# wangbaonan/RAG-SNVBERT

Hardware: AMD Instinct MI355X
Metric: masked SNVs imputed/sec (+ kNN queries/sec), window=1024 k=32 (higher is better)
Workload: dtype bf16

## Files before the change

### include/snvrag.h

```cpp
#ifndef SNVRAG_H
#define SNVRAG_H

#include <stddef.h>
#include <stdint.h>

#ifdef __cplusplus
extern "C" {
#endif

#define SNVRAG_ABI_VERSION 31

enum { SNVRAG_F32 = 0, SNVRAG_BF16 = 1 };
enum { SNVRAG_ACT_NONE = 0, SNVRAG_ACT_GELU = 1, SNVRAG_ACT_LRELU = 2, SNVRAG_ACT_SIGMOID = 3 };

int snvrag_abi_version(void);
const char* snvrag_last_error(void);
int snvrag_device_info(int device, char* name, int name_len);
int snvrag_set_option(const char* name, int64_t value);
int snvrag_get_option(const char* name, int64_t* value);

typedef struct {
  const float* bias;
  const float* row1; int64_t row1_stride; const float* col1;
  const float* row2; int64_t row2_stride; const float* col2;
  int64_t row_period;
  int act; float slope;
  const void* resid; int64_t ld_resid;
  const float* ln_g; const float* ln_b; float ln_eps; int ln_act;
  const void* post_base; int64_t ld_post; float post_scale;
  const float* post_af; int64_t post_af_period; int post_maf;
  float* stats_out;
} snvrag_epilogue_t;

typedef struct {
  const float* stats; int n_parts; int64_t dim; float eps; const float* c1;
} snvrag_rownorm_t;

int snvrag_linear(int dtype_in, int dtype_out, int64_t M, int64_t N, int64_t K,
                  const void* A, int64_t lda, const void* W, int64_t ldw,
                  void* C, int64_t ldc, const snvrag_epilogue_t* epi, void* stream);
int snvrag_linear_ex(int dtype_in, int dtype_out, int64_t M, int64_t N, int64_t K,
                     const void* A, int64_t lda, const void* W, int64_t ldw,
                     void* C, int64_t ldc, const snvrag_epilogue_t* epi,
                     const snvrag_rownorm_t* rownorm, void* stream);

typedef struct {
  const void* base; int64_t ld_base;
  float scale;
  const float* af; int64_t af_period; int maf_weight;
  int act;
} snvrag_ln_post_t;

int snvrag_layernorm(int dtype_in, int dtype_out, int64_t M, int64_t N,
                     const void* X, int64_t ldx, const void* R, int64_t ldr,
                     const float* gamma, const float* beta, float eps,
                     void* Y, int64_t ldy, const snvrag_ln_post_t* post, void* stream);

int snvrag_attention(int dtype, int64_t nseq, int64_t L, int heads, int dh,
                     const void* qkv, int64_t ld_qkv, void* out, int64_t ld_out,
                     float scale, void* stream);
int snvrag_attention_fallbacks(int reset);

int snvrag_af_features(int dtype_out, int64_t M, const float* af, const float* freqs, int nb,
                       void* feat, void* stream);
int snvrag_embed_tokens(int dtype_out, int64_t nseq, int64_t L, int64_t D, const int64_t* tok,
                        const float* W, int64_t vocab, const float* pe, const void* afemb,
                        int afemb_dtype, int64_t af_period, void* out, void* stream);

typedef struct {
  const float* c1_w; const float* c1_b;
  const float* c2_w; const float* c2_b;
  const float* c3_w; const float* c3_b;
  const float* bn1_w; const float* bn1_b; const float* bn1_rm; const float* bn1_rv;
  const float* bn2_w; const float* bn2_b; const float* bn2_rm; const float* bn2_rv;
  float bn_eps;
} snvrag_posfeat_w_t;
int snvrag_posfeat(int64_t B, int64_t L, const float* pos, const snvrag_posfeat_w_t* w,
                   float* out, void* stream);

typedef struct {
  const float* g1_w; const float* g1_b;
  const float* g2_w; const float* g2_b;
  const float* j_w; const float* j_b;
  const float* ln_w; const float* ln_b;
  float res_scale;
} snvrag_afgate_w_t;
int snvrag_af_gate(int dtype_out, int64_t M, int64_t D, const float* af, const float* af_p,
                   const snvrag_afgate_w_t* w, void* out, void* stream);

int snvrag_rag_weighted_concat(int dtype, int64_t M, int64_t D, const void* q, const void* rag,
                               const void* wgt, int64_t period, void* out, void* stream);

int snvrag_hap_head_out(int dtype_in, int64_t M, int64_t K, const void* H, int64_t ldh,
                        const float* w , const float* b ,
                        float* logits , float* probs , void* stream);
typedef struct {
  const float* f_w; const float* f_b;
  const float* n_w; const float* n_b;
  const float* w1; const float* b1;
  const float* ln_w; const float* ln_b;
  const float* w2; const float* b2;
  const float* c_w; const float* c_b;
} snvrag_gt_w_t;
int snvrag_gt_head(int64_t M, const float* p1, const float* p2, const float* ref,
                   const float* het, const float* hom, int64_t period,
                   const snvrag_gt_w_t* w, float* out , void* stream);

size_t snvrag_knn_lut_bytes(int64_t nq, int32_t n_sites_pad, int limbs);
int snvrag_knn_lut(int64_t nq, int64_t L, int64_t D, const int64_t* tok_q, const float* W,
                   const float* Aq, int64_t aq_period, const float* Ar,
                   const uint8_t* site_mask, int32_t n_sites, int32_t n_sites_pad,
                   int tok0, int tok1, int mask_tok, int limbs,
                   void* lut_out, int32_t* exp_out, float* const_out, void* stream);
int snvrag_knn_lut_panel(int64_t nq, int64_t L, int64_t D, const int64_t* tok_q, const float* W,
                         const float* Wp, const float* Aq, int64_t aq_period, const float* Ar,
                         const uint8_t* site_mask, int32_t n_sites, int32_t n_sites_pad,
                         int tok0, int tok1, int mask_tok, int limbs,
                         void* lut_out, int32_t* exp_out, float* const_out, void* stream);

int snvrag_knn_scan_parts(int64_t n_ref, int32_t nq);
int snvrag_knn_scan(const uint8_t* codes, int64_t n_ref, int64_t ld_codes, int32_t n_sites_pad,
                    const void* lut, int32_t nq, int limbs, int k, int64_t ref_offset,
                    uint64_t* part_keys, int32_t n_parts, const int32_t* th_init, void* stream);
int snvrag_knn_threshold(const uint64_t* keys, int32_t nq, int k, int32_t* th_out, void* stream);
size_t snvrag_topk_merge_ws_bytes(int32_t n_lists, int32_t nq, int k);
int snvrag_topk_merge(const uint64_t* keys, int32_t n_lists, int32_t nq, int k,
                      uint64_t* out_keys, void* ws, size_t ws_bytes, void* stream);
int snvrag_knn_decode(const uint64_t* keys, int32_t nq, int k, const int32_t* exps,
                      const float* consts, int64_t* idx_out, float* dist_out, void* stream);

int snvrag_knn_emb_splits(int64_t N, int64_t K, int Bq);
size_t snvrag_knn_emb_ws_bytes(int64_t N, int Bq, int splits);
size_t snvrag_knn_emb_packed_bytes(int64_t N, int64_t K);
int snvrag_knn_emb_pack(const void* E, int64_t N, int64_t K, void* Et, void* stream);
int snvrag_knn_emb_scan(const void* Et, int64_t N, int64_t K, const void* Q, int Bq, int splits, float* ws,
                        void* stream);
int snvrag_knn_emb_finish(const float* ws, int splits, int Bq, int64_t N, const float* qn, const float* rn,
                          float* dist, void* stream);

int snvrag_rag_mean(int dtype_out, int64_t nq, int64_t L, int64_t D, int k, const int64_t* idx,
                    const uint8_t* codes, int64_t ld_codes, int32_t n_sites,
                    const float* W, const float* pe, const float* Ar,
                    int tok0, int tok1, int sos, int eos, int pad, void* out, void* stream);

int snvrag_neighbor_counts(int64_t nq, int k, const int64_t* idx, const uint8_t* codes, int64_t ld,
                           int64_t row0, int64_t n_rows, uint8_t* counts, int64_t ld_out, void* stream);
int snvrag_rag_mean_counts(int dtype_out, int64_t nq, int64_t L, int64_t D, int k, const int64_t* idx,
                           const uint8_t* counts, int64_t ld_counts, int32_t n_sites,
                           const float* W, const float* pe, const float* Ar,
                           int tok0, int tok1, int sos, int eos, int pad, void* out, void* stream);

int snvrag_panel_pack_bits(const uint8_t* codes, int64_t n, int64_t ld, uint8_t* bits, int64_t ld_bits,
                           void* stream);
int snvrag_panel_synth_bits(uint8_t* bits, int64_t row0, int64_t n_rows, int64_t ld_bits, int32_t n_sites,
                            const float* af, uint64_t seed, void* stream);
int snvrag_panel_unpack_rows(const uint8_t* bits, int64_t n_ref, int64_t ld_bits, const int64_t* rows,
                             int64_t n_rows, uint8_t* out, int64_t ld_out, void* stream);
int snvrag_knn_scan_bits(const uint8_t* bits, int64_t n_ref, int64_t ld_bits, int32_t n_sites_pad,
                         const void* lut, int32_t nq, int limbs, int k, int64_t ref_offset,
                         uint64_t* part_keys, int32_t n_parts, const int32_t* th_init, void* stream);
int snvrag_rag_mean_bits(int dtype_out, int64_t nq, int64_t L, int64_t D, int k, const int64_t* idx,
                         const uint8_t* bits, int64_t ld_bits, int32_t n_sites,
                         const float* W, const float* pe, const float* Ar,
                         int tok0, int tok1, int sos, int eos, int pad, void* out, void* stream);
int snvrag_neighbor_counts_bits(int64_t nq, int k, const int64_t* idx, const uint8_t* bits, int64_t ld_bits,
                                int64_t row0, int64_t n_rows, uint8_t* counts, int64_t ld_out, void* stream);

int snvrag_hamming_lists(int64_t nq, int64_t N, int32_t nw, int k, const uint32_t* codes_wm,
                         const uint32_t* queries, uint64_t* lists, void* stream);
int32_t snvrag_hamming_list_count(void);

int snvrag_panel_synth(uint8_t* codes, int64_t n_ref, int64_t ld, int32_t n_sites,
                       const float* af, uint64_t seed, void* stream);
int snvrag_panel_synth_rows(uint8_t* codes, int64_t row0, int64_t n_rows, int64_t ld, int32_t n_sites,
                            const float* af, uint64_t seed, void* stream);

typedef struct {
  const void* w_qkv; const float* b_qkv;
  const void* w_o; const float* b_o;
  const float* ln1_g; const float* ln1_b;
  const void* w1; const float* b1;
  const float* lnf_g; const float* lnf_b;
  const void* w2; const float* b2;
  const float* ln2_g; const float* ln2_b;
  const void* w2g; const float* b2g; const float* c2g;
  float q_scale;
  const float* ffn_v;
  const void* tail_w;
  const void* qkv_pw;
  const void* qkv_sg;
} snvrag_layer_t;

size_t snvrag_tail_pack_bytes(int D);
int snvrag_tail_pack(int D, const void* w_o, const void* w1, const void* w2g, void* out, void* stream);
int snvrag_tail_forward(int64_t M, int D, const void* att, void* x, const void* wstream, const float* b_o,
                        const float* ln1_g, const float* ln1_b, const float* ffn_vec, float eps, void* stream);
int snvrag_tail_ffn_forward(int64_t M, int D, const void* x1, void* out, const void* wstream,
                            const float* ffn_vec, float eps, void* stream);
int snvrag_tail_qkv_forward(int64_t M, int D, const void* att, void* x, const void* wstream, const float* b_o,
                            const float* ln1_g, const float* ln1_b, const float* ffn_vec, float eps,
                            const void* qkv_pw, const float* b_qkv, void* qkv_out, void* stream);
int snvrag_tail_stamps(void* buf);
size_t snvrag_proj_pack_bytes(int D, int NC);
int snvrag_proj_pack(int D, int NC, const void* w, void* out, void* stream);
int snvrag_proj_forward(int64_t M, int D, int NC, const void* x, const void* wstream, const float* bias,
                        void* out, void* stream);

int snvrag_sgemm_cat_forward(int64_t M, int Dh, int N, const void* q, const void* x2, const void* g2,
                             int64_t period2, const void* wstream, const float* vec, void* out, void* stream);
size_t snvrag_mlp_pack_bytes(int D);
int snvrag_mlp_pack(int D, const void* w1, const void* w2, void* out, void* stream);
int snvrag_mlp_forward(int64_t M, int D, int epi2, const void* x, const void* wstream, const float* vec,
                       const float* r1, const float* r2, int64_t period, float eps, void* out, void* stream);
int snvrag_mlp_afgate_forward(int64_t M, int D, const float* af, const float* af_p, const void* gate_frags,
                              float res_scale, const void* wstream, const float* vec, void* out, void* stream);
size_t snvrag_sgemm_pack_bytes(int D, int N);
int snvrag_sgemm_pack(int D, int N, const void* w, void* out, void* stream);

typedef struct {
  int32_t kind, nparts;
  int64_t rows, cols, dst_ld, piece0, pieces;
  int64_t part_rows[4], rs[4], cs[4];
  const float* src[4];
  void* dst;
} snvrag_derive_job_t;
int snvrag_derive(const snvrag_derive_job_t* jobs, int njobs, int64_t total_pieces, void* stream);

size_t snvrag_gemm256_pack_bytes(int N, int K);
int snvrag_gemm256_pack(int N, int K, const void* w, int64_t ldw, void* out, void* stream);
int snvrag_gemm256_forward(int64_t M, int N, int K, const void* A, int64_t lda, const void* wpacked, const float* bias,
                           const void* resid, int64_t ld_resid, void* out, int64_t ldo, void* stream);
int snvrag_gemm256_ln_forward(int64_t M, int N, int K, const void* A, int64_t lda, const void* wpacked,
                              const float* bias, const float* ln_g, const float* ln_b, float eps, const void* base,
                              int64_t ld_base, float post_scale, const float* post_af, int64_t post_af_period,
                              void* out, int64_t ldo, void* stream);

int snvrag_head2_fwd(int64_t M, int K, const void* x, const float* w, const float* b, float* out, void* stream);
size_t snvrag_head2_ws_bytes(int64_t M, int K);
size_t snvrag_tokgrad_ws_bytes(int64_t M, int V, int D);
int snvrag_tokgrad(int64_t M, int V, int D, int padding_idx, const int64_t* tok, const float* g, float* dw,
                   void* ws, size_t ws_bytes, void* stream);
int snvrag_head2_bwd(int64_t M, int K, const float* g, const void* x, const float* w, void* dx, float* dw,
                     int accumulate, void* ws, size_t ws_bytes, void* stream);
int snvrag_sgemm_forward(int64_t M, int D, int N, int epi, int act, float slope, const void* x,
                         const void* wstream, const float* vec, const float* r1, const float* r2,
                         int64_t period, float eps, void* out, float* probs, float* logits, void* stream);

size_t snvrag_encoder_ws_bytes(int dtype, int64_t nseq, int64_t L, int D, int heads);
int snvrag_encoder_forward(int dtype, int64_t nseq, int64_t L, int D, int heads, int n_layers,
                           const snvrag_layer_t* layers, void* x, void* ws, size_t ws_bytes,
                           void* stream);

int snvrag_evlog_enable(int capacity);
int snvrag_evlog_pause(int paused);
int snvrag_evlog_reset(void);
int snvrag_evlog_read(int* kinds, float* ms, double* work, int max);

int snvrag_attention_train_fwd(int64_t nseq, int64_t L, int heads, int dh, const void* qkv, int64_t ld_qkv,
                               void* out, int64_t ld_out, float* lse, float scale, float dropout_p,
                               uint64_t seed, void* stream);
int snvrag_attention_bwd(int64_t nseq, int64_t L, int heads, int dh, const void* qkv, int64_t ld_qkv,
                         const void* out, int64_t ld_out, const void* dout, int64_t ld_dout,
                         const float* lse, float* d_ws, void* dqkv, int64_t ld_dqkv, float scale,
                         float dropout_p, uint64_t seed, void* stream);
int snvrag_focal_loss(int64_t M, int C, const float* probs, const int64_t* labels, const uint8_t* mask,
                      float gamma, float weight, float* loss_sum, float* grad, void* stream);
size_t snvrag_focal_loss_det_ws_bytes(int64_t M);
int snvrag_focal_loss_det(int64_t M, int C, const float* probs, const int64_t* labels, const uint8_t* mask,
                          float gamma, float weight, float* loss_sum, float* grad, float* ws, size_t ws_bytes,
                          void* stream);
int snvrag_sqnorm(int64_t n, const float* x, float* acc, void* stream);
size_t snvrag_sqnorm_ws_bytes(void);
int snvrag_sqnorm_ws(int64_t n, const float* x, float* acc, float* ws, size_t ws_bytes, void* stream);
typedef struct {
  float lr, beta1, beta2, eps, weight_decay;
  float grad_scale;
  float max_norm;
  int step;
} snvrag_adam_t;
int snvrag_adam_step(int64_t n, float* p, const float* g, float* m, float* v, void* p_bf16,
                     const float* sqnorm, const snvrag_adam_t* a, void* stream);
int snvrag_confusion(int64_t M, int C, const float* probs, const int64_t* labels, const uint8_t* mask,
                     const uint8_t* mask2, uint64_t* counts, void* stream);

int snvrag_ln_fwd_train(int64_t M, int N, const void* x, const void* r, const float* g, const float* b,
                        float eps, void* y, void* s_out, float* stats, float p_r, float p_out, uint64_t seed,
                        void* stream);
int snvrag_ln_fwd_train_act(int64_t M, int N, const void* x, const void* r, const float* g, const float* b,
                            float eps, void* y, void* s_out, float* stats, float p_r, float p_out, uint64_t seed,
                            float slope_x, float slope_r, void* stream);
int snvrag_ln_bwd_act(int64_t M, int N, const void* dy, const void* s, const float* stats, const float* g,
                      void* ds, void* dres, const void* r_pre, float* dg, float* db, int accumulate, float p_r,
                      float p_out, uint64_t seed, float slope_x, float slope_r, void* ws, size_t ws_bytes,
                      void* stream);
int snvrag_nbr_mean_drop_fwd(int64_t nq, int k, int64_t L, int D, int n_sites, int64_t ld_codes, int V,
                             const int32_t* inv, const uint8_t* codes, const float* W, const float* pe,
                             const float* Ar, float p, uint64_t seed, int tok0, int sos, int eos, int pad,
                             float* out, void* stream);
int snvrag_nbr_mean_drop_bwd(int64_t nq, int k, int64_t L, int D, int n_sites, int64_t ld_codes, int V,
                             const int32_t* inv, const uint8_t* codes, const float* W, const float* pe,
                             const float* Ar, float p, uint64_t seed, int tok0, int sos, int eos, int pad,
                             const float* dout, float* dW, float* dAr, void* stream);
size_t snvrag_nbr_mean_drop_bwd_det_ws_bytes(int64_t L, int V, int D);
int snvrag_nbr_mean_drop_bwd_det(int64_t nq, int k, int64_t L, int D, int n_sites, int64_t ld_codes, int V,
                                 const int32_t* inv, const uint8_t* codes, const float* W, const float* pe,
                                 const float* Ar, float p, uint64_t seed, int tok0, int sos, int eos, int pad,
                                 const float* dout, float* dW, float* dAr, void* ws, size_t ws_bytes, void* stream);
size_t snvrag_ln_bwd_ws_bytes(int64_t M, int N);
int snvrag_ln_bwd(int64_t M, int N, const void* dy, const void* s, const float* stats, const float* g,
                  void* ds, void* dres, float* dg, float* db, int accumulate, float p_r, float p_out,
                  uint64_t seed, void* ws, size_t ws_bytes, void* stream);
size_t snvrag_colsum_ws_bytes(int64_t M, int N);
int snvrag_colsum_bf16(int64_t M, int N, const void* x, float* out, void* ws, size_t ws_bytes, void* stream);

int snvrag_dw_splits(int64_t M, int64_t N, int64_t K);
int snvrag_linear_dw(int64_t M, int64_t N, int64_t K, const void* dy, int64_t ldy, const void* x, int64_t ldx,
                     float* dw, float* db, int splits, void* stream);
int snvrag_linear_dw_parts(int64_t M, int64_t N, int64_t K, const void* dy, int64_t ldy, const void* x,
                           int64_t ldx, int n_parts, float* const* dw_parts, float* const* db_parts, int splits,
                           void* stream);
size_t snvrag_linear_dw_det_ws_bytes(int64_t M, int64_t N, int64_t K, int splits);
int snvrag_linear_dw_det(int64_t M, int64_t N, int64_t K, const void* dy, int64_t ldy, const void* x, int64_t ldx,
                         float* dw, float* db, int splits, void* ws, size_t ws_bytes, void* stream);
int snvrag_linear_dw_parts_det(int64_t M, int64_t N, int64_t K, const void* dy, int64_t ldy, const void* x,
                               int64_t ldx, int n_parts, float* const* dw_parts, float* const* db_parts,
                               int splits, void* ws, size_t ws_bytes, void* stream);

int snvrag_infer_post(int64_t M, const float* probs_h1, const float* probs_h2, float* p1, float* p2,
                      float* gt, void* stream);

int snvrag_infer_scatter(int64_t B, int32_t L, const float* probs_h1, const float* probs_h2,
                         const int64_t* mask, const int32_t* rows_dev, const int32_t* rows_host,
                         int32_t window_len, int64_t n_variants, int64_t S, float* hap1, float* hap2,
                         float* gp, int64_t* mask_out, void* stream);

typedef struct {
  const uint8_t* gt_bits;
  const int32_t* win_off;
  const int32_t* site_row;
  const int32_t* freq_col;
  const float* pos_norm;
  const uint8_t* win_mask;
  const float* freq;
  const int32_t* pop_of_sample;
  int64_t ld_bits;
  int64_t n_cols;
  int32_t n_samples;
  int32_t n_windows;
  int32_t max_window_sites;
  int32_t n_pop;
  int32_t global_row;
} snvrag_feature_tables_t;
int snvrag_batch_features(const snvrag_feature_tables_t* tables, const int32_t* rows_dev,
                          const int32_t* rows_host, int64_t B, int32_t L, int sos, int eos, int pad, int mask,
                          int tok0, int tok1, int64_t* tokens, int64_t* mask_out, float* floats, int64_t* labels,
                          void* stream);

int snvrag_vcf_format(int64_t n, int64_t S, const float* h1, const float* h2, const float* gt,
                      int64_t n_lines, const int32_t* rows, const int64_t* line_off, const int32_t* prefix_off,
                      const uint8_t* prefix_blob, int64_t prefix_bytes, uint8_t* out, int64_t out_bytes,
                      int32_t* bad_count, void* stream);

int snvrag_site_stats(int64_t n, int64_t S, const float* h1, const float* h2, const float* gt,
                      const int8_t* truth, int64_t n_truth, int64_t S_truth, const int32_t* truth_row,
                      const int32_t* truth_col, double* est, double* acc, int32_t* table, int32_t* bad_count,
                      void* stream);

size_t snvrag_vcf_line_index_ws_bytes(int64_t nbytes);
int snvrag_vcf_line_index(const uint8_t* text, int64_t nbytes, int64_t max_lines, int64_t* line_off,
                          int64_t* n_lines, void* ws, size_t ws_bytes, void* stream);
size_t snvrag_vcf_parse_ws_bytes(int64_t n_lines, int64_t S);
int snvrag_vcf_parse_gt(const uint8_t* text, int64_t nbytes, const int64_t* line_off, int64_t n_lines,
                        int64_t S, int force_general, int32_t* pos, uint32_t* flags, uint8_t* codes,
                        int64_t ld_codes, void* ws, size_t ws_bytes, void* stream);
int snvrag_vcf_pack_rows(const uint8_t* codes, int64_t ld_codes, int64_t n_lines, int64_t S, int64_t site0,
                         uint8_t* alt_bits, uint8_t* miss_bits, int64_t ld_bits, void* stream);
int snvrag_panel_gather_bits(const uint8_t* bits, int64_t N, int64_t ld_bits, int64_t n_src_sites,
                             const int32_t* site_idx, int64_t n, int64_t n_sites_pad, int packed, uint8_t* out,
                             void* stream);
int snvrag_vcf_unpack_gt(const uint8_t* alt_bits, const uint8_t* miss_bits, int64_t ld_bits, int64_t S,
                         int64_t n_sites, int8_t* gt, void* stream);

enum { SNVRAG_INFL_OK = 0, SNVRAG_INFL_BAD_TYPE = 1, SNVRAG_INFL_BAD_STORED = 2, SNVRAG_INFL_BAD_LENGTHS = 3,
       SNVRAG_INFL_BAD_SYMBOL = 4, SNVRAG_INFL_BAD_DISTANCE = 5, SNVRAG_INFL_INPUT_END = 6,
       SNVRAG_INFL_OUTPUT_FULL = 7, SNVRAG_INFL_OUTPUT_SHORT = 8, SNVRAG_INFL_BAD_CRC = 9 };
int snvrag_bgzf_inflate(const uint8_t* comp, int64_t comp_bytes, const int64_t* table_host, int64_t* table_dev,
                        int64_t n_blocks, uint8_t* text, int64_t text_bytes, int32_t* status, void* stream);
int snvrag_text_last_newline(const uint8_t* text, int64_t nbytes, int64_t* out, void* stream);

int snvrag_bgzf_deflate(const uint8_t* text, int64_t nbytes, int64_t block_size, uint8_t* members,
                        int32_t* member_len, void* stream);
int snvrag_bgzf_pack(const uint8_t* members, const int32_t* member_len, int64_t n_blocks, uint8_t* out,
                     int64_t out_bytes, int64_t* total, void* stream);

int snvrag_selftest_mfma(void* stream);

#ifdef __cplusplus
}
#endif
#endif
```

### rag-snvbert_amd/csrc/common.h

```cpp
#pragma once
#include <hip/hip_runtime.h>
#include <stdint.h>
#include <stddef.h>
#include <string>
#include <type_traits>

#pragma clang diagnostic ignored "-Winline-asm"

#include "../../include/snvrag.h"
#include "host.h"

namespace snvrag {

typedef __bf16 bf16;
typedef __bf16 bf16x8 __attribute__((ext_vector_type(8)));
typedef __bf16 bf16x4 __attribute__((ext_vector_type(4)));
typedef float f32x4 __attribute__((ext_vector_type(4)));
typedef float f32x16 __attribute__((ext_vector_type(16)));
typedef int i32x4 __attribute__((ext_vector_type(4)));
typedef uint32_t u32x4 __attribute__((ext_vector_type(4)));

void set_error(const std::string& msg);

enum EvKind { EV_GEMM = 1, EV_ATTN = 2, EV_LN = 3, EV_KNN_SCAN = 4, EV_KNN_LUT = 5, EV_MERGE = 6, EV_OTHER = 7, EV_BLOCK = 8,
              EV_ATTN_BWD = 10, EV_TRAIN = 11 };
bool evlog_on();
void evlog_begin(hipStream_t s);
void evlog_end(hipStream_t s, int kind, double work);
struct Options {
  int64_t knn_no_reduce;
  int64_t scan_mode;
  int64_t scan_nt;
  int64_t unfused_ln;
  int64_t encoder_chunk;
  int64_t gemm_tile128;
  int64_t gemm_nw;
  int64_t tail_variant;
  int64_t tail_desync;
  int64_t sg_desync;
  int64_t mlp_desync;
  int64_t g2_desync;
  int64_t sg_waves4;
  int64_t ln_bwd_nopf;
  int64_t attn_variant;
  int64_t dw_xcd;
  int64_t ln_rows1;
  int64_t g2_groups;
  int64_t g2_variant;
  int64_t tail_split;
  int64_t proj_wide;
  int64_t tail_wide;
  int64_t tail_qkv;
  int64_t deterministic;
};
Options& options();
unsigned long long* diag_stamps();

int tailw_launch(int M, const void* att, const void* resid, void* out, const void* ws, const float* vec,
                 const float* b_o, const float* g1, const float* be1, float eps, int desync, int var,
                 const void* pw, const float* pbias, void* qkv_out, hipStream_t s);

int projw_launch(int M, int NC, const void* x, const void* ws, const float* bias, void* out, int desync, hipStream_t s);

__device__ __forceinline__ i32x4 dma_rsrc(const void* base, long bytes) {
  const uint64_t a = (uint64_t)(uintptr_t)base;
  i32x4 r;
  r[0] = __builtin_amdgcn_readfirstlane((int)(uint32_t)a);
  r[1] = __builtin_amdgcn_readfirstlane((int)((uint32_t)(a >> 32) & 0xffffu));
  r[2] = __builtin_amdgcn_readfirstlane((int)(bytes < 0x7fffffffL ? bytes : 0x7fffffffL));
  r[3] = 0x00020000;
  return r;
}

__device__ __forceinline__ void dma_x4(const i32x4& rsrc, uint32_t lds, int voffset, int soffset) {
  asm volatile("s_mov_b32 m0, %0\n\ts_nop 0\n\tbuffer_load_dwordx4 %1, %2, %3 offen lds"
               :
               : "s"(lds), "v"(voffset), "s"(rsrc), "s"(soffset)
               : "memory", "m0");
}
__device__ __forceinline__ uint32_t lds_addr(const void* p) {
  return __builtin_amdgcn_readfirstlane((int)(uint32_t)(uintptr_t)p);
}
template <typename A, typename B>
__device__ __forceinline__ void retire_loads(A& a, B& b) { asm volatile("" : "+v"(a), "+v"(b)); }
template <typename A, typename B, typename C>
__device__ __forceinline__ void retire_loads(A& a, B& b, C& c) { asm volatile("" : "+v"(a), "+v"(b), "+v"(c)); }

template <int PPT>
__device__ __forceinline__ void ring_wait(int y) {
  if (y >= 2) asm volatile("s_waitcnt vmcnt(%0)" ::"n"(2 * PPT) : "memory");
  else if (y == 1) asm volatile("s_waitcnt vmcnt(%0)" ::"n"(PPT) : "memory");
  else asm volatile("s_waitcnt vmcnt(0)" ::: "memory");
}

__device__ __forceinline__ float to_f32(float x) { return x; }
__device__ __forceinline__ float to_f32(bf16 x) { return (float)x; }
template <typename T> __device__ __forceinline__ T from_f32(float x);
template <> __device__ __forceinline__ float from_f32<float>(float x) { return x; }
template <> __device__ __forceinline__ bf16 from_f32<bf16>(float x) { return (bf16)x; }

__device__ __forceinline__ float gelu_erf(float x) {
  const float ax = fabsf(x) * 0.70710678118654752f;
  const float t = __builtin_amdgcn_rcpf(fmaf(0.3275911f, ax, 1.0f));
  float q = fmaf(t, 1.061405429f, -1.453152027f);
  q = fmaf(t, q, 1.421413741f);
  q = fmaf(t, q, -0.284496736f);
  q = fmaf(t, q, 0.254829592f);
  q = t * q * __builtin_amdgcn_exp2f(ax * ax * -1.4426950408889634f);
  return x * (x >= 0.f ? fmaf(-0.5f, q, 1.0f) : 0.5f * q);
}
__device__ __forceinline__ float gelu_bf16(float x) {
  constexpr float L2E = 1.4426950408889634f;
  const float xc = __builtin_amdgcn_fmed3f(x, -8.f, 8.f);
  const float x2 = xc * xc;
  const float z = xc * fmaf(x2, fmaf(x2, 7.03033577e-4f * L2E, -7.40112920e-2f * L2E), -1.59501577f * L2E);
  return x * __builtin_amdgcn_rcpf(1.0f + __builtin_amdgcn_exp2f(z));
}
__device__ __forceinline__ float sigmoidf_(float x) { return 1.0f / (1.0f + __expf(-x)); }

__device__ __forceinline__ float apply_act(int act, float x, float slope) {
  switch (act) {
    case SNVRAG_ACT_GELU: return gelu_erf(x);
    case SNVRAG_ACT_LRELU: return x >= 0.f ? x : x * slope;
    case SNVRAG_ACT_SIGMOID: return 1.0f / (1.0f + expf(-x));
    default: return x;
  }
}
template <typename TO> __device__ __forceinline__ float apply_act_t(int act, float x, float slope) {
  if constexpr (std::is_same<TO, bf16>::value) {
    if (act == SNVRAG_ACT_GELU) return gelu_bf16(x);
  }
  return apply_act(act, x, slope);
}

__device__ __forceinline__ float wave_sum(float v) {
#pragma unroll
  for (int o = 32; o >= 1; o >>= 1) v += __shfl_xor(v, o, 64);
  return v;
}
template <int CTRL> __device__ __forceinline__ float dpp_mov(float v) {
  return __builtin_bit_cast(float, __builtin_amdgcn_update_dpp(0, __builtin_bit_cast(int, v), CTRL, 0xF, 0xF, false));
}
template <int W> __device__ __forceinline__ float group_sum(float v) {
  static_assert(W == 2 || W == 4 || W == 8 || W == 16, "group width");
  v += dpp_mov<0xB1>(v);
  if constexpr (W >= 4) v += dpp_mov<0x4E>(v);
  if constexpr (W >= 8) v += dpp_mov<0x141>(v);
  if constexpr (W >= 16) v += dpp_mov<0x140>(v);
  return v;
}
__device__ __forceinline__ float wave_max(float v) {
#pragma unroll
  for (int o = 32; o >= 1; o >>= 1) v = fmaxf(v, __shfl_xor(v, o, 64));
  return v;
}

}
```

### rag-snvbert_amd/csrc/engine.hip

```cpp
#include "common.h"

#include <cmath>

namespace snvrag {

static int64_t chunk_seqs(int64_t nseq, int64_t L, int D, int esz) {
  if (options().encoder_chunk > 0) return std::min<int64_t>(options().encoder_chunk, nseq);
  const double per_seq = (double)L * D * 10.0 * esz;
  int64_t c = (int64_t)(16.0e9 / per_seq);
  if (c < 1) c = 1;
  if (c >= nseq) return nseq;
  const int64_t nchunks = (nseq + c - 1) / c;
  return (nseq + nchunks - 1) / nchunks;
}

}

using namespace snvrag;

extern "C" size_t snvrag_encoder_ws_bytes(int dtype, int64_t nseq, int64_t L, int D, int heads) {
  (void)heads;
  const int esz = dtype == SNVRAG_BF16 ? 2 : 4;
  const int64_t c = chunk_seqs(nseq, L, D, esz);
  const size_t M = (size_t)c * L;
  return M * (size_t)D * 9 * esz + M * 64 * 8 + 8192;
}

extern "C" int snvrag_encoder_forward(int dtype, int64_t nseq, int64_t L, int D, int heads, int n_layers,
                                      const snvrag_layer_t* layers, void* x, void* ws, size_t ws_bytes,
                                      void* stream) {
  SNV_CHECK_PTRS(layers, x, ws);
  SNV_CHECK_ARG(D % heads == 0, "D % heads");
  SNV_CHECK_ARG(ws_bytes >= snvrag_encoder_ws_bytes(dtype, nseq, L, D, heads), "encoder workspace too small");
  const int esz = dtype == SNVRAG_BF16 ? 2 : 4;
  const int64_t cs = chunk_seqs(nseq, L, D, esz);
  const size_t Mc = (size_t)cs * L;
  char* w = (char*)ws;
  auto carve = [&](size_t elems) { char* p = w; w += ((elems * esz + 255) / 256) * 256; return (void*)p; };
  void* qkv = carve(Mc * 3 * D);
  void* att = carve(Mc * D);
  void* x1 = carve(Mc * D);
  void* h = carve(Mc * 4 * D);
  const int n_stat_parts = (4 * D) % 384 == 0 ? (4 * D) / 384 : (4 * D) % 256 == 0 ? (4 * D) / 256
                           : (4 * D) % 128 == 0 ? (4 * D) / 128 : (4 * D) / 64;
  w = (char*)(((uintptr_t)w + 255) & ~(uintptr_t)255);
  void* stats = w; w += ((Mc * n_stat_parts * 8 + 255) / 256) * 256;
  const int dh = D / heads;
  const float scale = 1.0f / sqrtf((float)dh);

  const bool fused = (D == 64 || D == 128 || D == 256 || D == 384) && !options().unfused_ln &&
                     layers[0].w2g && layers[0].b2g && layers[0].c2g;
  for (int64_t s0 = 0; s0 < nseq; s0 += cs) {
    const int64_t ns = std::min<int64_t>(cs, nseq - s0);
    const int64_t M = ns * L;
    char* xc = (char*)x + (size_t)s0 * L * D * esz;
    bool have_qkv = false;
    for (int i = 0; i < n_layers; ++i) {
      const snvrag_layer_t& ly = layers[i];
      snvrag_epilogue_t e{};
      int rc;
      e.bias = ly.b_qkv;
      if (have_qkv)
        rc = 0;
      else if (dtype == SNVRAG_BF16 && ly.qkv_sg && M * 3 * D * 2 < (1L << 31))
        rc = snvrag_sgemm_forward(M, (int)D, (int)(3 * D), 0, SNVRAG_ACT_NONE, 0.f, xc, ly.qkv_sg, ly.b_qkv, nullptr,
                                  nullptr, 0, 0.f, qkv, nullptr, nullptr, stream);
      else if (dtype == SNVRAG_BF16 && ly.qkv_pw)
        rc = snvrag_proj_forward(M, D, 3, xc, ly.qkv_pw, ly.b_qkv, qkv, stream);
      else
        rc = snvrag_linear(dtype, dtype, M, 3 * D, D, xc, D, ly.w_qkv, D, qkv, 3 * D, &e, stream);
      if (rc) return rc;
      const float sc = ly.q_scale > 0.f ? scale / ly.q_scale : scale;
      rc = snvrag_attention(dtype, ns, L, heads, dh, qkv, 3 * D, att, D, sc, stream);
      if (rc) return rc;
      if (fused && dtype == SNVRAG_BF16 && ly.tail_w && ly.ffn_v) {
        have_qkv = i + 1 < n_layers && D == 384 && options().tail_qkv && options().tail_variant == 0 &&
                   (options().tail_wide == 1 || options().tail_wide == 2) && layers[i + 1].qkv_pw &&
                   layers[i + 1].b_qkv && M * 3 * D * 2 < (1L << 31);
        if (have_qkv)
          rc = snvrag_tail_qkv_forward(M, D, att, xc, ly.tail_w, ly.b_o, ly.ln1_g, ly.ln1_b, ly.ffn_v, 1e-5f,
                                       layers[i + 1].qkv_pw, layers[i + 1].b_qkv, qkv, stream);
        else
          rc = snvrag_tail_forward(M, D, att, xc, ly.tail_w, ly.b_o, ly.ln1_g, ly.ln1_b, ly.ffn_v, 1e-5f, stream);
        if (rc) return rc;
        continue;
      }
      if (fused) {
        e = snvrag_epilogue_t{};
        e.bias = ly.b_o; e.resid = xc; e.ld_resid = D; e.ln_g = ly.ln1_g; e.ln_b = ly.ln1_b; e.ln_eps = 1e-5f;
        rc = snvrag_linear(dtype, dtype, M, D, D, att, D, ly.w_o, D, x1, D, &e, stream);
        if (rc) return rc;
        e = snvrag_epilogue_t{};
        e.bias = ly.b1; e.act = SNVRAG_ACT_LRELU; e.slope = 0.1f; e.stats_out = (float*)stats;
        rc = snvrag_linear(dtype, dtype, M, 4 * D, D, x1, D, ly.w1, D, h, 4 * D, &e, stream);
        if (rc) return rc;
        snvrag_rownorm_t rn{(const float*)stats, n_stat_parts, 4 * D, 1e-5f, ly.c2g};
        e = snvrag_epilogue_t{};
        e.bias = ly.b2g; e.act = SNVRAG_ACT_LRELU; e.slope = 0.1f; e.resid = x1; e.ld_resid = D;
        e.ln_g = ly.ln2_g; e.ln_b = ly.ln2_b; e.ln_eps = 1e-5f;
        rc = snvrag_linear_ex(dtype, dtype, M, D, 4 * D, h, 4 * D, ly.w2g, 4 * D, xc, D, &e, &rn, stream);
        if (rc) return rc;
        continue;
      }
      e = snvrag_epilogue_t{};
      e.bias = ly.b_o; e.resid = xc; e.ld_resid = D;
      rc = snvrag_linear(dtype, dtype, M, D, D, att, D, ly.w_o, D, x1, D, &e, stream);
      if (rc) return rc;
      rc = snvrag_layernorm(dtype, dtype, M, D, x1, D, nullptr, 0, ly.ln1_g, ly.ln1_b, 1e-5f, x1, D, nullptr, stream);
      if (rc) return rc;
      e = snvrag_epilogue_t{};
      e.bias = ly.b1; e.act = SNVRAG_ACT_LRELU; e.slope = 0.1f;
      rc = snvrag_linear(dtype, dtype, M, 4 * D, D, x1, D, ly.w1, D, h, 4 * D, &e, stream);
      if (rc) return rc;
      rc = snvrag_layernorm(dtype, dtype, M, 4 * D, h, 4 * D, nullptr, 0, ly.lnf_g, ly.lnf_b, 1e-5f, h, 4 * D,
                            nullptr, stream);
      if (rc) return rc;
      e = snvrag_epilogue_t{};
      e.bias = ly.b2; e.act = SNVRAG_ACT_LRELU; e.slope = 0.1f; e.resid = x1; e.ld_resid = D;
      rc = snvrag_linear(dtype, dtype, M, D, 4 * D, h, 4 * D, ly.w2, 4 * D, xc, D, &e, stream);
      if (rc) return rc;
      rc = snvrag_layernorm(dtype, dtype, M, D, xc, D, nullptr, 0, ly.ln2_g, ly.ln2_b, 1e-5f, xc, D, nullptr, stream);
      if (rc) return rc;
    }
  }
  return 0;
}
```

### rag-snvbert_amd/csrc/misc.hip

```cpp
#include "common.h"

#include <cctype>
#include <cstdlib>
#include <cstring>

namespace snvrag {

static thread_local std::string g_err;

struct EvLog {
  bool on = false;
  int cap = 0, n = 0;
  hipEvent_t* ev = nullptr;
  int* kind = nullptr;
  double* work = nullptr;
};
static EvLog g_ev;

bool evlog_on() { return g_ev.on && g_ev.n < g_ev.cap; }
void evlog_begin(hipStream_t s) {
  if (evlog_on()) (void)hipEventRecord(g_ev.ev[2 * g_ev.n], s);
}
void evlog_end(hipStream_t s, int kind, double work) {
  if (!evlog_on()) return;
  (void)hipEventRecord(g_ev.ev[2 * g_ev.n + 1], s);
  g_ev.kind[g_ev.n] = kind;
  g_ev.work[g_ev.n] = work;
  g_ev.n++;
}

void set_error(const std::string& msg) { g_err = msg; }
int fail(const char* where, const std::string& msg) {
  g_err = std::string(where) + ": " + msg;
  return 1;
}

__global__ void mfma_selftest_kernel(int* errors) {
  const int lane = threadIdx.x, li = lane & 15, lg = lane >> 4;
  __shared__ int A[16][64], B[64][16];
  for (int i = lane; i < 16 * 64; i += 64) {
    const int r = i / 64, k = i % 64;
    A[r][k] = ((r * 7 + k * 3) % 11) - 5;
    B[k][r] = ((k * 5 + r * 13) % 9) - 4;
  }
  __syncthreads();
  int err = 0;
  {
    int8_t a8[16], b8[16];
    for (int j = 0; j < 16; ++j) { a8[j] = (int8_t)A[li][16 * lg + j]; b8[j] = (int8_t)B[16 * lg + j][li]; }
    i32x4 av = *reinterpret_cast<i32x4*>(a8), bv = *reinterpret_cast<i32x4*>(b8);
    i32x4 c = __builtin_amdgcn_mfma_i32_16x16x64_i8(av, bv, i32x4{0, 0, 0, 0}, 0, 0, 0);
    for (int i = 0; i < 4; ++i) {
      const int row = 4 * lg + i, col = li;
      int ref = 0;
      for (int k = 0; k < 64; ++k) ref += A[row][k] * B[k][col];
      err += c[i] != ref;
    }
  }
  {
    bf16x8 av, bv;
    for (int j = 0; j < 8; ++j) { av[j] = (bf16)(float)A[li][8 * lg + j]; bv[j] = (bf16)(float)B[8 * lg + j][li]; }
    f32x4 c = __builtin_amdgcn_mfma_f32_16x16x32_bf16(av, bv, f32x4{0, 0, 0, 0}, 0, 0, 0);
    for (int i = 0; i < 4; ++i) {
      const int row = 4 * lg + i, col = li;
      int ref = 0;
      for (int k = 0; k < 32; ++k) ref += A[row][k] * B[k][col];
      err += c[i] != (float)ref;
    }
  }
  {
    f32x4 c = __builtin_amdgcn_mfma_f32_16x16x4f32((float)A[li][lg], (float)B[lg][li], f32x4{0, 0, 0, 0}, 0, 0, 0);
    for (int i = 0; i < 4; ++i) {
      const int row = 4 * lg + i, col = li;
      int ref = 0;
      for (int k = 0; k < 4; ++k) ref += A[row][k] * B[k][col];
      err += c[i] != (float)ref;
    }
  }
  atomicAdd(errors, err);
}

}

using namespace snvrag;

namespace snvrag {
namespace {
struct OptDesc { const char* name; int64_t Options::*field; int64_t dflt; };
const OptDesc kOpts[] = {
    {"knn_no_reduce", &Options::knn_no_reduce, 0}, {"scan_mode", &Options::scan_mode, 0},
    {"scan_nt", &Options::scan_nt, -1},            {"unfused_ln", &Options::unfused_ln, 0},
    {"encoder_chunk", &Options::encoder_chunk, 0}, {"gemm_tile128", &Options::gemm_tile128, 0},
    {"gemm_nw", &Options::gemm_nw, 0},             {"tail_variant", &Options::tail_variant, 0},
    {"tail_desync", &Options::tail_desync, -1},    {"sg_desync", &Options::sg_desync, -1},      {"mlp_desync", &Options::mlp_desync, -1},      {"g2_desync", &Options::g2_desync, -1},
    {"sg_waves4", &Options::sg_waves4, 0},         {"ln_bwd_nopf", &Options::ln_bwd_nopf, 0},
    {"attn_variant", &Options::attn_variant, 0},   {"dw_xcd", &Options::dw_xcd, 1},
    {"ln_rows1", &Options::ln_rows1, 0},           {"tail_wide", &Options::tail_wide, 1},
    {"proj_wide", &Options::proj_wide, 1},         {"g2_variant", &Options::g2_variant, 0},
    {"g2_groups", &Options::g2_groups, 0},         {"tail_split", &Options::tail_split, 64},
    {"deterministic", &Options::deterministic, 0}, {"tail_qkv", &Options::tail_qkv, 1},
};
Options make_options() {
  Options o{};
  for (const OptDesc& d : kOpts) {
    std::string env = "SNVRAG_";
    for (const char* c = d.name; *c; ++c) env += (char)toupper(*c);
    const char* v = getenv(env.c_str());
    o.*(d.field) = v ? atoll(v) : d.dflt;
  }
  return o;
}
const OptDesc* find_opt(const char* name) {
  for (const OptDesc& d : kOpts)
    if (name && strcmp(d.name, name) == 0) return &d;
  return nullptr;
}
}
Options& options() {
  static Options o = make_options();
  return o;
}
}

extern "C" int snvrag_set_option(const char* name, int64_t value) {
  const snvrag::OptDesc* d = snvrag::find_opt(name);
  if (!d) return fail(__func__, std::string("unknown option ") + (name ? name : "(null)"));
  snvrag::options().*(d->field) = value;
  return 0;
}

extern "C" int snvrag_get_option(const char* name, int64_t* value) {
  const snvrag::OptDesc* d = snvrag::find_opt(name);
  if (!d || !value) return fail(__func__, std::string("unknown option ") + (name ? name : "(null)"));
  *value = snvrag::options().*(d->field);
  return 0;
}

extern "C" int snvrag_abi_version(void) { return SNVRAG_ABI_VERSION; }
extern "C" const char* snvrag_last_error(void) { return g_err.c_str(); }

extern "C" int snvrag_device_info(int device, char* name, int name_len) {
  hipDeviceProp_t p;
  if (hipGetDeviceProperties(&p, device) != hipSuccess) return -1;
  if (name && name_len > 0) {
    std::strncpy(name, p.gcnArchName, name_len - 1);
    name[name_len - 1] = 0;
  }
  return p.multiProcessorCount;
}

extern "C" int snvrag_evlog_enable(int capacity) {
  if (g_ev.ev) {
    for (int i = 0; i < 2 * g_ev.cap; ++i) (void)hipEventDestroy(g_ev.ev[i]);
    delete[] g_ev.ev; delete[] g_ev.kind; delete[] g_ev.work;
    g_ev = EvLog{};
  }
  if (capacity <= 0) return 0;
  g_ev.ev = new hipEvent_t[2 * capacity];
  g_ev.kind = new int[capacity];
  g_ev.work = new double[capacity];
  for (int i = 0; i < 2 * capacity; ++i) SNV_HIP(hipEventCreate(&g_ev.ev[i]));
  g_ev.cap = capacity;
  g_ev.n = 0;
  g_ev.on = true;
  return 0;
}

extern "C" int snvrag_evlog_pause(int paused) { g_ev.on = !paused && g_ev.cap > 0; return 0; }
extern "C" int snvrag_evlog_reset(void) { g_ev.n = 0; return 0; }

extern "C" int snvrag_evlog_read(int* kinds, float* ms, double* work, int max) {
  const int n = g_ev.n < max ? g_ev.n : max;
  for (int i = 0; i < n; ++i) {
    SNV_HIP(hipEventSynchronize(g_ev.ev[2 * i + 1]));
    float t = 0.f;
    SNV_HIP(hipEventElapsedTime(&t, g_ev.ev[2 * i], g_ev.ev[2 * i + 1]));
    kinds[i] = g_ev.kind[i];
    ms[i] = t;
    work[i] = g_ev.work[i];
  }
  return n;
}

extern "C" int snvrag_selftest_mfma(void* stream) {
  int* d = nullptr;
  SNV_HIP(hipMalloc(&d, sizeof(int)));
  hipStream_t s = as_stream(stream);
  SNV_HIP(hipMemsetAsync(d, 0, sizeof(int), s));
  hipLaunchKernelGGL(mfma_selftest_kernel, dim3(1), dim3(64), 0, s, d);
  int h = -1;
  SNV_HIP(hipMemcpyAsync(&h, d, sizeof(int), hipMemcpyDeviceToHost, s));
  SNV_HIP(hipStreamSynchronize(s));
  SNV_HIP(hipFree(d));
  return h;
}
```

### rag-snvbert_amd/csrc/tailw.hip

```cpp
#include "common.h"
#include "mfma32.h"

namespace snvrag {

#ifndef TW_PACKED_LN
#define TW_PACKED_LN 1
#endif

constexpr int TW_D = 384, TW_NT = 12, TW_KS = 24;
constexpr int TW_FPRE = TW_NT * TW_KS;
constexpr int TW_FPC = 96;
constexpr int TW_NFRAG = TW_FPRE + 24 * TW_FPC;
constexpr int TW_X = 0;
constexpr int TW_H = 96 * 1024;
constexpr int TW_LDS = 160 * 1024;
constexpr int TW_AH = 9;
constexpr int TW_RING = 12;
constexpr int TW_QA = 24;
constexpr int TW_Q0 = 48;
constexpr int TW_HS = 32;
constexpr int TW_QF = TW_Q0 + 11 * TW_HS;
constexpr int TW_QEND = TW_QF + 8;
constexpr int TW_QREP = TW_Q0 + TW_HS;
constexpr int TW_NB1 = 4;

__host__ __device__ constexpr int tw_nf(int q) {
  return q < 0 ? 0 : q < TW_QA ? 3 : q < TW_Q0 ? 1 : q < TW_QF ? ((q - TW_Q0) % TW_HS < 24 ? 1 : 3) : q < TW_QEND ? 3 : 0;
}
__host__ __device__ constexpr int tw_f0(int q) {
  if (q <= TW_QA) return 3 * q;
  if (q <= TW_Q0) return 72 + (q - TW_QA);
  if (q <= TW_QF) {
    const int k = (q - TW_Q0) / TW_HS, r = (q - TW_Q0) % TW_HS;
    return 96 + 48 * k + (r <= 24 ? r : 24 + 3 * (r - 24));
  }
  return q <= TW_QEND ? 624 + 3 * (q - TW_QF) : 648;
}
__host__ __device__ constexpr int tw_step_of(int m) {
  if (m < 72) return m / 3;
  if (m < 96) return TW_QA + (m - 72);
  if (m < 624) {
    const int k = (m - 96) / 48, r = (m - 96) % 48;
    return TW_Q0 + TW_HS * k + (r < 24 ? r : 24 + (r - 24) / 3);
  }
  return TW_QF + (m - 624) / 3;
}
constexpr int TW_NFRAGW = 648;
__host__ __device__ constexpr int tw_extra(int q) {
  return (q == TW_QA + 16 || (q >= TW_Q0 && q < TW_QF && (q - TW_Q0) % TW_HS == 24)) ? TW_NB1 : 0;
}
__host__ __device__ constexpr int tw_issuer(int n) { return n < TW_AH ? -1 : tw_step_of(n - TW_AH); }
__host__ __device__ constexpr int tw_min(int a, int b) { return a < b ? a : b; }
__host__ __device__ constexpr int tw_younger(int q) {
  const int nl = tw_f0(q) + tw_nf(q) - 1;
  int n = tw_min(tw_f0(q) + TW_AH, TW_NFRAGW) - 1 - nl;
  const int qi = tw_issuer(nl);
  for (int j = qi < 0 ? 0 : qi; j < q; ++j) n += tw_extra(j);
  return n;
}
__host__ __device__ constexpr int tw_ops_between(int qa, int qb) {
  int n = 0;
  for (int q = qa + 1; q <= qb; ++q) n += (tw_f0(q) + TW_AH < TW_NFRAGW ? tw_nf(q) : 0) + tw_extra(q);
  return n;
}
constexpr int TW_B1_WAIT = tw_min(tw_ops_between(TW_QA + 16, TW_Q0 + 2), tw_ops_between(TW_Q0 + 24, TW_QREP + 2));
constexpr int TW_B1_WAIT_END = tw_ops_between(TW_Q0 + 10 * TW_HS + 24, TW_QF - 1);
__host__ __device__ constexpr int tw_younger_it(int i) {
  int m = 63;
  for (int h = 1; h <= 11; ++h) m = tw_min(m, tw_younger(TW_Q0 + (h - 1) * TW_HS + i));
  return m;
}
__host__ __device__ constexpr int tw_wait_of(int q) {
  return (q >= TW_QREP && q < TW_QREP + TW_HS) ? tw_younger_it(q - TW_QREP) : tw_younger(q);
}
__host__ __device__ constexpr bool tw_ring_periodic() {
  return tw_f0(TW_QEND) == TW_NFRAGW && tw_f0(TW_QA) % TW_RING == 0 && tw_f0(TW_Q0) % TW_RING == 0 &&
         tw_f0(TW_QREP) % TW_RING == 0 && (tw_f0(TW_QREP + TW_HS) - tw_f0(TW_QREP)) % TW_RING == 0 &&
         tw_f0(TW_QF) % TW_RING == 0;
}
static_assert(tw_ring_periodic(), "fragment ring registers periodic over the sections");
static_assert(TW_B1_WAIT_END <= 63 && tw_younger(0) <= 63, "vmcnt range");

#ifndef TW_NOPMASK
#define TW_NOPMASK 2
#endif
__device__ __forceinline__ void tw_drain_o(f32x16 (&a)[3][4]) {
  asm volatile("s_nop 7\n\ts_nop 7\n\ts_nop 7"
               : "+a"(a[0][0]), "+a"(a[0][1]), "+a"(a[0][2]), "+a"(a[0][3]), "+a"(a[1][0]), "+a"(a[1][1]),
                 "+a"(a[1][2]), "+a"(a[1][3]), "+a"(a[2][0]), "+a"(a[2][1]), "+a"(a[2][2]), "+a"(a[2][3])
               :: "memory");
}
template <bool AGPR> __device__ __forceinline__ void tw_drain_h4(f32x16 (&h)[4]) {
  if constexpr (AGPR)
    asm volatile("s_nop 7\n\ts_nop 7\n\ts_nop 7" : "+a"(h[0]), "+a"(h[1]), "+a"(h[2]), "+a"(h[3]) :: "memory");
  else
    asm volatile("s_nop 7\n\ts_nop 7\n\ts_nop 7" : "+v"(h[0]), "+v"(h[1]), "+v"(h[2]), "+v"(h[3]) :: "memory");
}
__device__ __forceinline__ f32x2 tw_lrelu2(f32x2 x) {
  const f32x2 m = x * 0.1f;
  float a, b;
  asm("v_max_f32 %0, %1, %2" : "=v"(a) : "v"(x.x), "v"(m.x));
  asm("v_max_f32 %0, %1, %2" : "=v"(b) : "v"(x.y), "v"(m.y));
  return f32x2{a, b};
}
__device__ __forceinline__ void tw_ld16p(const char* p, float (&v)[16]) {
#pragma unroll
  for (int i = 0; i < 4; ++i) {
    const f32x4 q = *reinterpret_cast<const f32x4*>(p + 16 * i);
#pragma unroll
    for (int j = 0; j < 4; ++j) v[4 * i + j] = q[j];
  }
}
#ifndef TW_ASM_WAITS
#define TW_ASM_WAITS 0
#endif
template <int Y> __device__ __forceinline__ void tw_wait1(u32x4& a) {
  static_assert(Y >= 0 && Y <= 63, "vmcnt range");
  if constexpr (TW_ASM_WAITS) asm volatile("s_waitcnt vmcnt(%1)" : "+v"(a) : "n"(Y) : "memory");
}
template <int Y> __device__ __forceinline__ void tw_wait3(u32x4& a, u32x4& b, u32x4& c) {
  static_assert(Y >= 0 && Y <= 63, "vmcnt range");
  if constexpr (TW_ASM_WAITS) asm volatile("s_waitcnt vmcnt(%3)" : "+v"(a), "+v"(b), "+v"(c) : "n"(Y) : "memory");
}
template <int OFF> __device__ __forceinline__ void tw_load_off(u32x4& r, int voff, const i32x4& rsrc, int so) {
  asm volatile("buffer_load_dwordx4 %0, %1, %2, %3 offen offset:%4" : "=v"(r) : "v"(voff), "s"(rsrc), "s"(so), "n"(OFF) : "memory");
}
__device__ __forceinline__ void tw_barrier() { asm volatile("s_waitcnt lgkmcnt(0)\n\ts_barrier" ::: "memory"); }

struct TwArgs {
  int M;
  const bf16* att;
  const bf16* resid;
  bf16* out;
  const char* ws;
  const float* vec;
  const float* b_o; const float* g1; const float* be1;
  float eps;
  int desync;
  unsigned long long* stamps;
  int n_full;
  const char* pw;
  const float* pbias;
  bf16* qkv_out;
};

__device__ __forceinline__ void pw_loadW(u32x4& r, const __amdgpu_buffer_rsrc_t wrb, int lane16, int wave, int NC, int c,
                                         int n72) {
  const int cc = c < NC ? c : NC - 1;
  r = __builtin_amdgcn_raw_buffer_load_b128(wrb, lane16, (cc * TW_FPRE + (n72 / 3) * TW_NT + 3 * wave + n72 % 3) * FRAG_BYTES, 0);
}
template <int G, bool NOP>
__device__ __forceinline__ void pw_chunks(const char* smem, uint32_t bias_lds, int wave, int lane16,
                                          const __amdgpu_buffer_rsrc_t wrb, int NC, const __amdgpu_buffer_rsrc_t ors,
                                          u32x4 (&wf)[TW_RING], f32x16 (&acc)[3][4]) {
  constexpr int D = TW_D, KS = TW_KS, GI = G > 1 ? 1 : 0;
  auto rdB = [&](int blk) -> u32x4 { return *reinterpret_cast<const u32x4*>(smem + TW_X + blk * FRAG_BYTES + lane16); };
  u32x4 bq[2][4];
#pragma unroll 1
  for (int c = 0; c < NC; ++c) {
#pragma unroll
    for (int g = 0; g < G; ++g) bq[0][g] = rdB(g);
    unroll([&](auto sc) {
      constexpr int s = decltype(sc)::value, n0 = 3 * s;
#pragma unroll
      for (int g = 0; g < G; ++g) {
#pragma unroll
        for (int t = 0; t < 3; ++t) {
          if constexpr (s == 0) mfma32_asm0<true, NOP>(acc[t][g], wf[(n0 + t) % TW_RING], bq[s & 1][g]);
          else mfma32_asm<true, NOP>(acc[t][g], wf[(n0 + t) % TW_RING], bq[s & 1][g]);
        }
        if constexpr (s + 1 < KS) bq[(s + 1) & 1][g] = rdB((s + 1) * 4 + g);
        if (g == GI) {
#pragma unroll
          for (int t = 0; t < 3; ++t) {
            const int m = n0 + TW_AH + t;
            if (m < 72) pw_loadW(wf[(n0 + TW_AH + t) % TW_RING], wrb, lane16, wave, NC, c, m);
            else pw_loadW(wf[(n0 + TW_AH + t) % TW_RING], wrb, lane16, wave, NC, c + 1, m - 72);
          }
        }
      }
      __builtin_amdgcn_sched_barrier(0);
    }, std::make_integer_sequence<int, KS>{});
    tw_drain_o(acc);
    const int l = lane_id();
    const uint32_t bb = bias_lds + 4 * (c * D + 16 * (l >> 5));
#pragma unroll
    for (int t = 0; t < 3; ++t) {
      const int T = 3 * wave + t;
      float bv[16];
      ld16(bb + 4 * 32 * T, bv);
#pragma unroll
      for (int g = 0; g < G; ++g) {
        const int ro = ((32 * g + (l & 31)) * NC * D + c * D + 32 * T + 16 * (l >> 5)) * 2;
#pragma unroll
        for (int h2 = 0; h2 < 2; ++h2) {
          float y[8];
#pragma unroll
          for (int j = 0; j < 8; ++j) y[j] = acc[t][g][8 * h2 + j] + bv[8 * h2 + j];
          __builtin_amdgcn_raw_buffer_store_b128(u32x4{pack2(y[0], y[1]), pack2(y[2], y[3]), pack2(y[4], y[5]),
                                                       pack2(y[6], y[7])},
                                                 ors, ro + 16 * h2, 0, 0);
        }
      }
    }
  }
}
__device__ __forceinline__ __amdgpu_buffer_rsrc_t pw_out_rsrc(bf16* out, int M, long row0, int NC) {
  const long o_bytes = ((long)M - row0) * NC * TW_D * 2;
  return __builtin_amdgcn_make_buffer_rsrc((void*)(out + row0 * NC * TW_D), (short)0,
                                           (int)(o_bytes < 0x7fffffffL ? o_bytes : 0x7fffffffL), 0x00020000);
}

template <bool STAMP, int G, bool PROJ>
__device__ __forceinline__ void tailw_body(const TwArgs& p, const long row0, const int wave) {
  constexpr int D = TW_D, NT = TW_NT, GI = G > 1 ? 1 : 0;
  constexpr uint32_t TW_PB = TW_H + 16 * 1024;
  constexpr int TW_RES_STEP = 21;
  constexpr bool NOPA = G == 1 || (TW_NOPMASK & 1), NOP0 = G == 1 || (TW_NOPMASK & 2);
  constexpr bool NOPT = G == 1 || (TW_NOPMASK & 4), NOPF = G == 1 || (TW_NOPMASK & 8);
  constexpr bool NOPP = G == 1 || (TW_NOPMASK & 16);
  using TNA = std::integral_constant<bool, NOP0>;
  using TNT = std::integral_constant<bool, NOPT>;
  using TNF = std::integral_constant<bool, NOPF>;
  extern __shared__ __attribute__((aligned(16))) char smem[];
  unsigned long long st[8] = {};
  auto stamp = [&](int i) {
    if constexpr (STAMP) st[i] = __builtin_amdgcn_s_memtime();
  };
  if (p.desync > 0 && blockIdx.x < 256) stagger_wait(p.desync);
  stamp(0);
  const uint32_t lds0 = lds_addr(smem);
  int lane16 = lane_id() * 16;
  asm volatile("" : "+v"(lane16));

  const i32x4 ars = dma_rsrc(p.att + row0 * D, ((long)p.M - row0) * D * 2);
  const i32x4 wrs = dma_rsrc(p.ws, (long)TW_NFRAG * FRAG_BYTES);
  const i32x4 brs = dma_rsrc(p.vec, 4L * D * 4);
  {
    const int l = lane_id();
    const int voff = (32 * wave + (l & 31)) * (D * 2) + 32 * (l >> 5);
    if (wave < G) {
#pragma unroll
      for (int s = 0; s < TW_KS; ++s)
        dma_x4(ars, lds0 + TW_X + (s * 4 + wave) * FRAG_BYTES, voff, 64 * (s >> 1) + 16 * (s & 1));
    }
  }
  u32x4 wf[TW_RING];
  const __amdgpu_buffer_rsrc_t wrb = __builtin_amdgcn_make_buffer_rsrc((void*)p.ws, (short)0, TW_NFRAG * FRAG_BYTES, 0x00020000);
  auto loadW = [&](u32x4& r, int F) { r = __builtin_amdgcn_raw_buffer_load_b128(wrb, lane16, F * FRAG_BYTES, 0); };
  auto f_ffn1 = [&](int h, int i) { return TW_FPRE + (4 * (h >> 1) + wave) * TW_FPC + 2 * i + (h & 1); };
  auto f_ffn2 = [&](int h, int u, int t) {
    return TW_FPRE + (4 * (h >> 1) + (u >> 1)) * TW_FPC + 48 + (2 * (h & 1) + (u & 1)) * NT + 3 * wave + t;
  };
  auto issue_a = [&](auto n_tag) {
    constexpr int n = decltype(n_tag)::value;
    if constexpr (n < 72) loadW(wf[n % TW_RING], (n / 3) * NT + 3 * wave + n % 3);
    else if constexpr (n < 96) loadW(wf[n % TW_RING], f_ffn1(0, n - 72));
    else loadW(wf[n % TW_RING], f_ffn1(1, n - 96));
  };
  unroll([&](auto nc) { issue_a(nc); }, std::make_integer_sequence<int, TW_AH>{});
  u32x4 rr[3][4][2];
  auto load_res = [&]() {
    const int l = lane_id();
#pragma unroll
    for (int g = 0; g < G; ++g) {
      long r = row0 + 32 * g + (l & 31);
      r = r < p.M ? r : (long)p.M - 1;
#pragma unroll
      for (int t = 0; t < 3; ++t)
#pragma unroll
        for (int h2 = 0; h2 < 2; ++h2)
          rr[t][g][h2] = *reinterpret_cast<const u32x4*>(p.resid + r * D + 32 * (3 * wave + t) + 16 * (l >> 5) + 8 * h2);
    }
  };
  float* tab = reinterpret_cast<float*>(smem + TW_H);
  for (int i = 64 * wave + lane_id(); i < D; i += 256) {
    tab[i] = p.b_o[i];
    tab[D + i] = p.g1[i];
    tab[2 * D + i] = p.be1[i];
  }
  asm volatile("s_waitcnt vmcnt(0)" ::: "memory");
  tw_barrier();
  stamp(1);

  f32x16 acc[3][4];
  u32x4 bq[3][4];
  auto rdB = [&](uint32_t base, int blk) -> u32x4 {
    return *reinterpret_cast<const u32x4*>(smem + base + blk * FRAG_BYTES + lane16);
  };
#pragma unroll
  for (int g = 0; g < G; ++g) bq[0][g] = rdB(TW_X, g);
  unroll([&](auto qc) {
    constexpr int q = decltype(qc)::value, n0 = 3 * q;
    tw_wait3<tw_younger(q)>(wf[n0 % TW_RING], wf[(n0 + 1) % TW_RING], wf[(n0 + 2) % TW_RING]);
#pragma unroll
    for (int g = 0; g < G; ++g) {
#pragma unroll
      for (int t = 0; t < 3; ++t) {
        if constexpr (q == 0) mfma32_asm0<true, NOPA>(acc[t][g], wf[(n0 + t) % TW_RING], bq[q & 1][g]);
        else mfma32_asm<true, NOPA>(acc[t][g], wf[(n0 + t) % TW_RING], bq[q & 1][g]);
      }
      if constexpr (q + 1 < TW_KS) bq[(q + 1) & 1][g] = rdB(TW_X, (q + 1) * 4 + g);
      if (g == GI)
        unroll([&](auto tc) { issue_a(std::integral_constant<int, n0 + TW_AH + decltype(tc)::value>{}); },
                  std::make_integer_sequence<int, 3>{});
    }
    if constexpr (q == TW_RES_STEP) load_res();
    __builtin_amdgcn_sched_barrier(0);
  }, std::make_integer_sequence<int, TW_QA>{});
  tw_drain_o(acc);
  stamp(2);

  float2* s1 = reinterpret_cast<float2*>(smem + TW_H + 8 * 1024);
  {
    const uint32_t tb = lds0 + TW_H + 64 * (lane_id() >> 5);
#if TW_PACKED_LN
    f32x2 s2v[4], q2v[4];
#pragma unroll
    for (int g = 0; g < G; ++g) s2v[g] = q2v[g] = f32x2{0.f, 0.f};
#pragma unroll
    for (int t = 0; t < 3; ++t) {
      float bo[16];
      tw_ld16p(smem + (tb - lds0) + 4 * 32 * (3 * wave + t), bo);
#pragma unroll
      for (int g = 0; g < G; ++g)
#pragma unroll
        for (int e = 0; e < 8; ++e) {
          const f32x2 v = f32x2{acc[t][g][2 * e], acc[t][g][2 * e + 1]} + f32x2{bo[2 * e], bo[2 * e + 1]} +
                          bf_pair(rr[t][g][e >> 2][e & 3]);
          acc[t][g][2 * e] = v.x;
          acc[t][g][2 * e + 1] = v.y;
          s2v[g] += v;
          q2v[g] = v * v + q2v[g];
        }
    }
    float sum[4], sq[4];
#pragma unroll
    for (int g = 0; g < G; ++g) {
      sum[g] = s2v[g].x + s2v[g].y;
      sq[g] = q2v[g].x + q2v[g].y;
    }
#else
    float sum[4] = {0.f, 0.f, 0.f, 0.f}, sq[4] = {0.f, 0.f, 0.f, 0.f};
#pragma unroll
    for (int t = 0; t < 3; ++t) {
      float bo[16];
      tw_ld16p(smem + (tb - lds0) + 4 * 32 * (3 * wave + t), bo);
#pragma unroll
      for (int g = 0; g < G; ++g)
#pragma unroll
        for (int i = 0; i < 16; ++i) {
          const float v = acc[t][g][i] + bo[i] + bf_at(rr[t][g][i >> 3], i & 7);
          acc[t][g][i] = v;
          sum[g] += v;
          sq[g] = fmaf(v, v, sq[g]);
        }
    }
#endif
#pragma unroll
    for (int t = 0; t < 3; ++t)
#pragma unroll
      for (int g = 0; g < G; ++g) {}
    const int l = lane_id();
#pragma unroll
    for (int g = 0; g < G; ++g) {
      sum[g] = xsum32(sum[g]);
      sq[g] = xsum32(sq[g]);
      s1[wave * 128 + 32 * g + (l & 31)] = make_float2(sum[g], sq[g]);
    }
  }
  tw_barrier();
  {
    const int l = lane_id();
    const uint32_t tb = lds0 + TW_H + 64 * (l >> 5);
    float mean[4], rstd[4];
#pragma unroll
    for (int g = 0; g < G; ++g) {
      float a = 0.f, b = 0.f;
#pragma unroll
      for (int w2 = 0; w2 < 4; ++w2) {
        const float2 v = s1[w2 * 128 + 32 * g + (l & 31)];
        a += v.x;
        b += v.y;
      }
      mean[g] = a * (1.0f / D);
      rstd[g] = 1.0f / sqrtf(fmaxf(b * (1.0f / D) - mean[g] * mean[g], 0.f) + p.eps);
    }
#pragma unroll
    for (int t = 0; t < 3; ++t) {
      float gg[16], bb[16];
      tw_ld16p(smem + (tb - lds0) + 4 * (D + 32 * (3 * wave + t)), gg);
      tw_ld16p(smem + (tb - lds0) + 4 * (2 * D + 32 * (3 * wave + t)), bb);
      const int T = 3 * wave + t;
#pragma unroll
      for (int g = 0; g < G; ++g) {
        float y[16];
#if TW_PACKED_LN
        const float nmr = -mean[g] * rstd[g];
#pragma unroll
        for (int e = 0; e < 8; ++e) {
          const f32x2 z = (f32x2{acc[t][g][2 * e], acc[t][g][2 * e + 1]} * rstd[g] + nmr) * f32x2{gg[2 * e], gg[2 * e + 1]} +
                          f32x2{bb[2 * e], bb[2 * e + 1]};
          y[2 * e] = z.x;
          y[2 * e + 1] = z.y;
        }
#else
#pragma unroll
        for (int i = 0; i < 16; ++i) y[i] = (acc[t][g][i] - mean[g]) * rstd[g] * gg[i] + bb[i];
#endif
#pragma unroll
        for (int h2 = 0; h2 < 2; ++h2)
          *reinterpret_cast<u32x4*>(smem + TW_X + ((2 * T + h2) * 4 + g) * FRAG_BYTES + lane16) =
              u32x4{pack2(y[8 * h2], y[8 * h2 + 1]), pack2(y[8 * h2 + 2], y[8 * h2 + 3]),
                    pack2(y[8 * h2 + 4], y[8 * h2 + 5]), pack2(y[8 * h2 + 6], y[8 * h2 + 7])};
      }
    }
  }
  tw_barrier();
  stamp(3);

  f32x16 hv[4], ha[4];
#pragma unroll
  for (int t = 0; t < 3; ++t)
#pragma unroll
    for (int g = 0; g < G; ++g) acc[t][g] = f32x16{};
#pragma unroll
  for (int t = 0; t < 3; ++t)
#pragma unroll
    for (int g = 0; g < G; ++g) asm volatile("" : "+a"(acc[t][g]));
  typedef float f2 __attribute__((ext_vector_type(2)));
  float sa1[4], sa2[4];
#pragma unroll
  for (int g = 0; g < G; ++g) sa1[g] = sa2[g] = 0.f;
  u32x4 b1v[4];
  const __amdgpu_buffer_rsrc_t b1b = __builtin_amdgcn_make_buffer_rsrc((void*)p.vec, (short)0, 4 * D * 4, 0x00020000);
  auto b1_load = [&](int h) {
    const int so = 4 * (64 * (4 * (h >> 1) + wave) + 32 * (h & 1));
    const int vo = 16 * (lane_id() >> 5);
#pragma unroll
    for (int r = 0; r < 4; ++r) b1v[r] = __builtin_amdgcn_raw_buffer_load_b128(b1b, vo + 32 * r, so, 0);
  };
  constexpr int TW_EP = 3 * G;
  float ex[8];
  uint32_t epk[4];
  auto epi_piece = [&](auto k_tag, auto q_tag, auto p_tag) {
    constexpr int k = decltype(k_tag)::value, Q = decltype(q_tag)::value, pc = decltype(p_tag)::value;
    constexpr int g = k >> 1, j = k & 1;
    if constexpr (g < G) {
      const f32x16& a = Q ? ha[g] : hv[g];
      unroll([&](auto vc) {
        constexpr int v = decltype(vc)::value;
        if constexpr (v * (TW_EP - 2) / 8 == pc) {
          const float u = a[8 * j + v] + __uint_as_float(b1v[(8 * j + v) >> 2][(8 * j + v) & 3]);
          const float x = fmaxf(u, 0.1f * u);
          ex[v] = x;
          sa1[g] += x;
          sa2[g] = fmaf(x, x, sa2[g]);
        }
      }, std::make_integer_sequence<int, 8>{});
      if constexpr (pc == TW_EP - 2) {
#pragma unroll
        for (int e2 = 0; e2 < 4; ++e2) epk[e2] = pack2(ex[2 * e2], ex[2 * e2 + 1]);
      }
      if constexpr (pc == TW_EP - 1)
        *reinterpret_cast<u32x4*>(smem + TW_H + Q * 32768 + ((wave * 2 + j) * 4 + g) * FRAG_BYTES + lane16) =
            u32x4{epk[0], epk[1], epk[2], epk[3]};
    }
  };
  auto issue_it = [&](auto r_tag, int h, auto last_tag) {
    constexpr int r = decltype(r_tag)::value, n = r;
    if constexpr (r < 24) loadW(wf[n % TW_RING], f_ffn1(h, r));
    else if constexpr (r < 48) loadW(wf[n % TW_RING], f_ffn2(h - 1, (r - 24) / 3, (r - 24) % 3));
    else if constexpr (decltype(last_tag)::value) loadW(wf[n % TW_RING], f_ffn2(h, (r - 48) / 3, (r - 48) % 3));
    else loadW(wf[n % TW_RING], f_ffn1(h + 1, r - 48));
  };
  auto seg1 = [&](int h, auto p_tag, auto q0_tag, auto epi_tag, auto nop_tag) {
    constexpr int P = decltype(p_tag)::value, Q0 = decltype(q0_tag)::value;
    constexpr bool EPI = decltype(epi_tag)::value, NOP = decltype(nop_tag)::value;
    constexpr int F0 = tw_f0(Q0);
    unroll([&](auto ic) {
      constexpr int i = decltype(ic)::value, q = Q0 + i, n = F0 + i;
      tw_wait1<tw_wait_of(q)>(wf[n % TW_RING]);
      unroll([&](auto gc) {
        constexpr int g = decltype(gc)::value;
        if constexpr (P == 0) {
          if constexpr (i == 0) mfma32_asm0<false, NOP>(hv[g], wf[n % TW_RING], bq[(i + 2) % 3][g]);
          else mfma32_asm<false, NOP>(hv[g], wf[n % TW_RING], bq[(i + 2) % 3][g]);
        } else {
          if constexpr (i == 0) mfma32_asm0<true, NOP>(ha[g], wf[n % TW_RING], bq[(i + 2) % 3][g]);
          else mfma32_asm<true, NOP>(ha[g], wf[n % TW_RING], bq[(i + 2) % 3][g]);
        }
        if constexpr (i + 2 < 24) bq[(i + 4) % 3][g] = rdB(TW_X, (i + 2) * 4 + g);
        if constexpr (g == GI) {
          if constexpr (Q0 == TW_QA) issue_a(std::integral_constant<int, n + TW_AH>{});
          else issue_it(std::integral_constant<int, i + TW_AH>{}, h, std::false_type{});
        }
        if constexpr (EPI) {
          epi_piece(std::integral_constant<int, i / 3>{}, std::integral_constant<int, 1 - P>{},
                    std::integral_constant<int, (i % 3) * G + g>{});
          __builtin_amdgcn_sched_barrier(0);
        }
      }, std::make_integer_sequence<int, G>{});
      if constexpr (Q0 == TW_QA && i == 16) b1_load(0);
      __builtin_amdgcn_sched_barrier(0);
    }, std::make_integer_sequence<int, 24>{});
    if constexpr (P == 0) tw_drain_h4<false>(hv);
    else tw_drain_h4<true>(ha);
  };
  auto seg2 = [&](int h, auto p_tag, auto q0_tag, auto last_tag, auto final_tag, auto nop_tag) {
    constexpr int P = decltype(p_tag)::value, Q0 = decltype(q0_tag)::value;
    constexpr bool LAST = decltype(last_tag)::value, FINAL = decltype(final_tag)::value;
    constexpr bool NOP = decltype(nop_tag)::value;
    constexpr uint32_t HB = TW_H + P * 32768;
    constexpr int F0 = tw_f0(Q0);
// ... 348 lines not shown
```

### rag-snvbert_amd/src/engine.py

```python

from __future__ import annotations

import weakref
from typing import Dict, Optional

import math
import os

import torch
import torch.nn as nn

from . import kernels as K
from . import native as N

_ENGINES: "weakref.WeakKeyDictionary[nn.Module, Engine]" = weakref.WeakKeyDictionary()


def engine_for(module: nn.Module) -> "Engine":
    eng = _ENGINES.get(module)
    if eng is None:
        eng = Engine(module)
        _ENGINES[module] = eng
    return eng


def _rag_block_current(x: Dict[str, torch.Tensor]) -> bool:
    if "rag_emb_h1" not in x or "rag_mean" not in x:
        return True
    m, B = x["rag_mean"], x["rag_emb_h1"].shape[0]
    return (x["rag_emb_h1"].data_ptr() == m.data_ptr() and x["rag_emb_h2"].data_ptr() == m[B:].data_ptr()
            and x["rag_emb_h1"].dtype == m.dtype)


def set_compute_dtype(module: nn.Module, dtype: torch.dtype) -> None:
    engine_for(module).set_dtype(dtype)


class _Packed:
    pass


class Engine:
    rag_tail_wide = True
    rag_afgate_fused = True

    def __init__(self, root: nn.Module):
        self.root = root
        self.dtype = torch.float32
        self._packed: Optional[_Packed] = None
        self._key = None
        self._enc_ws: Optional[torch.Tensor] = None

    def set_dtype(self, dtype: torch.dtype) -> None:
        if dtype not in (torch.float32, torch.bfloat16):
            raise ValueError("compute dtype must be float32 or bfloat16")
        if dtype != self.dtype:
            self.dtype, self._packed = dtype, None
        _, _, emb = self._modules()
        if emb is not None and emb is not self.root:
            engine_for(emb).set_dtype(dtype)

    def _modules(self):
        r = self.root
        from .model.foundation_model import BERTFoundationModel
        from .model.bert import BERT
        from .model.embedding.bert import BERTEmbedding
        from .model.embedding.af_embedding import AFEmbedding
        if isinstance(r, BERTFoundationModel):
            return r, r.bert, r.bert.embedding
        if isinstance(r, BERT):
            return None, r, r.embedding
        if isinstance(r, BERTEmbedding):
            return None, None, r
        if isinstance(r, AFEmbedding):
            return None, None, None
        raise TypeError(f"no native engine for {type(r).__name__}")

    def _param_key(self):
        from .autograd_ops import _EPOCH
        return (_EPOCH[0],) + tuple((p.data_ptr(), p._version) for p in self.root.parameters()) + \
            tuple((b.data_ptr(), b._version) for b in self.root.buffers())

    def packed(self, allow_train: bool = False) -> _Packed:
        if self.root.training and not allow_train:
            raise NotImplementedError("the native engine runs eval semantics (dropout off); train-mode "
                                      "forwards go through src/train_forward.py (BERTFoundationModel.forward)")
        key = self._param_key()
        if self._packed is None or key != self._key:
            self._packed = self._pack()
            self._key = key
        return self._packed

    def _pack(self) -> _Packed:
        fm, bert, emb = self._modules()
        dev = next(self.root.parameters()).device
        if dev.type != "cuda":
            raise N.NativeUnavailable("model parameters must live on the HIP device (model.to('cuda'))")
        N.load()
        T = self.dtype
        P = _Packed()
        f32 = lambda t: t.detach().to(dev, torch.float32).contiguous()
        cvt = lambda t: t.detach().to(dev, T).contiguous()
        P.keep = []

        def afmlp(a):
            return dict(freqs=f32(a.basis_freqs), w0=cvt(a.projection[0].weight), b0=f32(a.projection[0].bias),
                        g=f32(a.projection[1].weight), bb=f32(a.projection[1].bias),
                        w3=cvt(a.projection[3].weight), b3=f32(a.projection[3].bias))

        if emb is None:
            P.af = afmlp(self.root)
            return P
        P.D = emb.embed_size
        P.W = f32(emb.tokenizer.weight)
        P.pe = f32(emb.position.pe[0])
        P.pe0 = torch.zeros_like(P.pe)
        P.af = afmlp(emb.af_embedding) if emb.use_af else None
        if bert is None:
            return P
        D = P.D
        P.heads, P.n_layers = bert.attn_heads, bert.n_layers
        ef = bert.emb_fusion
        fw = f32(ef.fusion.weight)
        P.ef = dict(w=cvt(fw[:, :D]), c_pos=fw[:, D].contiguous(), c_af=fw[:, D + 1].contiguous(),
                    b=f32(ef.fusion.bias), g=f32(ef.norm.weight), bb=f32(ef.norm.bias))
        sg_ok = T == torch.bfloat16 and D in (128, 256, 384)
        if sg_ok:
            P.ef["w_sg"] = K.sgemm_pack(P.ef["w"])
            P.ef["v_sg"] = K.sgemm_vec(P.ef["b"], P.ef["c_pos"], P.ef["c_af"], ln=(P.ef["g"], P.ef["bb"]))
        pf = ef.pos_feat
        P.pf_t = [f32(t) for t in (pf.conv1.weight, pf.conv1.bias, pf.conv2.weight, pf.conv2.bias,
                                   pf.conv3.weight, pf.conv3.bias, pf.norm1.weight, pf.norm1.bias,
                                   pf.norm1.running_mean, pf.norm1.running_var, pf.norm2.weight, pf.norm2.bias,
                                   pf.norm2.running_mean, pf.norm2.running_var)]
        P.pf = N.PosfeatW(*[t.data_ptr() for t in P.pf_t], pf.norm1.eps)
        rf = bert.rag_fusion
        ai = rf.af_interaction
        P.ag_t = [f32(t) for t in (ai.gate_net[0].weight, ai.gate_net[0].bias, ai.gate_net[2].weight,
                                   ai.gate_net[2].bias, ai.joint_encoder[0].weight, ai.joint_encoder[0].bias,
                                   ai.joint_encoder[1].weight, ai.joint_encoder[1].bias)]
        P.ag = N.AfGateW(*[t.data_ptr() for t in P.ag_t], float(ai.res_scale.detach().float().item()))
        P.rf = dict(a0=cvt(rf.af_adapter[0].weight), a0b=f32(rf.af_adapter[0].bias),
                    a3=cvt(rf.af_adapter[3].weight), a3b=f32(rf.af_adapter[3].bias),
                    f0=cvt(rf.fusion[0].weight), f0b=f32(rf.fusion[0].bias),
                    f3=cvt(rf.fusion[3].weight), f3b=f32(rf.fusion[3].bias),
                    g=f32(rf.fusion[4].weight), bb=f32(rf.fusion[4].bias),
                    rs=float(rf.res_scale.detach().float().item()))
        if sg_ok and D == 384 and P.rf["f0"].shape == (4 * D, 2 * D):
            P.rf["f0_sg"], P.rf["f0_v"] = K.sgemm_pack(P.rf["f0"]), K.sgemm_vec(P.rf["f0b"])
        if sg_ok and D == 384 and P.rf["f3"].shape == (D, 4 * D) and self.rag_tail_wide:
            P.rf["f3_g2"] = K.gemm256_pack(P.rf["f3"])
        mlp_ok = sg_ok and D == 384
        if mlp_ok and P.rf["a0"].shape == (4 * D, D) and P.rf["a3"].shape == (D, 4 * D):
            P.rf["a_mlp"] = K.mlp_pack(P.rf["a0"], P.rf["a3"])
            P.rf["a_mlp_v"] = K.sgemm_vec(torch.cat([P.rf["a0b"], P.rf["a3b"]]))
            if self.rag_afgate_fused and P.ag_t[2].shape == (D, 32):
                P.rf["afg_frags"], P.rf["afg_v"] = K.mlp_afgate_pack(P.ag_t, P.rf["a_mlp_v"])
        elif sg_ok and P.rf["a0"].shape == (4 * D, D):
            P.rf["a0_sg"], P.rf["a0_v"] = K.sgemm_pack(P.rf["a0"]), K.sgemm_vec(P.rf["a0b"])
        P.layers_t, P.layers = [], []
        for blk in bert.transformer_blocks:
            a, ff = blk.attention, blk.feed_forward
            w2g, b2g, c2g = K.fold_layernorm(ff.w_2.weight.detach().to(dev), ff.w_2.bias.detach().to(dev),
                                             ff.norm.weight.detach().to(dev), ff.norm.bias.detach().to(dev), T)
            qs = math.log2(math.e) / math.sqrt(a.dims) if T == torch.bfloat16 else 0.0
            wq = torch.cat([l.weight for l in a.linear_layers], 0).detach().to(dev).float().clone()
            bq = torch.cat([l.bias for l in a.linear_layers], 0).detach().to(dev).float().clone()
            if qs:
                wq[:D] *= qs
                bq[:D] *= qs
            t = dict(w_qkv=cvt(wq), b_qkv=f32(bq),
                     w_o=cvt(a.output_layer.weight), b_o=f32(a.output_layer.bias),
                     ln1_g=f32(blk.input_sublayer.norm.weight), ln1_b=f32(blk.input_sublayer.norm.bias),
                     w1=cvt(ff.w_1.weight), b1=f32(ff.w_1.bias),
                     lnf_g=f32(ff.norm.weight), lnf_b=f32(ff.norm.bias),
                     w2=cvt(ff.w_2.weight), b2=f32(ff.w_2.bias),
                     ln2_g=f32(blk.output_sublayer.norm.weight), ln2_b=f32(blk.output_sublayer.norm.bias),
                     w2g=w2g, b2g=b2g, c2g=c2g)
            if T == torch.bfloat16 and D in (128, 256, 384):
                t["ffn_v"] = K.ffn_vec(t["b1"], b2g, w2g, t["ln2_g"], t["ln2_b"])
                t["tail_w"] = K.tail_pack(t["w_o"], t["w1"], w2g)
                t["qkv_sg"] = K.sgemm_pack(t["w_qkv"])
                t["qkv_pw"] = K.proj_pack(t["w_qkv"])
            P.layers_t.append(t)
            P.layers.append(N.LayerW(**{k: v.data_ptr() for k, v in t.items()}, q_scale=qs))
        if fm is None:
            return P
        hc = fm.hap_classifier
        hw = f32(hc.af_fusion[0].weight)
        P.hh = dict(w0=cvt(hw[:, :D]), c_af=hw[:, D].contiguous(), c_afp=hw[:, D + 1].contiguous(),
                    b0=f32(hc.af_fusion[0].bias), w2=cvt(hc.af_fusion[2].weight), b2=f32(hc.af_fusion[2].bias),
                    g=f32(hc.af_fusion[3].weight), bb=f32(hc.af_fusion[3].bias),
                    n0=cvt(hc.net[0].weight), n0b=f32(hc.net[0].bias),
                    n2=f32(hc.net[2].weight), n2b=f32(hc.net[2].bias))
        if sg_ok and D == 384 and P.hh["w2"].shape == (D, 4 * D):
            P.hh["f_mlp"] = K.mlp_pack(P.hh["w0"], P.hh["w2"])
            P.hh["f_mlp_v"] = torch.cat([P.hh["b0"], P.hh["c_af"], P.hh["c_afp"], P.hh["b2"], P.hh["g"],
                                         P.hh["bb"]]).float().contiguous()
        elif sg_ok and P.hh["w0"].shape == (4 * D, D):
            P.hh["w0_sg"] = K.sgemm_pack(P.hh["w0"])
            P.hh["w0_v"] = K.sgemm_vec(P.hh["b0"], P.hh["c_af"], P.hh["c_afp"])
        if sg_ok and P.hh["n2"].shape[0] == 2 and P.hh["n0"].shape == (4 * D, D):
            P.hh["n0_sg"] = K.sgemm_pack(P.hh["n0"])
            P.hh["n0_v"] = K.sgemm_vec(P.hh["n0b"], head=(P.hh["n2"], P.hh["n2b"]))
        gc = fm.gt_classifier
        P.gt_t = [f32(t) for t in (gc.gf_fusion.weight, gc.gf_fusion.bias, gc.gf_norm.weight, gc.gf_norm.bias,
                                   gc.layer.w_1.weight, gc.layer.w_1.bias, gc.layer.norm.weight,
                                   gc.layer.norm.bias, gc.layer.w_2.weight, gc.layer.w_2.bias,
                                   gc.classifier.weight, gc.classifier.bias)]
        P.gt = N.GtW(*[t.data_ptr() for t in P.gt_t])
        return P

    def af_embedding(self, af: torch.Tensor, allow_train: bool = False) -> torch.Tensor:
        P = self.packed(allow_train)
        a = P.af
        N.require_gpu(af)
        af = af.float().contiguous()
        T = self.dtype
        feat = K.af_features(af, a["freqs"], T)
        h = K.linear(feat, a["w0"], a["b0"], ln=(a["g"], a["bb"]), ln_act=N.ACT_GELU)
        return K.linear(h, a["w3"], a["b3"])

    def embed(self, seq: torch.Tensor, af: Optional[torch.Tensor] = None, pos: bool = False,
              af_period: int = 0, afemb: Optional[torch.Tensor] = None) -> torch.Tensor:
        P = self.packed()
        N.require_gpu(seq)
        seq = seq.long().contiguous()
        if afemb is None and af is not None and P.af is not None:
            afemb = self.af_embedding(af)
            af_period = af_period or afemb.shape[0]
        return K.embed_tokens(seq, P.W, P.pe if pos else P.pe0, afemb, af_period, self.dtype)

    def _inputs(self, x: Dict[str, torch.Tensor]):
        h1, h2 = x["hap_1"], x["hap_2"]
        N.require_gpu(h1, h2)
        g = lambda k: x[k].to(h1.device, torch.float32).contiguous()
        return (h1.long().contiguous(), h2.long().contiguous(), g("af"), g("af_p") if "af_p" in x else g("af"),
                g("pos"))

    def input_block(self, B: int, L: int, device) -> torch.Tensor:
        return torch.empty(4 * B, L, self.packed(allow_train=True).D, device=device, dtype=self.dtype)

    def rag_means(self, x: Dict[str, torch.Tensor], B: int, L: int, D: int) -> Optional[torch.Tensor]:
        if not _rag_block_current(x):
            x = {k: v for k, v in x.items() if k not in ("rag_block", "rag_mean")}
        if "rag_block" in x:
            return x["rag_block"][2 * B:].to(self.dtype)
        if "rag_mean" in x:
            return x["rag_mean"].to(self.dtype).contiguous()
        if "rag_emb_h1" not in x:
            return None
        out = []
        for key in ("rag_emb_h1", "rag_emb_h2"):
            r = x[key]
            r = r[:, 0] if (r.dim() == 4 and r.size(1) == 1) else (r.mean(1) if r.dim() == 4 else r)
            out.append(r.to(self.dtype))
        return torch.cat(out, 0).contiguous()

    def forward_bert(self, x: Dict[str, torch.Tensor]) -> Dict[str, torch.Tensor]:
        P = self.packed()
        T, D = self.dtype, P.D
        h1, h2, af, af_p, pos = self._inputs(x)
        B, L = h1.shape
        BL = B * L
        afemb = self.af_embedding(af)
        rag = self.rag_means(x, B, L, D)
        nblk = 4 if rag is not None else 2
        blk = x.get("rag_block") if _rag_block_current(x) else None
        if blk is not None and (blk.dtype != T or tuple(blk.shape) != (4 * B, L, D) or not blk.is_contiguous()):
            blk = None
        if blk is not None:
            hm = blk
        else:
            hm = torch.empty(nblk * B, L, D, device=h1.device, dtype=T)
        K.embed_tokens(torch.cat([h1, h2], 0), P.W, P.pe, afemb, B, T, out=hm[:2 * B])
        if rag is not None and blk is None:
            hm[2 * B:].copy_(rag)
        pf = K.posfeat(pos, P.pf)
        ef = P.ef
        if "w_sg" in ef:
            fused = K.sgemm(hm, ef["w_sg"], D, ef["v_sg"], epi=K.SG_LN, act=N.ACT_LRELU, slope=0.1,
                            rank=(pf, af, BL))
        else:
            fused = K.linear(hm, ef["w"], ef["b"], row1=(pf, 1, ef["c_pos"]), row2=(af, 1, ef["c_af"]),
                             row_period=BL, act=N.ACT_LRELU, slope=0.1, resid=hm, ln=(ef["g"], ef["bb"]))
        if rag is not None:
            rf = P.rf
            if "afg_frags" in rf:
                aw = K.mlp_afgate(af, af_p, rf["afg_frags"], P.ag.res_scale, rf["a_mlp"], rf["afg_v"], D)
            elif "a_mlp" in rf:
                fa = K.af_gate(af, af_p, P.ag, D, T)
                aw = K.mlp(fa, rf["a_mlp"], rf["a_mlp_v"], epi2=0)
            else:
                fa = K.af_gate(af, af_p, P.ag, D, T)
                if "a0_sg" in rf:
                    t = K.sgemm(fa, rf["a0_sg"], rf["a0"].shape[0], rf["a0_v"], act=N.ACT_GELU)
                else:
                    t = K.linear(fa, rf["a0"], rf["a0b"], act=N.ACT_GELU)
                aw = K.linear(t, rf["a3"], rf["a3b"], act=N.ACT_SIGMOID)
            if "f0_sg" in rf:
                h = K.sgemm_cat(fused[:2 * B], fused[2 * B:], aw, BL, rf["f0_sg"], rf["f0"].shape[0], rf["f0_v"])
            else:
                cat = K.rag_concat(fused[:2 * B], fused[2 * B:], aw, BL)
                h = K.linear(cat, rf["f0"], rf["f0b"], act=N.ACT_GELU)
            if "f3_g2" in rf:
                xx = K.gemm256_ln(h.view(-1, h.shape[-1]), rf["f3_g2"], rf["f3b"], (rf["g"], rf["bb"]),
                                  base=fused[:2 * B].view(-1, D), post_scale=rf["rs"], post_af=af.view(-1),
                                  post_af_period=BL).view(2 * B, L, D)
            else:
                xx = K.linear(h, rf["f3"], rf["f3b"], ln=(rf["g"], rf["bb"]), post_base=fused[:2 * B],
                              post_scale=rf["rs"], post_af=af, post_af_period=BL, post_maf=True)
        else:
            xx = fused[:2 * B].clone()
        ws_bytes = K.encoder_ws_bytes(T, 2 * B, L, D, P.heads)
        if self._enc_ws is None or self._enc_ws.numel() < ws_bytes or self._enc_ws.device != h1.device:
            self._enc_ws = torch.empty(ws_bytes, device=h1.device, dtype=torch.uint8)
        K.encoder_forward(xx, P.layers, P.heads, self._enc_ws)
        return dict(h1_after=xx[:B], h2_after=xx[B:], h1_before=hm[:B], h2_before=hm[B:2 * B],
                    af=af, af_p=af_p, x_all=xx, B=B, L=L)

    def forward(self, x: Dict[str, torch.Tensor], want_logits: bool = False) -> Dict[str, torch.Tensor]:
        o = self.forward_bert(x)
        P = self.packed()
        B, L = o["B"], o["L"]
        BL = B * L
        hh = P.hh
        if "f_mlp" in hh:
            h = K.mlp(o["x_all"], hh["f_mlp"], hh["f_mlp_v"], epi2=1, rank=(o["af"], o["af_p"], BL))
        else:
            if "w0_sg" in hh:
                h = K.sgemm(o["x_all"], hh["w0_sg"], hh["w0"].shape[0], hh["w0_v"], act=N.ACT_GELU,
                            rank=(o["af"], o["af_p"], BL))
            else:
                h = K.linear(o["x_all"], hh["w0"], hh["b0"], row1=(o["af"], 1, hh["c_af"]),
                             row2=(o["af_p"], 1, hh["c_afp"]), row_period=BL, act=N.ACT_GELU)
            h = K.linear(h, hh["w2"], hh["b2"], ln=(hh["g"], hh["bb"]))
        if "n0_sg" in hh:
            logits, probs = K.sgemm(h, hh["n0_sg"], hh["n0"].shape[0], hh["n0_v"], epi=K.SG_HEAD2, act=N.ACT_GELU,
                                    want_logits=want_logits)
        else:
            h = K.linear(h, hh["n0"], hh["n0b"], act=N.ACT_GELU)
            logits, probs = K.hap_head_out(h, hh["n2"], hh["n2b"], want_logits=want_logits)
        dev = probs.device
        g = lambda k: x[k].to(dev, torch.float32).contiguous()
        gt = K.gt_head(probs[:B], probs[B:], g("ref"), g("het"), g("hom"), BL, P.gt)
        o.update(probs_h1=probs[:B], probs_h2=probs[B:], gt=gt)
        if want_logits:
            o.update(logits_h1=logits[:B], logits_h2=logits[B:])
        return o
```

### rag-snvbert_amd/src/kernels.py

```python

from __future__ import annotations

import contextlib

import ctypes as C
from typing import Optional, Sequence, Tuple

import torch

from . import native as N
from .native import check, ptr, stream_ptr

_dt = N.dtype_code


def _c(t: torch.Tensor) -> torch.Tensor:
    if not t.is_contiguous():
        raise ValueError("expected a contiguous tensor")
    return t


def linear(x: torch.Tensor, w: torch.Tensor, bias: Optional[torch.Tensor] = None, *,
           act: int = N.ACT_NONE, slope: float = 0.0,
           row1: Optional[Tuple[torch.Tensor, int, torch.Tensor]] = None,
# ... 181 lines not shown


def af_features(af: torch.Tensor, freqs: torch.Tensor, dtype: torch.dtype) -> torch.Tensor:
    N.require_gpu(af)
    nb = freqs.numel()
    out = torch.empty(*af.shape, 2 * nb, device=af.device, dtype=dtype)
    check(N.lib().snvrag_af_features(_dt(dtype), af.numel(), ptr(_c(af)), ptr(_c(freqs)), nb, ptr(out),
                                     stream_ptr()), "af_features")
    return out


def embed_tokens(tok: torch.Tensor, W: torch.Tensor, pe: torch.Tensor, afemb: Optional[torch.Tensor],
                 af_period: int, dtype: torch.dtype, out: Optional[torch.Tensor] = None) -> torch.Tensor:
    N.require_gpu(tok, W, pe, afemb, out)
    assert tok.dtype == torch.int64
    nseq, L = tok.shape
    D = W.shape[1]
    if W.dtype != torch.float32 or pe.dtype != torch.float32 or pe.dim() != 2 or pe.shape[0] < L or pe.shape[1] != D:
        raise ValueError(f"W and pe must be float32 with pe [>= {L}, {D}], got pe {tuple(pe.shape)} {pe.dtype}, W {W.dtype}")
    if afemb is not None:
        rows = af_period if af_period > 0 else nseq
        if afemb.shape[-2:] != (L, D) or afemb.numel() != rows * L * D:
            raise ValueError(f"afemb must be [{rows}, {L}, {D}], got {tuple(afemb.shape)}")
        _c(afemb)
    if out is None:
        out = torch.empty(nseq, L, D, device=tok.device, dtype=dtype)
    elif out.dtype != dtype or tuple(out.shape) != (nseq, L, D):
        raise ValueError(f"out must be {dtype} [{nseq}, {L}, {D}], got {out.dtype} {tuple(out.shape)}")
    check(N.lib().snvrag_embed_tokens(_dt(dtype), nseq, L, D, ptr(_c(tok)), ptr(_c(W)), W.shape[0],
                                      ptr(_c(pe)), ptr(afemb), _dt(afemb.dtype) if afemb is not None else 0,
                                      af_period, ptr(_c(out)), stream_ptr()), "embed_tokens")
    return out


def posfeat(pos: torch.Tensor, w: "N.PosfeatW") -> torch.Tensor:
    N.require_gpu(pos)
    B, L = pos.shape
    out = torch.empty(B, L, device=pos.device, dtype=torch.float32)
    check(N.lib().snvrag_posfeat(B, L, ptr(_c(pos)), C.byref(w), ptr(out), stream_ptr()), "posfeat")
    return out


def af_gate(af: torch.Tensor, af_p: torch.Tensor, w: "N.AfGateW", D: int, dtype: torch.dtype) -> torch.Tensor:
    N.require_gpu(af)
    out = torch.empty(*af.shape, D, device=af.device, dtype=dtype)
    check(N.lib().snvrag_af_gate(_dt(dtype), af.numel(), D, ptr(_c(af)), ptr(_c(af_p)), C.byref(w), ptr(out),
                                 stream_ptr()), "af_gate")
    return out


def rag_concat(q: torch.Tensor, rag: torch.Tensor, wgt: torch.Tensor, period: int) -> torch.Tensor:
    D = q.shape[-1]
    M = q.numel() // D
    out = torch.empty(*q.shape[:-1], 2 * D, device=q.device, dtype=q.dtype)
    check(N.lib().snvrag_rag_weighted_concat(_dt(q.dtype), M, D, ptr(_c(q)), ptr(_c(rag)), ptr(_c(wgt)),
                                             period, ptr(out), stream_ptr()), "rag_concat")
    return out


def hap_head_out(h: torch.Tensor, w: torch.Tensor, b: torch.Tensor, want_logits: bool = True):
    K = h.shape[-1]
    M = h.numel() // K
    probs = torch.empty(*h.shape[:-1], 2, device=h.device, dtype=torch.float32)
    logits = torch.empty_like(probs) if want_logits else None
    check(N.lib().snvrag_hap_head_out(_dt(h.dtype), M, K, ptr(_c(h)), K, ptr(_c(w)), ptr(_c(b)),
                                      ptr(logits), ptr(probs), stream_ptr()), "hap_head_out")
    return logits, probs


def gt_head(p1, p2, ref, het, hom, period: int, w: "N.GtW") -> torch.Tensor:
    M = p1.numel() // 2
    out = torch.empty(*p1.shape[:-1], 4, device=p1.device, dtype=torch.float32)
    check(N.lib().snvrag_gt_head(M, ptr(_c(p1)), ptr(_c(p2)), ptr(_c(ref)), ptr(_c(het)), ptr(_c(hom)), period,
                                 C.byref(w), ptr(out), stream_ptr()), "gt_head")
    return out


def knn_lut(tok_q: torch.Tensor, W: torch.Tensor, site_mask: torch.Tensor, n_sites: int, n_sites_pad: int,
            limbs: int = 2, Aq: Optional[torch.Tensor] = None, aq_period: int = 0,
            Ar: Optional[torch.Tensor] = None, tok0: int = 5, tok1: int = 6, mask_tok: int = 4,
            Wp: Optional[torch.Tensor] = None):
    N.require_gpu(tok_q)
    nq, L = tok_q.shape
    D = W.shape[1]
    nbytes = N.lib().snvrag_knn_lut_bytes(nq, n_sites_pad, limbs)
    lut = torch.empty(nbytes, device=tok_q.device, dtype=torch.int8)
    exps = torch.empty(nq, device=tok_q.device, dtype=torch.int32)
    consts = torch.empty(nq, device=tok_q.device, dtype=torch.float32)
    if Wp is not None and Wp is not W:
        assert Wp.shape == W.shape and Wp.dtype == torch.float32
        check(N.lib().snvrag_knn_lut_panel(nq, L, D, ptr(_c(tok_q)), ptr(_c(W)), ptr(_c(Wp)), ptr(Aq), aq_period,
                                           ptr(Ar), ptr(_c(site_mask)), n_sites, n_sites_pad, tok0, tok1, mask_tok,
                                           limbs, ptr(lut), ptr(exps), ptr(consts), stream_ptr()), "knn_lut_panel")
    else:
        check(N.lib().snvrag_knn_lut(nq, L, D, ptr(_c(tok_q)), ptr(_c(W)), ptr(Aq), aq_period, ptr(Ar),
                                     ptr(_c(site_mask)), n_sites, n_sites_pad, tok0, tok1, mask_tok, limbs,
                                     ptr(lut), ptr(exps), ptr(consts), stream_ptr()), "knn_lut")
    return lut, exps, consts


def knn_scan(codes: torch.Tensor, n_sites_pad: int, lut: torch.Tensor, nq: int, limbs: int, k: int,
             ref_offset: int = 0, n_parts: Optional[int] = None, th_init: Optional[torch.Tensor] = None) -> torch.Tensor:
    n_ref, ld = codes.shape
    if n_parts is None:
        n_parts = N.lib().snvrag_knn_scan_parts(n_ref, nq)
    parts = torch.empty(n_parts, nq, k, device=codes.device, dtype=torch.int64)
    if th_init is not None:
        assert th_init.dtype == torch.int32 and th_init.numel() == nq
    check(N.lib().snvrag_knn_scan(ptr(_c(codes)), n_ref, ld, n_sites_pad, ptr(lut), nq, limbs, k, ref_offset,
                                  ptr(parts), n_parts, ptr(th_init), stream_ptr()), "knn_scan")
    return parts


def knn_scan_bits(bits: torch.Tensor, n_sites_pad: int, lut: torch.Tensor, nq: int, limbs: int, k: int,
                  ref_offset: int = 0, n_parts: Optional[int] = None,
                  th_init: Optional[torch.Tensor] = None) -> torch.Tensor:
    assert bits.dtype == torch.uint8 and bits.dim() == 2
    n_ref, ldb = bits.shape
    if n_parts is None:
        n_parts = N.lib().snvrag_knn_scan_parts(n_ref, nq)
    parts = torch.empty(n_parts, nq, k, device=bits.device, dtype=torch.int64)
    if th_init is not None:
        assert th_init.dtype == torch.int32 and th_init.numel() == nq
    check(N.lib().snvrag_knn_scan_bits(ptr(_c(bits)), n_ref, ldb, n_sites_pad, ptr(lut), nq, limbs, k, ref_offset,
                                       ptr(parts), n_parts, ptr(th_init), stream_ptr()), "knn_scan_bits")
    return parts


def knn_threshold(keys: torch.Tensor, k: int) -> torch.Tensor:
    nq = keys.shape[0]
    th = torch.empty(nq, device=keys.device, dtype=torch.int32)
    check(N.lib().snvrag_knn_threshold(ptr(_c(keys)), nq, k, ptr(th), stream_ptr()), "knn_threshold")
    return th


def topk_merge(keys: torch.Tensor, k: int) -> torch.Tensor:
    n_lists, nq, kk = keys.shape
    assert kk == k
    out = torch.empty(nq, k, device=keys.device, dtype=torch.int64)
    wsb = N.lib().snvrag_topk_merge_ws_bytes(n_lists, nq, k)
    ws = torch.empty(wsb, device=keys.device, dtype=torch.uint8)
    check(N.lib().snvrag_topk_merge(ptr(_c(keys)), n_lists, nq, k, ptr(out), ptr(ws), wsb, stream_ptr()),
          "topk_merge")
    return out


def knn_decode(keys: torch.Tensor, exps: Optional[torch.Tensor] = None, consts: Optional[torch.Tensor] = None):
    nq, k = keys.shape
    idx = torch.empty(nq, k, device=keys.device, dtype=torch.int64)
    dist = torch.empty(nq, k, device=keys.device, dtype=torch.float32) if exps is not None else None
    check(N.lib().snvrag_knn_decode(ptr(_c(keys)), nq, k, ptr(exps), ptr(consts), ptr(idx), ptr(dist),
                                    stream_ptr()), "knn_decode")
    return idx, dist


def knn_emb_norms(E: torch.Tensor, chunk: int = 4096) -> torch.Tensor:
    out = torch.empty(E.shape[0], device=E.device, dtype=torch.float32)
    for i in range(0, E.shape[0], chunk):
        out[i:i + chunk] = E[i:i + chunk].float().pow(2).sum(1)
    return out


def knn_emb_pack(E: torch.Tensor, out: Optional[torch.Tensor] = None) -> torch.Tensor:
    assert E.dtype == torch.bfloat16 and E.dim() == 2
    n, kk = E.shape
    assert kk % 64 == 0
    rows = int(N.lib().snvrag_knn_emb_packed_bytes(n, kk)) // (2 * kk)
    if out is None:
        out = torch.empty(rows, kk, device=E.device, dtype=torch.bfloat16)
    assert out.dtype == torch.bfloat16 and out.is_contiguous() and out.numel() >= rows * kk
    check(N.lib().snvrag_knn_emb_pack(ptr(_c(E)), n, kk, ptr(out), stream_ptr()), "knn_emb_pack")
    return out


def knn_emb_dist(Et: torch.Tensor, Q: torch.Tensor, rn: torch.Tensor, qn: Optional[torch.Tensor] = None,
                 splits: Optional[int] = None) -> torch.Tensor:
    assert Et.dtype == torch.bfloat16 and Q.dtype == torch.bfloat16 and Et.shape[1] == Q.shape[1]
    n, kk = rn.shape[0], Et.shape[1]
    assert Et.shape[0] == (n + 31) // 32 * 32, "Et must be knn_emb_pack's output for len(rn) rows"
    bq = Q.shape[0]
    assert 0 < bq <= 128 and kk % 64 == 0
    if splits is None:
        splits = int(N.lib().snvrag_knn_emb_splits(n, kk, bq))
    if qn is None:
        qn = knn_emb_norms(Q)
    ws = torch.empty(int(N.lib().snvrag_knn_emb_ws_bytes(n, bq, splits)) // 4, device=Et.device, dtype=torch.float32)
    check(N.lib().snvrag_knn_emb_scan(ptr(_c(Et)), n, kk, ptr(_c(Q)), bq, splits, ptr(ws), stream_ptr()),
          "knn_emb_scan")
    dist = torch.empty(bq, n, device=Et.device, dtype=torch.float32)
    check(N.lib().snvrag_knn_emb_finish(ptr(ws), splits, bq, n, ptr(_c(qn.float())), ptr(_c(rn.float())), ptr(dist),
                                        stream_ptr()), "knn_emb_finish")
    return dist


def knn_emb_search(Et: torch.Tensor, Q: torch.Tensor, k: int, rn: torch.Tensor, qn: Optional[torch.Tensor] = None):
    d = knn_emb_dist(Et, Q, rn, qn)
    return torch.topk(d, k, dim=1, largest=False, sorted=True)


def rag_mean(idx: torch.Tensor, codes: torch.Tensor, n_sites: int, W: torch.Tensor, pe: torch.Tensor,
             Ar: Optional[torch.Tensor], L: int, dtype: torch.dtype, tok0=5, tok1=6, sos=2, eos=3, pad=0,
             out: Optional[torch.Tensor] = None, counts: Optional[torch.Tensor] = None, bits: bool = False):
    nq, k = idx.shape
    D = W.shape[1]
    if out is None:
        out = torch.empty(nq, L, D, device=idx.device, dtype=dtype)
    assert out.dtype == dtype and tuple(out.shape) == (nq, L, D) and out.is_contiguous()
    if counts is not None:
        assert counts.dtype == torch.uint8 and counts.shape[0] == nq
        check(N.lib().snvrag_rag_mean_counts(_dt(dtype), nq, L, D, k, ptr(_c(idx)), ptr(_c(counts)), counts.shape[1],
                                             n_sites, ptr(_c(W)), ptr(_c(pe)), ptr(Ar), tok0, tok1, sos, eos, pad,
                                             ptr(out), stream_ptr()), "rag_mean_counts")
        return out
    if bits:
        check(N.lib().snvrag_rag_mean_bits(_dt(dtype), nq, L, D, k, ptr(_c(idx)), ptr(_c(codes)), codes.shape[1],
                                           n_sites, ptr(_c(W)), ptr(_c(pe)), ptr(Ar), tok0, tok1, sos, eos, pad,
                                           ptr(out), stream_ptr()), "rag_mean_bits")
        return out
    check(N.lib().snvrag_rag_mean(_dt(dtype), nq, L, D, k, ptr(_c(idx)), ptr(_c(codes)), codes.shape[1], n_sites,
                                  ptr(_c(W)), ptr(_c(pe)), ptr(Ar), tok0, tok1, sos, eos, pad, ptr(out),
                                  stream_ptr()), "rag_mean")
    return out


def neighbor_counts(idx: torch.Tensor, codes: torch.Tensor, row0: int, ld_out: Optional[int] = None,
                    out: Optional[torch.Tensor] = None, bits: bool = False) -> torch.Tensor:
    nq, k = idx.shape
    n_rows, ld = codes.shape
    ld_out = ld_out or (8 * ld if bits else ld)
    if out is None:
        out = torch.empty(nq, ld_out, device=idx.device, dtype=torch.uint8)
    if bits:
        check(N.lib().snvrag_neighbor_counts_bits(nq, k, ptr(_c(idx)), ptr(_c(codes)), ld, row0, n_rows, ptr(out),
                                                  ld_out, stream_ptr()), "neighbor_counts_bits")
        return out
    check(N.lib().snvrag_neighbor_counts(nq, k, ptr(_c(idx)), ptr(_c(codes)), ld, row0, n_rows, ptr(out), ld_out,
                                         stream_ptr()), "neighbor_counts")
    return out


def hamming_topk(codes_wm: torch.Tensor, queries: torch.Tensor, k: int) -> torch.Tensor:
    nw, n = codes_wm.shape
    nq = queries.shape[0]
    assert queries.shape[1] == nw and codes_wm.dtype == torch.int32 and queries.dtype == torch.int32
    n_lists = int(N.lib().snvrag_hamming_list_count())
    lists = torch.empty(n_lists, nq, k, device=queries.device, dtype=torch.int64)
    check(N.lib().snvrag_hamming_lists(nq, n, nw, k, ptr(_c(codes_wm)), ptr(_c(queries)), ptr(lists),
                                       stream_ptr()), "hamming_lists")
    return topk_merge(lists, k)


def panel_synth(n_ref: int, n_sites: int, af: torch.Tensor, seed: int, ld: Optional[int] = None,
                row0: int = 0) -> torch.Tensor:
    N.require_gpu(af)
    ld = ld or max(256, ((n_sites + 255) // 256) * 256)
    codes = torch.empty(n_ref, ld, device=af.device, dtype=torch.uint8)
    check(N.lib().snvrag_panel_synth_rows(ptr(codes), row0, n_ref, ld, n_sites, ptr(_c(af)), seed, stream_ptr()),
          "panel_synth")
    return codes


def panel_synth_bits(n_ref: int, n_sites: int, af: torch.Tensor, seed: int, ld_bits: Optional[int] = None,
                     row0: int = 0) -> torch.Tensor:
    N.require_gpu(af)
    ld_bits = ld_bits or max(256, ((n_sites + 255) // 256) * 256) // 8
    bits = torch.empty(n_ref, ld_bits, device=af.device, dtype=torch.uint8)
    check(N.lib().snvrag_panel_synth_bits(ptr(bits), row0, n_ref, ld_bits, n_sites, ptr(_c(af)), seed, stream_ptr()),
          "panel_synth_bits")
    return bits


def panel_pack_bits(codes: torch.Tensor) -> torch.Tensor:
    N.require_gpu(codes)
    assert codes.dtype == torch.uint8 and codes.dim() == 2 and codes.shape[1] % 16 == 0
    n, ld = codes.shape
    bits = torch.empty(n, ld // 8, device=codes.device, dtype=torch.uint8)
    check(N.lib().snvrag_panel_pack_bits(ptr(_c(codes)), n, ld, ptr(bits), ld // 8, stream_ptr()), "panel_pack_bits")
    return bits


def panel_unpack_rows(bits: torch.Tensor, rows: torch.Tensor, ld_out: Optional[int] = None) -> torch.Tensor:
    N.require_gpu(bits, rows)
    assert bits.dtype == torch.uint8 and bits.dim() == 2 and rows.dtype == torch.int64 and rows.dim() == 1
    n_ref, ldb = bits.shape
    ld_out = ld_out or 8 * ldb
    out = torch.empty(rows.numel(), ld_out, device=bits.device, dtype=torch.uint8)
    check(N.lib().snvrag_panel_unpack_rows(ptr(_c(bits)), n_ref, ldb, ptr(_c(rows)), rows.numel(), ptr(out), ld_out,
                                           stream_ptr()), "panel_unpack_rows")
    return out


def encoder_forward(x: torch.Tensor, layers: Sequence["N.LayerW"], heads: int, ws: torch.Tensor) -> torch.Tensor:
    nseq, L, D = x.shape
    arr = (N.LayerW * len(layers))(*layers)
    check(N.lib().snvrag_encoder_forward(_dt(x.dtype), nseq, L, D, heads, len(layers), arr, ptr(_c(x)),
                                         ptr(ws), ws.numel(), stream_ptr()), "encoder_forward")
    return x


def encoder_ws_bytes(dtype: torch.dtype, nseq: int, L: int, D: int, heads: int) -> int:
    return int(N.lib().snvrag_encoder_ws_bytes(_dt(dtype), nseq, L, D, heads))


def selftest_mfma() -> int:
    return int(N.lib().snvrag_selftest_mfma(stream_ptr()))


def set_option(name: str, value: int) -> int:
    import ctypes
    prev = ctypes.c_int64()
    check(N.lib().snvrag_get_option(name.encode(), ctypes.byref(prev)), "get_option")
    check(N.lib().snvrag_set_option(name.encode(), int(value)), "set_option")
    return int(prev.value)


@contextlib.contextmanager
def option(name: str, value: int):
    prev = set_option(name, value)
    try:
        yield
    finally:
        set_option(name, prev)


_det_ws: dict = {}


def deterministic() -> bool:
    v = C.c_int64()
    check(N.lib().snvrag_get_option(b"deterministic", C.byref(v)), "get_option")
    return bool(v.value)


def _det_workspace(dev: torch.device, nbytes: int) -> torch.Tensor:
    key = (dev.index if dev.index is not None else torch.cuda.current_device(), stream_ptr())
    ws = _det_ws.get(key)
    if ws is None or ws.numel() < nbytes:
        ws = _det_ws[key] = torch.empty(max(int(nbytes), 16), device=dev, dtype=torch.uint8)
    return ws


def attention_train_fwd(qkv: torch.Tensor, nseq: int, L: int, heads: int, dh: int, dropout_p: float = 0.0,
                        seed: int = 0):
    N.require_gpu(qkv)
    assert qkv.dtype == torch.bfloat16
    D = heads * dh
    out = torch.empty(nseq * L, D, device=qkv.device, dtype=qkv.dtype)
    lse = torch.empty(nseq, heads, L, device=qkv.device, dtype=torch.float32)
    check(N.lib().snvrag_attention_train_fwd(nseq, L, heads, dh, ptr(_c(qkv)), qkv.shape[-1], ptr(out), D,
                                             ptr(lse), 1.0 / float(dh) ** 0.5, float(dropout_p), int(seed) & (2 ** 64 - 1),
                                             stream_ptr()), "attention_train_fwd")
    return out, lse


def attention_bwd(qkv: torch.Tensor, out: torch.Tensor, dout: torch.Tensor, lse: torch.Tensor, nseq: int, L: int,
                  heads: int, dh: int, dropout_p: float = 0.0, seed: int = 0) -> torch.Tensor:
    N.require_gpu(qkv, out, dout, lse)
    D = heads * dh
    dqkv = torch.empty(nseq * L, 3 * D, device=qkv.device, dtype=torch.bfloat16)
    ws = torch.empty(nseq * heads * L, device=qkv.device, dtype=torch.float32)
    check(N.lib().snvrag_attention_bwd(nseq, L, heads, dh, ptr(_c(qkv)), qkv.shape[-1], ptr(_c(out)), out.shape[-1],
                                       ptr(_c(dout)), dout.shape[-1], ptr(_c(lse)), ptr(ws), ptr(dqkv), 3 * D,
                                       1.0 / float(dh) ** 0.5, float(dropout_p), int(seed) & (2 ** 64 - 1),
                                       stream_ptr()), "attention_bwd")
    return dqkv


def focal_loss(probs: torch.Tensor, labels: torch.Tensor, mask: torch.Tensor, gamma: float, weight: float,
               loss_acc: Optional[torch.Tensor] = None):
    N.require_gpu(probs)
    Cc = probs.shape[-1]
    M = probs.numel() // Cc
    p = _c(probs.float().contiguous())
    lab = labels.reshape(-1).long().contiguous()
    msk = mask.reshape(-1).to(torch.uint8).contiguous()
    if loss_acc is None:
        loss_acc = torch.zeros(1, device=probs.device, dtype=torch.float32)
    grad = torch.empty_like(p)
    if deterministic():
        nb = int(N.lib().snvrag_focal_loss_det_ws_bytes(M))
        ws = _det_workspace(p.device, nb)
        check(N.lib().snvrag_focal_loss_det(M, Cc, ptr(p), ptr(lab), ptr(msk), float(gamma), float(weight),
                                            ptr(loss_acc), ptr(grad), ptr(ws), ws.numel(), stream_ptr()),
              "focal_loss_det")
        return loss_acc, grad
    check(N.lib().snvrag_focal_loss(M, Cc, ptr(p), ptr(lab), ptr(msk), float(gamma), float(weight), ptr(loss_acc),
                                    ptr(grad), stream_ptr()), "focal_loss")
    return loss_acc, grad


def sqnorm(x: torch.Tensor, acc: Optional[torch.Tensor] = None, ws: Optional[torch.Tensor] = None) -> torch.Tensor:
    N.require_gpu(x)
    assert x.dtype == torch.float32
    if acc is None:
        acc = torch.empty(1, device=x.device, dtype=torch.float32)
    nb = int(N.lib().snvrag_sqnorm_ws_bytes())
    if ws is None or ws.numel() * ws.element_size() < nb:
        ws = torch.empty(nb // 4, device=x.device, dtype=torch.float32)
    check(N.lib().snvrag_sqnorm_ws(x.numel(), ptr(_c(x)), ptr(acc), ptr(ws), ws.numel() * ws.element_size(),
                                   stream_ptr()), "sqnorm")
    return acc


def adam_step(p: torch.Tensor, g: torch.Tensor, m: torch.Tensor, v: torch.Tensor, *, lr: float, betas=(0.9, 0.999),
              eps: float = 1e-8, weight_decay: float = 0.0, step: int, grad_scale: float = 1.0,
              max_norm: float = 0.0, sq: Optional[torch.Tensor] = None, p_bf16: Optional[torch.Tensor] = None):
    N.require_gpu(p, g, m, v)
    a = N.AdamS(lr, betas[0], betas[1], eps, weight_decay, grad_scale, max_norm, step)
    check(N.lib().snvrag_adam_step(p.numel(), ptr(_c(p)), ptr(_c(g)), ptr(_c(m)), ptr(_c(v)), ptr(p_bf16), ptr(sq),
                                   C.byref(a), stream_ptr()), "adam_step")


def confusion(probs: torch.Tensor, labels: torch.Tensor, mask: torch.Tensor, counts: torch.Tensor,
              mask2: Optional[torch.Tensor] = None) -> torch.Tensor:
    N.require_gpu(probs)
    Cc = probs.shape[-1]
    M = probs.numel() // Cc
    p = probs.float().contiguous()
    m2 = mask2.reshape(-1).to(torch.uint8).contiguous() if mask2 is not None else None
    check(N.lib().snvrag_confusion(M, Cc, ptr(p), ptr(labels.reshape(-1).long().contiguous()),
                                   ptr(mask.reshape(-1).to(torch.uint8).contiguous()), ptr(m2), ptr(_c(counts)),
                                   stream_ptr()), "confusion")
    return counts


def infer_post(probs_h1: torch.Tensor, probs_h2: torch.Tensor):
    N.require_gpu(probs_h1, probs_h2)
    a, b = probs_h1.float().contiguous(), probs_h2.float().contiguous()
    M = a.numel() // 2
    p1 = torch.empty(a.shape[:-1], device=a.device, dtype=torch.float32)
    p2 = torch.empty_like(p1)
    gt = torch.empty(*a.shape[:-1], 4, device=a.device, dtype=torch.float32)
    check(N.lib().snvrag_infer_post(M, ptr(a), ptr(b), ptr(p1), ptr(p2), ptr(gt), stream_ptr()), "infer_post")
    return p1, p2, gt


def _rows_host(rows_host: torch.Tensor, B: int) -> int:
    assert not rows_host.is_cuda and rows_host.dtype == torch.int32 and rows_host.is_contiguous() and \
        rows_host.numel() >= 3 * B
    return int(rows_host.data_ptr())


def infer_scatter(probs_h1: torch.Tensor, probs_h2: torch.Tensor, mask: torch.Tensor, rows_dev: torch.Tensor,
                  rows_host: torch.Tensor, window_len: int, hap1: torch.Tensor, hap2: torch.Tensor, gp: torch.Tensor,
                  mask_out: torch.Tensor) -> None:
    N.require_gpu(probs_h1, probs_h2, mask, rows_dev, hap1, hap2, gp, mask_out)
    B, L = mask.shape
    assert probs_h1.shape == (B, L, 2) and probs_h2.shape == (B, L, 2) and mask.dtype == torch.int64
    assert probs_h1.dtype == torch.float32 and probs_h2.dtype == torch.float32
    assert rows_dev.dtype == torch.int32 and rows_dev.numel() >= 3 * B
    n_variants, S = hap1.shape
    assert hap2.shape == (n_variants, S) and gp.shape == (n_variants, S, 4) and mask_out.shape == (n_variants, S)
    assert hap1.dtype == hap2.dtype == gp.dtype == torch.float32 and mask_out.dtype == torch.int64
    check(N.lib().snvrag_infer_scatter(B, L, ptr(_c(probs_h1)), ptr(_c(probs_h2)), ptr(_c(mask)), ptr(_c(rows_dev)),
                                       _rows_host(rows_host, B), window_len, n_variants, S, ptr(_c(hap1)),
                                       ptr(_c(hap2)), ptr(_c(gp)), ptr(_c(mask_out)), stream_ptr()), "infer_scatter")


def batch_features(tables: "N.FeatureTables", rows_dev: torch.Tensor, rows_host: torch.Tensor, B: int, L: int,
                   token_ids: Sequence[int], labels: bool = False):
    N.require_gpu(rows_dev)
    assert rows_dev.dtype == torch.int32 and rows_dev.is_contiguous() and rows_dev.numel() >= 3 * B
    dev = rows_dev.device
    tokens = torch.empty(2 * B, L, device=dev, dtype=torch.int64)
    mask = torch.empty(B, L, device=dev, dtype=torch.int64)
    floats = torch.empty(6, B, L, device=dev, dtype=torch.float32)
    lab = torch.empty(3, B, L, device=dev, dtype=torch.int64) if labels else None
    sos, eos, pad, msk, tok0, tok1 = (int(v) for v in token_ids)
    check(N.lib().snvrag_batch_features(C.byref(tables), ptr(rows_dev), _rows_host(rows_host, B), B, L, sos, eos, pad,
                                        msk, tok0, tok1, ptr(tokens), ptr(mask), ptr(floats), ptr(lab), stream_ptr()),
          "batch_features")
    return tokens, mask, floats, lab


def vcf_format(h1: torch.Tensor, h2: torch.Tensor, gt: torch.Tensor, rows: torch.Tensor, line_off: torch.Tensor,
               prefix_off: torch.Tensor, prefix_blob: torch.Tensor, out: torch.Tensor, out_bytes: int,
               bad_count: torch.Tensor) -> None:
    N.require_gpu(h1, h2, gt, rows, line_off, prefix_off, prefix_blob, out, bad_count)
    n, S = h1.shape
    n_lines = rows.numel()
    assert h2.shape == (n, S) and gt.shape == (n, S, 4)
    assert h1.dtype == h2.dtype == gt.dtype == torch.float32
    assert h1.is_contiguous() and h2.is_contiguous() and gt.is_contiguous()
    assert rows.dtype == torch.int32 and prefix_off.dtype == torch.int32 and line_off.dtype == torch.int64
    assert rows.is_contiguous() and line_off.is_contiguous() and prefix_off.is_contiguous()
    assert line_off.numel() == n_lines + 1 and prefix_off.numel() == n_lines + 1
    assert prefix_blob.dtype == torch.uint8 and out.dtype == torch.uint8 and bad_count.dtype == torch.int32
    assert prefix_blob.is_contiguous() and out.is_contiguous() and 0 <= out_bytes <= out.numel()
    check(N.lib().snvrag_vcf_format(n, S, ptr(h1), ptr(h2), ptr(gt), n_lines, ptr(rows), ptr(line_off),
                                    ptr(prefix_off), ptr(prefix_blob), prefix_blob.numel(), ptr(out), out_bytes,
                                    ptr(bad_count), stream_ptr()), "vcf_format")


def site_stats(h1: torch.Tensor, h2: torch.Tensor, gt: torch.Tensor, truth: Optional[torch.Tensor] = None,
               truth_row: Optional[torch.Tensor] = None, truth_col: Optional[torch.Tensor] = None,
               bad_count: Optional[torch.Tensor] = None):
    N.require_gpu(h1, h2, gt, truth, truth_row, truth_col, bad_count)
    n, S = h1.shape
    assert h2.shape == (n, S) and gt.shape == (n, S, 4)
    assert h1.dtype == h2.dtype == gt.dtype == torch.float32
    assert h1.is_contiguous() and h2.is_contiguous() and gt.is_contiguous()
    dev = h1.device
    est = torch.empty(n, 5, device=dev, dtype=torch.float64)
    acc = table = None
    n_truth = S_truth = 0
    if truth is not None:
        assert truth_row is not None and truth_col is not None, "truth needs truth_row and truth_col"
        assert truth.dtype == torch.int8 and truth.dim() == 3 and truth.shape[2] == 2 and truth.is_contiguous()
        assert truth_row.dtype == truth_col.dtype == torch.int32
        assert truth_row.is_contiguous() and truth_col.is_contiguous()
        assert truth_row.numel() == n and truth_col.numel() == S
        n_truth, S_truth = truth.shape[:2]
        acc = torch.empty(n, 3, device=dev, dtype=torch.float64)
        table = torch.empty(n, 9, device=dev, dtype=torch.int32)
        if bad_count is None:
            bad_count = torch.zeros(1, device=dev, dtype=torch.int32)
        assert bad_count.dtype == torch.int32 and bad_count.numel() >= 1
    check(N.lib().snvrag_site_stats(n, S, ptr(h1), ptr(h2), ptr(gt), ptr(truth), n_truth, S_truth, ptr(truth_row),
                                    ptr(truth_col), ptr(est), ptr(acc), ptr(table), ptr(bad_count), stream_ptr()),
          "site_stats")
    return est, acc, table


def _text_ok(text: torch.Tensor, nbytes: int) -> None:
    assert text.dtype == torch.uint8 and text.dim() == 1 and text.is_contiguous()
    assert 1 <= nbytes and (nbytes + 15) // 16 * 16 <= text.numel(), "the text buffer must hold the '\\n' padding"


def vcf_line_index(text: torch.Tensor, nbytes: int, max_lines: int):
    N.require_gpu(text)
    _text_ok(text, nbytes)
    dev = text.device
    line_off = torch.empty(max_lines + 1, device=dev, dtype=torch.int64)
    n_lines = torch.empty(1, device=dev, dtype=torch.int64)
    nws = N.lib().snvrag_vcf_line_index_ws_bytes(nbytes)
    ws = torch.empty(nws, device=dev, dtype=torch.uint8)
    check(N.lib().snvrag_vcf_line_index(ptr(text), nbytes, max_lines, ptr(line_off), ptr(n_lines), ptr(ws), nws,
                                        stream_ptr()), "vcf_line_index")
    return line_off, n_lines


def vcf_parse_gt(text: torch.Tensor, nbytes: int, line_off: torch.Tensor, n_lines: int, S: int, codes: torch.Tensor,
                 force_general: bool = False):
    N.require_gpu(text, line_off, codes)
    _text_ok(text, nbytes)
    assert line_off.dtype == torch.int64 and line_off.is_contiguous() and line_off.numel() >= n_lines
    assert codes.dtype == torch.uint8 and codes.dim() == 2 and codes.is_contiguous()
    assert codes.shape[0] >= n_lines and codes.shape[1] >= S and codes.shape[1] % 4 == 0
    dev = text.device
    pos = torch.empty(n_lines, device=dev, dtype=torch.int32)
    flags = torch.empty(n_lines, device=dev, dtype=torch.int32)
    nws = N.lib().snvrag_vcf_parse_ws_bytes(n_lines, S)
    ws = torch.empty(nws, device=dev, dtype=torch.uint8)
    check(N.lib().snvrag_vcf_parse_gt(ptr(text), nbytes, ptr(line_off), n_lines, S, int(bool(force_general)), ptr(pos),
                                      ptr(flags), ptr(codes), codes.shape[1], ptr(ws), nws, stream_ptr()),
          "vcf_parse_gt")
    return pos, flags


def vcf_pack_rows(codes: torch.Tensor, n_lines: int, S: int, alt_bits: torch.Tensor, miss_bits: torch.Tensor,
                  site0: int = 0) -> None:
    N.require_gpu(codes, alt_bits, miss_bits)
    assert codes.dtype == torch.uint8 and codes.dim() == 2 and codes.is_contiguous() and codes.shape[0] >= n_lines
    for b in (alt_bits, miss_bits):
        assert b.dtype == torch.uint8 and b.is_contiguous() and b.shape == (2 * S, alt_bits.shape[1])
    check(N.lib().snvrag_vcf_pack_rows(ptr(codes), codes.shape[1], n_lines, S, site0, ptr(alt_bits), ptr(miss_bits),
                                       alt_bits.shape[1], stream_ptr()), "vcf_pack_rows")


def panel_gather_bits(bits: torch.Tensor, n_src_sites: int, site_idx: torch.Tensor, n_sites_pad: int,
                      packed: bool) -> torch.Tensor:
    N.require_gpu(bits, site_idx)
    assert bits.dtype == torch.uint8 and bits.dim() == 2 and bits.is_contiguous()
    assert site_idx.dtype == torch.int32 and site_idx.dim() == 1 and site_idx.is_contiguous()
    out = torch.empty(bits.shape[0], n_sites_pad // 8 if packed else n_sites_pad, device=bits.device,
                      dtype=torch.uint8)
    check(N.lib().snvrag_panel_gather_bits(ptr(bits), bits.shape[0], bits.shape[1], n_src_sites, ptr(site_idx),
                                           site_idx.numel(), n_sites_pad, int(bool(packed)), ptr(out), stream_ptr()),
          "panel_gather_bits")
    return out


def vcf_unpack_gt(alt_bits: torch.Tensor, miss_bits: torch.Tensor, n_sites: int) -> torch.Tensor:
    N.require_gpu(alt_bits, miss_bits)
    assert alt_bits.dtype == miss_bits.dtype == torch.uint8 and alt_bits.shape == miss_bits.shape
    assert alt_bits.dim() == 2 and alt_bits.is_contiguous() and miss_bits.is_contiguous() and alt_bits.shape[0] % 2 == 0
    S = alt_bits.shape[0] // 2
    gt = torch.empty(n_sites, S, 2, device=alt_bits.device, dtype=torch.int8)
    check(N.lib().snvrag_vcf_unpack_gt(ptr(alt_bits), ptr(miss_bits), alt_bits.shape[1], S, n_sites, ptr(gt),
                                       stream_ptr()), "vcf_unpack_gt")
    return gt


def bgzf_table(in_off, out_off, in_len, isize, crc, out: Optional[torch.Tensor] = None) -> torch.Tensor:
    import numpy as np
    n = len(in_off)
    t = np.empty((n, 4), np.int64)
    t[:, 0], t[:, 1] = in_off, out_off
    t[:, 2] = np.asarray(in_len, np.int64) & 0xffffffff | np.asarray(isize, np.int64) << 32
    t[:, 3] = np.asarray(crc, np.int64) & 0xffffffff
    if out is None:
        return torch.from_numpy(t)
    assert out.dtype == torch.int64 and out.is_contiguous() and out.shape[0] >= n and out.shape[1:] == (4,)
    out.numpy()[:n] = t
    return out[:n]


def bgzf_inflate(comp: torch.Tensor, table: torch.Tensor, text: torch.Tensor, status: Optional[torch.Tensor] = None,
# ... 484 lines not shown
```

### rag-snvbert_amd/src/native.py

```python

from __future__ import annotations

import ctypes as C
import os
from pathlib import Path
from typing import Optional

import torch

PKG_DIR = Path(__file__).resolve().parents[1]
LIB_PATH = Path(os.environ.get("SNVRAG_LIB", PKG_DIR / "lib" / "libsnvrag.so"))

F32, BF16 = 0, 1
ACT_NONE, ACT_GELU, ACT_LRELU, ACT_SIGMOID = 0, 1, 2, 3
ABI_VERSION = 31

vp, i64, i32, f32, sz = C.c_void_p, C.c_int64, C.c_int32, C.c_float, C.c_size_t


class DeriveJob(C.Structure):
    _fields_ = [("kind", i32), ("nparts", i32), ("rows", i64), ("cols", i64), ("dst_ld", i64),
                ("piece0", i64), ("pieces", i64), ("part_rows", i64 * 4), ("rs", i64 * 4), ("cs", i64 * 4),
                ("src", vp * 4), ("dst", vp)]


class Epilogue(C.Structure):
    _fields_ = [("bias", vp), ("row1", vp), ("row1_stride", i64), ("col1", vp),
                ("row2", vp), ("row2_stride", i64), ("col2", vp), ("row_period", i64),
                ("act", C.c_int), ("slope", f32), ("resid", vp), ("ld_resid", i64),
                ("ln_g", vp), ("ln_b", vp), ("ln_eps", f32), ("ln_act", C.c_int),
                ("post_base", vp), ("ld_post", i64), ("post_scale", f32),
                ("post_af", vp), ("post_af_period", i64), ("post_maf", C.c_int),
                ("stats_out", vp)]


class RowNormS(C.Structure):
    _fields_ = [("stats", vp), ("n_parts", C.c_int), ("dim", i64), ("eps", f32), ("c1", vp)]


class LnPost(C.Structure):
    _fields_ = [("base", vp), ("ld_base", i64), ("scale", f32), ("af", vp),
                ("af_period", i64), ("maf_weight", C.c_int), ("act", C.c_int)]


class PosfeatW(C.Structure):
    _fields_ = [(n, vp) for n in ("c1_w", "c1_b", "c2_w", "c2_b", "c3_w", "c3_b",
                                  "bn1_w", "bn1_b", "bn1_rm", "bn1_rv",
                                  "bn2_w", "bn2_b", "bn2_rm", "bn2_rv")] + [("bn_eps", f32)]


class AfGateW(C.Structure):
    _fields_ = [(n, vp) for n in ("g1_w", "g1_b", "g2_w", "g2_b", "j_w", "j_b", "ln_w", "ln_b")] + \
               [("res_scale", f32)]


class GtW(C.Structure):
    _fields_ = [(n, vp) for n in ("f_w", "f_b", "n_w", "n_b", "w1", "b1", "ln_w", "ln_b",
                                  "w2", "b2", "c_w", "c_b")]


class AdamS(C.Structure):
    _fields_ = [("lr", f32), ("beta1", f32), ("beta2", f32), ("eps", f32), ("weight_decay", f32),
                ("grad_scale", f32), ("max_norm", f32), ("step", C.c_int)]


class FeatureTables(C.Structure):
    _fields_ = [(n, vp) for n in ("gt_bits", "win_off", "site_row", "freq_col", "pos_norm", "win_mask", "freq",
                                  "pop_of_sample")] + \
               [("ld_bits", i64), ("n_cols", i64), ("n_samples", i32), ("n_windows", i32), ("max_window_sites", i32),
                ("n_pop", i32), ("global_row", i32)]


class LayerW(C.Structure):
    _fields_ = [(n, vp) for n in ("w_qkv", "b_qkv", "w_o", "b_o", "ln1_g", "ln1_b", "w1", "b1",
                                  "lnf_g", "lnf_b", "w2", "b2", "ln2_g", "ln2_b", "w2g", "b2g", "c2g")] + [("q_scale", f32)] + \
        [("ffn_v", vp), ("tail_w", vp), ("qkv_pw", vp), ("qkv_sg", vp)]


_SIGS = {
    "snvrag_abi_version": ([], C.c_int),
    "snvrag_last_error": ([], C.c_char_p),
    "snvrag_device_info": ([C.c_int, C.c_char_p, C.c_int], C.c_int),
    "snvrag_set_option": ([C.c_char_p, i64], C.c_int),
    "snvrag_get_option": ([C.c_char_p, C.POINTER(i64)], C.c_int),
    "snvrag_linear": ([C.c_int, C.c_int, i64, i64, i64, vp, i64, vp, i64, vp, i64, C.POINTER(Epilogue), vp], C.c_int),
    "snvrag_linear_ex": ([C.c_int, C.c_int, i64, i64, i64, vp, i64, vp, i64, vp, i64, C.POINTER(Epilogue),
                          C.POINTER(RowNormS), vp], C.c_int),
    "snvrag_layernorm": ([C.c_int, C.c_int, i64, i64, vp, i64, vp, i64, vp, vp, f32, vp, i64,
                          C.POINTER(LnPost), vp], C.c_int),
    "snvrag_attention": ([C.c_int, i64, i64, C.c_int, C.c_int, vp, i64, vp, i64, f32, vp], C.c_int),
    "snvrag_attention_fallbacks": ([C.c_int], C.c_int),
    "snvrag_af_features": ([C.c_int, i64, vp, vp, C.c_int, vp, vp], C.c_int),
    "snvrag_embed_tokens": ([C.c_int, i64, i64, i64, vp, vp, i64, vp, vp, C.c_int, i64, vp, vp], C.c_int),
    "snvrag_posfeat": ([i64, i64, vp, C.POINTER(PosfeatW), vp, vp], C.c_int),
    "snvrag_af_gate": ([C.c_int, i64, i64, vp, vp, C.POINTER(AfGateW), vp, vp], C.c_int),
    "snvrag_rag_weighted_concat": ([C.c_int, i64, i64, vp, vp, vp, i64, vp, vp], C.c_int),
    "snvrag_hap_head_out": ([C.c_int, i64, i64, vp, i64, vp, vp, vp, vp, vp], C.c_int),
    "snvrag_gt_head": ([i64, vp, vp, vp, vp, vp, i64, C.POINTER(GtW), vp, vp], C.c_int),
    "snvrag_knn_lut_bytes": ([i64, i32, C.c_int], sz),
    "snvrag_knn_lut": ([i64, i64, i64, vp, vp, vp, i64, vp, vp, i32, i32, C.c_int, C.c_int, C.c_int,
                        C.c_int, vp, vp, vp, vp], C.c_int),
    "snvrag_knn_lut_panel": ([i64, i64, i64, vp, vp, vp, vp, i64, vp, vp, i32, i32, C.c_int, C.c_int, C.c_int,
                              C.c_int, vp, vp, vp, vp], C.c_int),
    "snvrag_knn_scan_parts": ([i64, i32], C.c_int),
    "snvrag_knn_scan": ([vp, i64, i64, i32, vp, i32, C.c_int, C.c_int, i64, vp, i32, vp, vp], C.c_int),
    "snvrag_knn_threshold": ([vp, i32, C.c_int, vp, vp], C.c_int),
    "snvrag_topk_merge_ws_bytes": ([i32, i32, C.c_int], sz),
    "snvrag_topk_merge": ([vp, i32, i32, C.c_int, vp, vp, sz, vp], C.c_int),
    "snvrag_knn_decode": ([vp, i32, C.c_int, vp, vp, vp, vp, vp], C.c_int),
    "snvrag_knn_emb_splits": ([i64, i64, C.c_int], C.c_int),
    "snvrag_knn_emb_ws_bytes": ([i64, C.c_int, C.c_int], sz),
    "snvrag_knn_emb_packed_bytes": ([i64, i64], sz),
    "snvrag_knn_emb_pack": ([vp, i64, i64, vp, vp], C.c_int),
    "snvrag_knn_emb_scan": ([vp, i64, i64, vp, C.c_int, C.c_int, vp, vp], C.c_int),
    "snvrag_knn_emb_finish": ([vp, C.c_int, C.c_int, i64, vp, vp, vp, vp], C.c_int),
    "snvrag_rag_mean": ([C.c_int, i64, i64, i64, C.c_int, vp, vp, i64, i32, vp, vp, vp, C.c_int, C.c_int,
                         C.c_int, C.c_int, C.c_int, vp, vp], C.c_int),
    "snvrag_panel_synth": ([vp, i64, i64, i32, vp, C.c_uint64, vp], C.c_int),
    "snvrag_hamming_lists": ([i64, i64, i32, C.c_int, vp, vp, vp, vp], C.c_int),
    "snvrag_hamming_list_count": ([], i32),
    "snvrag_panel_synth_rows": ([vp, i64, i64, i64, i32, vp, C.c_uint64, vp], C.c_int),
    "snvrag_neighbor_counts": ([i64, C.c_int, vp, vp, i64, i64, i64, vp, i64, vp], C.c_int),
    "snvrag_rag_mean_counts": ([C.c_int, i64, i64, i64, C.c_int, vp, vp, i64, i32, vp, vp, vp, C.c_int, C.c_int,
                                C.c_int, C.c_int, C.c_int, vp, vp], C.c_int),
    "snvrag_panel_pack_bits": ([vp, i64, i64, vp, i64, vp], C.c_int),
    "snvrag_panel_synth_bits": ([vp, i64, i64, i64, i32, vp, C.c_uint64, vp], C.c_int),
    "snvrag_panel_unpack_rows": ([vp, i64, i64, vp, i64, vp, i64, vp], C.c_int),
    "snvrag_knn_scan_bits": ([vp, i64, i64, i32, vp, i32, C.c_int, C.c_int, i64, vp, i32, vp, vp], C.c_int),
    "snvrag_rag_mean_bits": ([C.c_int, i64, i64, i64, C.c_int, vp, vp, i64, i32, vp, vp, vp, C.c_int, C.c_int,
                              C.c_int, C.c_int, C.c_int, vp, vp], C.c_int),
    "snvrag_neighbor_counts_bits": ([i64, C.c_int, vp, vp, i64, i64, i64, vp, i64, vp], C.c_int),
    "snvrag_encoder_ws_bytes": ([C.c_int, i64, i64, C.c_int, C.c_int], sz),
    "snvrag_encoder_forward": ([C.c_int, i64, i64, C.c_int, C.c_int, C.c_int, C.POINTER(LayerW), vp, vp, sz, vp],
                               C.c_int),
    "snvrag_proj_pack_bytes": ([C.c_int, C.c_int], sz),
    "snvrag_proj_pack": ([C.c_int, C.c_int, vp, vp, vp], C.c_int),
    "snvrag_proj_forward": ([i64, C.c_int, C.c_int, vp, vp, vp, vp, vp], C.c_int),
    "snvrag_tail_pack_bytes": ([C.c_int], sz),
    "snvrag_tail_pack": ([C.c_int, vp, vp, vp, vp, vp], C.c_int),
    "snvrag_tail_forward": ([i64, C.c_int, vp, vp, vp, vp, vp, vp, vp, f32, vp], C.c_int),
    "snvrag_tail_qkv_forward": ([i64, C.c_int, vp, vp, vp, vp, vp, vp, vp, f32, vp, vp, vp, vp], C.c_int),
    "snvrag_tail_ffn_forward": ([i64, C.c_int, vp, vp, vp, vp, f32, vp], C.c_int),
    "snvrag_tail_stamps": ([vp], C.c_int),
    "snvrag_attention_train_fwd": ([i64, i64, C.c_int, C.c_int, vp, i64, vp, i64, vp, f32, f32, C.c_uint64, vp],
                                   C.c_int),
    "snvrag_attention_bwd": ([i64, i64, C.c_int, C.c_int, vp, i64, vp, i64, vp, i64, vp, vp, vp, i64, f32, f32,
                              C.c_uint64, vp], C.c_int),
    "snvrag_focal_loss": ([i64, C.c_int, vp, vp, vp, f32, f32, vp, vp, vp], C.c_int),
    "snvrag_sqnorm": ([i64, vp, vp, vp], C.c_int),
    "snvrag_sqnorm_ws_bytes": ([], sz),
    "snvrag_sqnorm_ws": ([i64, vp, vp, vp, sz, vp], C.c_int),
    "snvrag_adam_step": ([i64, vp, vp, vp, vp, vp, vp, C.POINTER(AdamS), vp], C.c_int),
    "snvrag_confusion": ([i64, C.c_int, vp, vp, vp, vp, vp, vp], C.c_int),
    "snvrag_infer_post": ([i64, vp, vp, vp, vp, vp, vp], C.c_int),
    "snvrag_infer_scatter": ([i64, i32, vp, vp, vp, vp, vp, i32, i64, i64, vp, vp, vp, vp, vp], C.c_int),
    "snvrag_batch_features": ([C.POINTER(FeatureTables), vp, vp, i64, i32, C.c_int, C.c_int, C.c_int, C.c_int,
                               C.c_int, C.c_int, vp, vp, vp, vp, vp], C.c_int),
    "snvrag_vcf_format": ([i64, i64, vp, vp, vp, i64, vp, vp, vp, vp, i64, vp, i64, vp, vp], C.c_int),
    "snvrag_site_stats": ([i64, i64, vp, vp, vp, vp, i64, i64, vp, vp, vp, vp, vp, vp, vp], C.c_int),
    "snvrag_vcf_line_index_ws_bytes": ([i64], sz),
    "snvrag_vcf_line_index": ([vp, i64, i64, vp, vp, vp, sz, vp], C.c_int),
    "snvrag_vcf_parse_ws_bytes": ([i64, i64], sz),
    "snvrag_vcf_parse_gt": ([vp, i64, vp, i64, i64, C.c_int, vp, vp, vp, i64, vp, sz, vp], C.c_int),
    "snvrag_vcf_pack_rows": ([vp, i64, i64, i64, i64, vp, vp, i64, vp], C.c_int),
    "snvrag_panel_gather_bits": ([vp, i64, i64, i64, vp, i64, i64, C.c_int, vp, vp], C.c_int),
    "snvrag_vcf_unpack_gt": ([vp, vp, i64, i64, i64, vp, vp], C.c_int),
    "snvrag_bgzf_inflate": ([vp, i64, vp, vp, i64, vp, i64, vp, vp], C.c_int),
    "snvrag_text_last_newline": ([vp, i64, vp, vp], C.c_int),
    "snvrag_bgzf_deflate": ([vp, i64, i64, vp, vp, vp], C.c_int),
    "snvrag_bgzf_pack": ([vp, vp, i64, vp, i64, vp, vp], C.c_int),
    "snvrag_mlp_pack_bytes": ([C.c_int], sz),
    "snvrag_mlp_pack": ([C.c_int, vp, vp, vp, vp], C.c_int),
    "snvrag_mlp_forward": ([i64, C.c_int, C.c_int, vp, vp, vp, vp, vp, i64, f32, vp, vp], C.c_int),
    "snvrag_mlp_afgate_forward": ([i64, C.c_int, vp, vp, vp, f32, vp, vp, vp, vp], C.c_int),
    "snvrag_sgemm_cat_forward": ([i64, C.c_int, C.c_int, vp, vp, vp, i64, vp, vp, vp, vp], C.c_int),
    "snvrag_sgemm_pack_bytes": ([C.c_int, C.c_int], sz),
    "snvrag_sgemm_pack": ([C.c_int, C.c_int, vp, vp, vp], C.c_int),
    "snvrag_derive": ([vp, C.c_int, i64, vp], C.c_int),
    "snvrag_gemm256_pack_bytes": ([C.c_int, C.c_int], sz),
    "snvrag_gemm256_pack": ([C.c_int, C.c_int, vp, i64, vp, vp], C.c_int),
    "snvrag_gemm256_forward": ([i64, C.c_int, C.c_int, vp, i64, vp, vp, vp, i64, vp, i64, vp], C.c_int),
    "snvrag_gemm256_ln_forward": ([i64, C.c_int, C.c_int, vp, i64, vp, vp, vp, vp, f32, vp, i64, f32,
                                   vp, i64, vp, i64, vp], C.c_int),
    "snvrag_head2_fwd": ([i64, C.c_int, vp, vp, vp, vp, vp], C.c_int),
    "snvrag_head2_ws_bytes": ([i64, C.c_int], sz),
    "snvrag_tokgrad_ws_bytes": ([i64, C.c_int, C.c_int], sz),
    "snvrag_tokgrad": ([i64, C.c_int, C.c_int, C.c_int, vp, vp, vp, vp, sz, vp], C.c_int),
    "snvrag_head2_bwd": ([i64, C.c_int, vp, vp, vp, vp, vp, C.c_int, vp, sz, vp], C.c_int),
    "snvrag_sgemm_forward": ([i64, C.c_int, C.c_int, C.c_int, C.c_int, f32, vp, vp, vp, vp, vp, i64, f32, vp, vp, vp,
                              vp], C.c_int),
    "snvrag_ln_fwd_train": ([i64, C.c_int, vp, vp, vp, vp, f32, vp, vp, vp, f32, f32, C.c_uint64, vp], C.c_int),
    "snvrag_nbr_mean_drop_fwd": ([i64, C.c_int, i64, C.c_int, C.c_int, i64, C.c_int, vp, vp, vp, vp, vp, f32,
                                  C.c_uint64, C.c_int, C.c_int, C.c_int, C.c_int, vp, vp], C.c_int),
    "snvrag_nbr_mean_drop_bwd": ([i64, C.c_int, i64, C.c_int, C.c_int, i64, C.c_int, vp, vp, vp, vp, vp, f32,
                                  C.c_uint64, C.c_int, C.c_int, C.c_int, C.c_int, vp, vp, vp, vp], C.c_int),
    "snvrag_ln_fwd_train_act": ([i64, C.c_int, vp, vp, vp, vp, f32, vp, vp, vp, f32, f32, C.c_uint64, f32, f32, vp],
                                C.c_int),
    "snvrag_ln_bwd_act": ([i64, C.c_int, vp, vp, vp, vp, vp, vp, vp, vp, vp, C.c_int, f32, f32, C.c_uint64, f32, f32,
                           vp, sz, vp], C.c_int),
    "snvrag_ln_bwd_ws_bytes": ([i64, C.c_int], sz),
    "snvrag_ln_bwd": ([i64, C.c_int, vp, vp, vp, vp, vp, vp, vp, vp, C.c_int, f32, f32, C.c_uint64, vp, sz, vp],
                      C.c_int),
    "snvrag_colsum_ws_bytes": ([i64, C.c_int], sz),
    "snvrag_colsum_bf16": ([i64, C.c_int, vp, vp, vp, sz, vp], C.c_int),
    "snvrag_dw_splits": ([i64, i64, i64], C.c_int),
    "snvrag_linear_dw": ([i64, i64, i64, vp, i64, vp, i64, vp, vp, C.c_int, vp], C.c_int),
    "snvrag_linear_dw_parts": ([i64, i64, i64, vp, i64, vp, i64, C.c_int, C.POINTER(vp), C.POINTER(vp), C.c_int, vp],
                               C.c_int),
    "snvrag_linear_dw_det_ws_bytes": ([i64, i64, i64, C.c_int], sz),
    "snvrag_linear_dw_det": ([i64, i64, i64, vp, i64, vp, i64, vp, vp, C.c_int, vp, sz, vp], C.c_int),
    "snvrag_linear_dw_parts_det": ([i64, i64, i64, vp, i64, vp, i64, C.c_int, C.POINTER(vp), C.POINTER(vp), C.c_int,
                                    vp, sz, vp], C.c_int),
    "snvrag_nbr_mean_drop_bwd_det_ws_bytes": ([i64, C.c_int, C.c_int], sz),
    "snvrag_nbr_mean_drop_bwd_det": ([i64, C.c_int, i64, C.c_int, C.c_int, i64, C.c_int, vp, vp, vp, vp, vp, f32,
                                      C.c_uint64, C.c_int, C.c_int, C.c_int, C.c_int, vp, vp, vp, vp, sz, vp], C.c_int),
    "snvrag_focal_loss_det_ws_bytes": ([i64], sz),
    "snvrag_focal_loss_det": ([i64, C.c_int, vp, vp, vp, f32, f32, vp, vp, vp, sz, vp], C.c_int),
    "snvrag_evlog_enable": ([C.c_int], C.c_int),
    "snvrag_evlog_pause": ([C.c_int], C.c_int),
    "snvrag_evlog_reset": ([], C.c_int),
    "snvrag_evlog_read": ([vp, vp, vp, C.c_int], C.c_int),
    "snvrag_selftest_mfma": ([vp], C.c_int),
}

EXPORTED = tuple(_SIGS)
_lib: Optional[C.CDLL] = None


class NativeUnavailable(RuntimeError):
    pass


def load(path: Path | str | None = None) -> C.CDLL:
    global _lib
    if _lib is not None and path is None:
        return _lib
    p = Path(path) if path is not None else LIB_PATH
    if not p.exists():
        raise NativeUnavailable(f"{p} not found — build it with `make -C {PKG_DIR}` "
                                "(there is no CPU fallback for the hot path)")
    lib = C.CDLL(str(p))
    for name, (args, res) in _SIGS.items():
        fn = getattr(lib, name)
        fn.argtypes, fn.restype = args, res
    if lib.snvrag_abi_version() != ABI_VERSION:
        raise NativeUnavailable(f"ABI mismatch: lib {lib.snvrag_abi_version()} != {ABI_VERSION}")
    if path is None:
        _lib = lib
    return lib


def lib() -> C.CDLL:
    return load()


def check(rc: int, what: str = "snvrag") -> None:
    if rc != 0:
        msg = lib().snvrag_last_error().decode(errors="replace")
        raise RuntimeError(f"{what} failed ({rc}): {msg}")


def require_gpu(*tensors: torch.Tensor) -> None:
    if not torch.cuda.is_available():
        raise NativeUnavailable("no HIP device: the SNV-RAG hot path runs only on the GPU (no CPU fallback)")
    for t in tensors:
        if t is not None and not t.is_cuda:
            raise ValueError("expected device tensors (got a CPU tensor)")


def stream_ptr(stream: Optional[torch.cuda.Stream] = None) -> int:
    s = stream if stream is not None else torch.cuda.current_stream()
    return int(s.cuda_stream)


def ptr(t: Optional[torch.Tensor]) -> Optional[int]:
    return None if t is None else int(t.data_ptr())


def dtype_code(dt: torch.dtype) -> int:
    if dt == torch.float32:
        return F32
    if dt == torch.bfloat16:
        return BF16
    raise ValueError(f"unsupported dtype {dt}")
```

Baseline: 8.206 million.

## Fuse RAG-fusion MLP, LayerNorm residual, and layer-0 QKV projection into one kernel

Adds a ragfuse kernel that forms the gated concat of h and h_rag*aw in LDS, then runs the W0 GEMM with GELU and the W3 GEMM, bias, LayerNorm, MAF-weighted residual and optional layer-0 QKV projection in one pass, with weights streamed through a register ring. The aim is to remove the separate sgemm_cat, gemm256 tail and first QKV linear launches, along with their intermediate round trips through HBM. The encoder gains an entry point that skips the layer-0 QKV GEMM when the fused kernel has already written it. The kernel is hard-coded to D=384, uses one wave per EU and large LDS, and the QKV shortcut is limited to single-chunk bf16 runs.

```diff
diff --git a/include/snvrag.h b/include/snvrag.h
--- a/include/snvrag.h
+++ b/include/snvrag.h
@@ -250,6 +250,18 @@
 int snvrag_encoder_forward(int dtype, int64_t nseq, int64_t L, int D, int heads, int n_layers,
                            const snvrag_layer_t* layers, void* x, void* ws, size_t ws_bytes,
                            void* stream);
+int64_t snvrag_encoder_chunk_seqs(int dtype, int64_t nseq, int64_t L, int D);
+int snvrag_encoder_forward_qkv0(int dtype, int64_t nseq, int64_t L, int D, int heads, int n_layers,
+                                const snvrag_layer_t* layers, void* x, void* ws, size_t ws_bytes,
+                                int qkv0_ready, void* stream);
+
+size_t snvrag_ragfuse_pack_bytes(int D);
+int snvrag_ragfuse_pack(int D, const void* w0, const void* w3, void* out, void* stream);
+int snvrag_ragfuse_forward(int64_t M, int D, const void* h, const void* h_rag, const void* aw, int64_t period,
+                           const void* wstream, const float* b0, const float* b3, const float* ln_g,
+                           const float* ln_b, float eps, float post_scale, const float* post_af,
+                           int64_t post_af_period, void* out, const void* qkv_pw, const float* b_qkv,
+                           void* qkv_out, void* stream);
 
 int snvrag_evlog_enable(int capacity);
 int snvrag_evlog_pause(int paused);
diff --git a/rag-snvbert_amd/csrc/common.h b/rag-snvbert_amd/csrc/common.h
--- a/rag-snvbert_amd/csrc/common.h
+++ b/rag-snvbert_amd/csrc/common.h
@@ -51,6 +51,7 @@
   int64_t proj_wide;
   int64_t tail_wide;
   int64_t tail_qkv;
+  int64_t rag_fuse;
   int64_t deterministic;
 };
 Options& options();
diff --git a/rag-snvbert_amd/csrc/engine.hip b/rag-snvbert_amd/csrc/engine.hip
--- a/rag-snvbert_amd/csrc/engine.hip
+++ b/rag-snvbert_amd/csrc/engine.hip
@@ -26,14 +26,17 @@
   return M * (size_t)D * 9 * esz + M * 64 * 8 + 8192;
 }
 
-extern "C" int snvrag_encoder_forward(int dtype, int64_t nseq, int64_t L, int D, int heads, int n_layers,
-                                      const snvrag_layer_t* layers, void* x, void* ws, size_t ws_bytes,
-                                      void* stream) {
-  SNV_CHECK_PTRS(layers, x, ws);
-  SNV_CHECK_ARG(D % heads == 0, "D % heads");
-  SNV_CHECK_ARG(ws_bytes >= snvrag_encoder_ws_bytes(dtype, nseq, L, D, heads), "encoder workspace too small");
+namespace snvrag {
+static int encoder_forward(const char* where, int dtype, int64_t nseq, int64_t L, int D, int heads, int n_layers,
+                           const snvrag_layer_t* layers, void* x, void* ws, size_t ws_bytes, bool qkv0_ready,
+                           void* stream) {
+  SNV_CHECK_AS(where, non_null(layers, x, ws), "null pointer");
+  SNV_CHECK_AS(where, D % heads == 0, "D % heads");
+  SNV_CHECK_AS(where, ws_bytes >= snvrag_encoder_ws_bytes(dtype, nseq, L, D, heads), "encoder workspace too small");
   const int esz = dtype == SNVRAG_BF16 ? 2 : 4;
   const int64_t cs = chunk_seqs(nseq, L, D, esz);
+  SNV_CHECK_AS(where, !qkv0_ready || (cs >= nseq && dtype == SNVRAG_BF16 && n_layers > 0),
+               "layer 0's qkv can be passed in only for a one-chunk bf16 forward");
   const size_t Mc = (size_t)cs * L;
   char* w = (char*)ws;
   auto carve = [&](size_t elems) { char* p = w; w += ((elems * esz + 255) / 256) * 256; return (void*)p; };
@@ -54,7 +57,7 @@
     const int64_t ns = std::min<int64_t>(cs, nseq - s0);
     const int64_t M = ns * L;
     char* xc = (char*)x + (size_t)s0 * L * D * esz;
-    bool have_qkv = false;
+    bool have_qkv = qkv0_ready;
     for (int i = 0; i < n_layers; ++i) {
       const snvrag_layer_t& ly = layers[i];
       snvrag_epilogue_t e{};
@@ -70,6 +73,7 @@
       else
         rc = snvrag_linear(dtype, dtype, M, 3 * D, D, xc, D, ly.w_qkv, D, qkv, 3 * D, &e, stream);
       if (rc) return rc;
+      have_qkv = false;
       const float sc = ly.q_scale > 0.f ? scale / ly.q_scale : scale;
       rc = snvrag_attention(dtype, ns, L, heads, dh, qkv, 3 * D, att, D, sc, stream);
       if (rc) return rc;
@@ -125,3 +129,21 @@
   }
   return 0;
 }
+}
+
+extern "C" int snvrag_encoder_forward(int dtype, int64_t nseq, int64_t L, int D, int heads, int n_layers,
+                                      const snvrag_layer_t* layers, void* x, void* ws, size_t ws_bytes,
+                                      void* stream) {
+  return encoder_forward(__func__, dtype, nseq, L, D, heads, n_layers, layers, x, ws, ws_bytes, false, stream);
+}
+
+extern "C" int64_t snvrag_encoder_chunk_seqs(int dtype, int64_t nseq, int64_t L, int D) {
+  return chunk_seqs(nseq, L, D, dtype == SNVRAG_BF16 ? 2 : 4);
+}
+
+extern "C" int snvrag_encoder_forward_qkv0(int dtype, int64_t nseq, int64_t L, int D, int heads, int n_layers,
+                                           const snvrag_layer_t* layers, void* x, void* ws, size_t ws_bytes,
+                                           int qkv0_ready, void* stream) {
+  return encoder_forward(__func__, dtype, nseq, L, D, heads, n_layers, layers, x, ws, ws_bytes, qkv0_ready != 0,
+                         stream);
+}
diff --git a/rag-snvbert_amd/csrc/misc.hip b/rag-snvbert_amd/csrc/misc.hip
--- a/rag-snvbert_amd/csrc/misc.hip
+++ b/rag-snvbert_amd/csrc/misc.hip
@@ -99,6 +99,7 @@
     {"proj_wide", &Options::proj_wide, 1},         {"g2_variant", &Options::g2_variant, 0},
     {"g2_groups", &Options::g2_groups, 0},         {"tail_split", &Options::tail_split, 64},
     {"deterministic", &Options::deterministic, 0}, {"tail_qkv", &Options::tail_qkv, 1},
+    {"rag_fuse", &Options::rag_fuse, 1},
 };
 Options make_options() {
   Options o{};
diff --git a/rag-snvbert_amd/csrc/ragfuse.hip b/rag-snvbert_amd/csrc/ragfuse.hip
--- /dev/null
+++ b/rag-snvbert_amd/csrc/ragfuse.hip
@@ -0,0 +1,364 @@
+#include "common.h"
+#include "mfma32.h"
+#include "tailw_shared.h"
+
+namespace snvrag {
+
+constexpr int RF_D = 384, RF_G = 2, RF_ROWS = 32 * RF_G;
+constexpr int RF_KS1 = 48;
+constexpr int RF_NH = 12;
+constexpr int RF_FPB = RF_KS1 + 24;
+constexpr int RF_NFRAG = RF_NH * 4 * RF_FPB;
+constexpr int RF_RING = 24, RF_AH = 18;
+static_assert(RF_KS1 % RF_RING == 0 && RF_FPB % RF_RING == 0, "ring registers periodic over the sections");
+constexpr int RF_X = TW_X;
+constexpr int RF_H = 96 * 1024;
+constexpr int RF_T0 = 128 * 1024;
+constexpr int RF_T1 = RF_T0 + 4 * RF_D * 4;
+constexpr int RF_T2 = RF_T1 + 3 * RF_D * 4;
+constexpr int RF_T3 = RF_T2 + 3 * RF_D * 4;
+constexpr int RF_LDS = RF_T3 + 4 * RF_G * 32 * 4;
+static_assert(RF_LDS <= 160 * 1024, "LDS budget");
+
+struct RfArgs {
+  int M;
+  const bf16* h;
+  const bf16* hr;
+  const bf16* aw;
+  int period;
+  const char* ws;
+  const float* b0;
+  const float* b3; const float* ln_g; const float* ln_b;
+  float eps, post_scale;
+  const float* af; int af_period;
+  bf16* out;
+  const char* pw;
+  const float* pbias;
+  bf16* qkv;
+};
+
+__global__ __launch_bounds__(256) __attribute__((amdgpu_waves_per_eu(1, 1)))
+void ragfuse_kernel(RfArgs p) {
+  constexpr int D = RF_D, G = RF_G;
+  extern __shared__ __attribute__((aligned(16))) char smem[];
+  const int wave = __builtin_amdgcn_readfirstlane(threadIdx.x >> 6);
+  const long row0 = (long)blockIdx.x * RF_ROWS;
+  const int M = p.M;
+  const int lane = threadIdx.x & 63, n = lane & 31, hh = lane >> 5;
+  const int lane16 = lane * 16;
+  const uint32_t lds0 = lds_addr(smem);
+
+  const __amdgpu_buffer_rsrc_t wrb =
+      __builtin_amdgcn_make_buffer_rsrc((void*)p.ws, (short)0, RF_NFRAG * FRAG_BYTES, 0x00020000);
+  u32x4 wf[RF_RING];
+  auto loadW = [&](u32x4& r, int h, int q) {
+    r = __builtin_amdgcn_raw_buffer_load_b128(wrb, lane16, ((4 * h + wave) * RF_FPB + q) * FRAG_BYTES, 0);
+  };
+  unroll([&](auto nc) { loadW(wf[decltype(nc)::value], 0, decltype(nc)::value); },
+         std::make_integer_sequence<int, RF_AH>{});
+
+  {
+    float* t0 = reinterpret_cast<float*>(smem + RF_T0);
+    for (int i = threadIdx.x; i < 4 * D; i += 256) t0[i] = p.b0[i];
+    float* t1 = reinterpret_cast<float*>(smem + RF_T1);
+    for (int i = threadIdx.x; i < D; i += 256) {
+      t1[i] = p.b3[i];
+      t1[D + i] = p.ln_g[i];
+      t1[2 * D + i] = p.ln_b[i];
+    }
+    if (p.pw) {
+      float* t2 = reinterpret_cast<float*>(smem + RF_T2);
+      for (int i = threadIdx.x; i < 3 * D; i += 256) t2[i] = p.pbias[i];
+    }
+    const int g = wave & 1;
+    long r = row0 + 32 * g + n;
+    r = r < M ? r : (long)M - 1;
+    const long rg = r % p.period;
+#pragma unroll
+    for (int j = 0; j < 12; ++j) {
+      const int s = (wave >> 1) + 2 * j;
+      const u32x4 v = *reinterpret_cast<const u32x4*>(p.h + r * D + in_feat(s, hh, 0));
+      *reinterpret_cast<u32x4*>(smem + RF_X + (s * G + g) * FRAG_BYTES + lane16) = v;
+    }
+#pragma unroll
+    for (int j = 0; j < 12; ++j) {
+      const int s = (wave >> 1) + 2 * j;
+      const int f = in_feat(s, hh, 0);
+      const u32x4 a = *reinterpret_cast<const u32x4*>(p.hr + r * D + f);
+      const u32x4 b = *reinterpret_cast<const u32x4*>(p.aw + rg * D + f);
+      u32x4 v;
+#pragma unroll
+      for (int w = 0; w < 4; ++w)
+        v[w] = pack2(bf_lo(a[w]) * bf_lo(b[w]), bf_hi(a[w]) * bf_hi(b[w]));
+      *reinterpret_cast<u32x4*>(smem + RF_X + ((24 + s) * G + g) * FRAG_BYTES + lane16) = v;
+    }
+  }
+  __syncthreads();
+
+  auto rdX = [&](int s, int g) -> u32x4 {
+    return *reinterpret_cast<const u32x4*>(smem + RF_X + (s * G + g) * FRAG_BYTES + lane16);
+  };
+  auto rdH = [&](int par, int u, int g) -> u32x4 {
+    return *reinterpret_cast<const u32x4*>(smem + RF_H + par * 16384 + (u * G + g) * FRAG_BYTES + lane16);
+  };
+  auto issue = [&](auto q_tag, int h, auto first_tag) {
+    constexpr int q = decltype(q_tag)::value + RF_AH;
+    constexpr bool FIRST = decltype(first_tag)::value;
+    constexpr int LEN = FIRST ? RF_KS1 : RF_FPB;
+    if constexpr (q < RF_KS1) loadW(wf[q % RF_RING], h, q);
+    else if constexpr (q < LEN) loadW(wf[q % RF_RING], h - 1, q);
+    else if constexpr (q - LEN < RF_KS1) {
+      if (h + 1 < RF_NH) loadW(wf[q % RF_RING], h + 1, q - LEN);
+      else if (q - LEN < 24) loadW(wf[q % RF_RING], h, RF_KS1 + q - LEN);
+    }
+  };
+
+  f32x16 acc[3][G];
+#pragma unroll
+  for (int t = 0; t < 3; ++t)
+#pragma unroll
+    for (int g = 0; g < G; ++g) acc[t][g] = f32x16{};
+  f32x16 hva[G], hvb[G];
+
+  auto gemm1 = [&](int h, f32x16 (&hc)[G], const f32x16 (&hp)[G], auto epi_tag, auto first_tag) {
+    constexpr bool EPI = decltype(epi_tag)::value;
+    u32x4 bq[4][G];
+#pragma unroll
+    for (int s = 0; s < 3; ++s)
+#pragma unroll
+      for (int g = 0; g < G; ++g) bq[s][g] = rdX(s, g);
+    float ex[8];
+    const float* b0t = reinterpret_cast<const float*>(smem + RF_T0) + 32 * (4 * (EPI ? h - 1 : 0) + wave) + 16 * hh;
+    unroll([&](auto ic) {
+      constexpr int i = decltype(ic)::value;
+#pragma unroll
+      for (int g = 0; g < G; ++g) {
+        if constexpr (i == 0) hc[g] = mfma32(wf[i % RF_RING], bq[i & 3][g], f32x16{});
+        else hc[g] = mfma32(wf[i % RF_RING], bq[i & 3][g], hc[g]);
+      }
+      if constexpr (i + 3 < RF_KS1) {
+#pragma unroll
+        for (int g = 0; g < G; ++g) bq[(i + 3) & 3][g] = rdX(i + 3, g);
+      }
+      issue(ic, h, first_tag);
+      if constexpr (EPI) {
+        constexpr int k = i / 12, r = i % 12, g = k >> 1, j = k & 1;
+        if constexpr (r < 8) ex[r] = gelu_bf16(hp[g][8 * j + r] + b0t[8 * j + r]);
+        if constexpr (r == 8)
+          *reinterpret_cast<u32x4*>(smem + RF_H + ((h - 1) & 1) * 16384 + ((wave * 2 + j) * G + g) * FRAG_BYTES + lane16) =
+              u32x4{pack2(ex[0], ex[1]), pack2(ex[2], ex[3]), pack2(ex[4], ex[5]), pack2(ex[6], ex[7])};
+      }
+      __builtin_amdgcn_sched_barrier(0);
+    }, std::make_integer_sequence<int, RF_KS1>{});
+  };
+  auto gemm2 = [&](int h2, auto final_tag) {
+    constexpr bool FINAL = decltype(final_tag)::value;
+    const int par = h2 & 1;
+    u32x4 bq[3][G];
+#pragma unroll
+    for (int u = 0; u < 2; ++u)
+#pragma unroll
+      for (int g = 0; g < G; ++g) bq[u][g] = rdH(par, u, g);
+    unroll([&](auto uc) {
+      constexpr int u = decltype(uc)::value;
+#pragma unroll
+      for (int g = 0; g < G; ++g)
+#pragma unroll
+        for (int t = 0; t < 3; ++t) acc[t][g] = mfma32(wf[(3 * u + t) % RF_RING], bq[u % 3][g], acc[t][g]);
+      if constexpr (u + 2 < 8) {
+#pragma unroll
+        for (int g = 0; g < G; ++g) bq[(u + 2) % 3][g] = rdH(par, u + 2, g);
+      }
+      unroll([&](auto tc) {
+        constexpr int q = 3 * u + decltype(tc)::value;
+        if constexpr (FINAL) {
+          if constexpr (q + RF_AH < 24) loadW(wf[(q + RF_AH) % RF_RING], h2, RF_KS1 + q + RF_AH);
+        } else {
+          issue(std::integral_constant<int, RF_KS1 + q>{}, h2 + 1, std::false_type{});
+        }
+      }, std::make_integer_sequence<int, 3>{});
+      __builtin_amdgcn_sched_barrier(0);
+    }, std::make_integer_sequence<int, 8>{});
+  };
+
+  gemm1(0, hva, hvb, std::false_type{}, std::true_type{});
+#pragma unroll 1
+  for (int h = 1; h < RF_NH - 1; h += 2) {
+    gemm1(h, hvb, hva, std::true_type{}, std::false_type{});
+    __syncthreads();
+    gemm2(h - 1, std::false_type{});
+    gemm1(h + 1, hva, hvb, std::true_type{}, std::false_type{});
+    __syncthreads();
+    gemm2(h, std::false_type{});
+  }
+  gemm1(RF_NH - 1, hvb, hva, std::true_type{}, std::false_type{});
+  __syncthreads();
+  gemm2(RF_NH - 2, std::false_type{});
+  {
+    const float* b0t = reinterpret_cast<const float*>(smem + RF_T0) + 32 * (4 * (RF_NH - 1) + wave) + 16 * hh;
+#pragma unroll
+    for (int g = 0; g < G; ++g)
+#pragma unroll
+      for (int j = 0; j < 2; ++j) {
+        float ex[8];
+#pragma unroll
+        for (int r = 0; r < 8; ++r) ex[r] = gelu_bf16(hvb[g][8 * j + r] + b0t[8 * j + r]);
+        *reinterpret_cast<u32x4*>(smem + RF_H + 16384 + ((wave * 2 + j) * G + g) * FRAG_BYTES + lane16) =
+            u32x4{pack2(ex[0], ex[1]), pack2(ex[2], ex[3]), pack2(ex[4], ex[5]), pack2(ex[6], ex[7])};
+      }
+  }
+  __syncthreads();
+  gemm2(RF_NH - 1, std::true_type{});
+
+  u32x4 base[3][G][2];
+#pragma unroll
+  for (int t = 0; t < 3; ++t)
+#pragma unroll
+    for (int g = 0; g < G; ++g)
+#pragma unroll
+      for (int h2 = 0; h2 < 2; ++h2) base[t][g][h2] = rdX(2 * (3 * wave + t) + h2, g);
+  const float* sb = reinterpret_cast<const float*>(smem + RF_T1);
+  float* red = reinterpret_cast<float*>(smem + RF_T3);
+  auto row_sum = [&](float (&s)[G]) {
+#pragma unroll
+    for (int g = 0; g < G; ++g) {
+      s[g] += __shfl_xor(s[g], 32, 64);
+      if (hh == 0) red[(wave * G + g) * 32 + n] = s[g];
+    }
+    __syncthreads();
+#pragma unroll
+    for (int g = 0; g < G; ++g)
+      s[g] = ((red[g * 32 + n] + red[(G + g) * 32 + n]) + red[(2 * G + g) * 32 + n]) + red[(3 * G + g) * 32 + n];
+    __syncthreads();
+  };
+  float mean[G], rstd[G];
+#pragma unroll
+  for (int g = 0; g < G; ++g) mean[g] = 0.f;
+#pragma unroll
+  for (int t = 0; t < 3; ++t) {
+    const float* bv = sb + 96 * wave + 32 * t + 16 * hh;
+#pragma unroll
+    for (int g = 0; g < G; ++g)
+#pragma unroll
+      for (int i = 0; i < 16; ++i) mean[g] += acc[t][g][i] + bv[i];
+  }
+  row_sum(mean);
+#pragma unroll
+  for (int g = 0; g < G; ++g) {
+    mean[g] *= 1.0f / D;
+    rstd[g] = 0.f;
+  }
+#pragma unroll
+  for (int t = 0; t < 3; ++t) {
+    const float* bv = sb + 96 * wave + 32 * t + 16 * hh;
+#pragma unroll
+    for (int g = 0; g < G; ++g)
+#pragma unroll
+      for (int i = 0; i < 16; ++i) {
+        const float d = acc[t][g][i] + bv[i] - mean[g];
+        rstd[g] = fmaf(d, d, rstd[g]);
+      }
+  }
+  row_sum(rstd);
+  float w[G];
+#pragma unroll
+  for (int g = 0; g < G; ++g) {
+    rstd[g] = 1.0f / sqrtf(rstd[g] * (1.0f / D) + p.eps);
+    long m = row0 + 32 * g + n;
+    m = m < M ? m : (long)M - 1;
+    w[g] = maf_w(p.af[m % p.af_period]);
+  }
+  const bool proj = p.pw != nullptr;
+#pragma unroll
+  for (int t = 0; t < 3; ++t)
+#pragma unroll
+    for (int h2 = 0; h2 < 2; ++h2) {
+      const int T = 3 * wave + t;
+      const int f0 = 32 * T + 16 * hh + 8 * h2;
+#pragma unroll
+      for (int g = 0; g < G; ++g) {
+        const long r = row0 + 32 * g + n;
+        float y[8];
+#pragma unroll
+        for (int i = 0; i < 8; ++i)
+          y[i] = fmaf((acc[t][g][8 * h2 + i] + sb[f0 + i] - mean[g]) * rstd[g], sb[D + f0 + i], sb[2 * D + f0 + i]);
+        const u32x4 b = base[t][g][h2];
+#pragma unroll
+        for (int e = 0; e < 4; ++e) {
+          y[2 * e] = bf_lo(b[e]) + p.post_scale * (y[2 * e] * w[g]);
+          y[2 * e + 1] = bf_hi(b[e]) + p.post_scale * (y[2 * e + 1] * w[g]);
+        }
+        u32x4 v{pack2(y[0], y[1]), pack2(y[2], y[3]), pack2(y[4], y[5]), pack2(y[6], y[7])};
+        if (r < M) *reinterpret_cast<u32x4*>(p.out + r * D + f0) = v;
+        else v = u32x4{0u, 0u, 0u, 0u};
+        if (proj) *reinterpret_cast<u32x4*>(smem + TW_X + ((2 * T + h2) * 4 + g) * FRAG_BYTES + lane16) = v;
+      }
+    }
+  if (!proj) return;
+
+  const __amdgpu_buffer_rsrc_t pwb =
+      __builtin_amdgcn_make_buffer_rsrc((void*)p.pw, (short)0, 3 * TW_FPRE * FRAG_BYTES, 0x00020000);
+  u32x4 pf[TW_RING];
+#pragma unroll
+  for (int i = 0; i < TW_AH; ++i) pw_loadW(pf[i], pwb, lane16, wave, 3, 0, i);
+  __syncthreads();
+  f32x16 pacc[3][4];
+  pw_chunks<G, true>(smem, lds0 + RF_T2, wave, lane16, pwb, 3, pw_out_rsrc(p.qkv, M, row0, 3), pf, pacc);
+}
+
+__global__ void ragfuse_pack_kernel(const bf16* __restrict__ w0, const bf16* __restrict__ w3, bf16* __restrict__ out) {
+  const long pc = (long)blockIdx.x * blockDim.x + threadIdx.x;
+  if (pc >= (long)RF_NFRAG * 64) return;
+  const int l = (int)(pc % 64), m = l & 31, kh = l >> 5;
+  const int F = (int)(pc / 64), q = F % RF_FPB, hw = F / RF_FPB, h = hw >> 2, w = hw & 3;
+  const bf16* src;
+  if (q < RF_KS1) {
+    src = w0 + (long)(32 * (4 * h + w) + out_feat(m)) * (2 * RF_D) + in_feat(q, kh, 0);
+  } else {
+    const int u = (q - RF_KS1) / 3, t = (q - RF_KS1) % 3;
+    src = w3 + (long)out_feat(3 * w + t, m) * (4 * RF_D) + 32 * (4 * h + (u >> 1)) + 16 * kh + 8 * (u & 1);
+  }
+  for (int j = 0; j < 8; ++j) out[pc * 8 + j] = src[j];
+}
+
+}
+
+using namespace snvrag;
+
+extern "C" size_t snvrag_ragfuse_pack_bytes(int D) { return D == RF_D ? (size_t)RF_NFRAG * FRAG_BYTES : 0; }
+
+extern "C" int snvrag_ragfuse_pack(int D, const void* w0, const void* w3, void* out, void* stream) {
+  SNV_CHECK_ARG(D == RF_D, "the rag fusion kernel needs D = 384");
+  SNV_CHECK_ARG(w0 && w3 && out, "null pointer");
+  const long pieces = (long)RF_NFRAG * 64;
+  hipLaunchKernelGGL(ragfuse_pack_kernel, dim3((unsigned)cdiv(pieces, 256)), dim3(256), 0, as_stream(stream),
+                     (const bf16*)w0, (const bf16*)w3, (bf16*)out);
+  SNV_LAUNCH_CHECK();
+  return 0;
+}
+
+extern "C" int snvrag_ragfuse_forward(int64_t M, int D, const void* h, const void* h_rag, const void* aw,
+                                      int64_t period, const void* wstream, const float* b0, const float* b3,
+                                      const float* ln_g, const float* ln_b, float eps, float post_scale,
+                                      const float* post_af, int64_t post_af_period, void* out, const void* qkv_pw,
+                                      const float* b_qkv, void* qkv_out, void* stream) {
+  SNV_CHECK_ARG(D == RF_D, "the rag fusion kernel needs D = 384");
+  SNV_CHECK_ARG(h && h_rag && aw && wstream && b0 && b3 && ln_g && ln_b && post_af && out, "null pointer");
+  SNV_CHECK_ARG(!qkv_pw || (b_qkv && qkv_out), "the QKV phase needs its bias and output");
+  SNV_CHECK_ARG(M >= 0, "bad M");
+  SNV_CHECK_ARG(M < (1L << 31), "bad M");
+  SNV_CHECK_ARG(period > 0 && period < (1L << 31) && post_af_period > 0 && post_af_period < (1L << 31), "bad period");
+  SNV_CHECK_ARG(!qkv_pw || M * 3 * D * 2 < (1L << 31), "QKV output of 2 GiB or more");
+  const void* ps[] = {h, h_rag, aw, wstream, out, qkv_pw, qkv_out};
+  for (const void* q : ps) SNV_CHECK_ARG(((uintptr_t)q & 15) == 0, "pointers must be 16-byte aligned");
+  if (M == 0) return 0;
+  const RfArgs a{(int)M, (const bf16*)h, (const bf16*)h_rag, (const bf16*)aw, (int)period, (const char*)wstream, b0,
+                 b3, ln_g, ln_b, eps, post_scale, post_af, (int)post_af_period, (bf16*)out, (const char*)qkv_pw, b_qkv,
+                 (bf16*)qkv_out};
+  hipStream_t s = as_stream(stream);
+  evlog_begin(s);
+  const int rc = SNV_LAUNCH_LDS(ragfuse_kernel, dim3((unsigned)cdiv(M, RF_ROWS)), dim3(256), RF_LDS, s, a);
+  if (rc) return rc;
+  evlog_end(s, EV_GEMM, 2.0 * M * ((double)2 * D * 4 * D + (double)4 * D * D + (qkv_pw ? (double)D * 3 * D : 0.0)));
+  return 0;
+}
diff --git a/rag-snvbert_amd/csrc/tailw.hip b/rag-snvbert_amd/csrc/tailw.hip
--- a/rag-snvbert_amd/csrc/tailw.hip
+++ b/rag-snvbert_amd/csrc/tailw.hip
@@ -1,5 +1,6 @@
 #include "common.h"
 #include "mfma32.h"
+#include "tailw_shared.h"
 
 namespace snvrag {
 
@@ -7,15 +8,6 @@
 #define TW_PACKED_LN 1
 #endif
 
-constexpr int TW_D = 384, TW_NT = 12, TW_KS = 24;
-constexpr int TW_FPRE = TW_NT * TW_KS;
-constexpr int TW_FPC = 96;
-constexpr int TW_NFRAG = TW_FPRE + 24 * TW_FPC;
-constexpr int TW_X = 0;
-constexpr int TW_H = 96 * 1024;
-constexpr int TW_LDS = 160 * 1024;
-constexpr int TW_AH = 9;
-constexpr int TW_RING = 12;
 constexpr int TW_QA = 24;
 constexpr int TW_Q0 = 48;
 constexpr int TW_HS = 32;
@@ -84,12 +76,6 @@
 #ifndef TW_NOPMASK
 #define TW_NOPMASK 2
 #endif
-__device__ __forceinline__ void tw_drain_o(f32x16 (&a)[3][4]) {
-  asm volatile("s_nop 7\n\ts_nop 7\n\ts_nop 7"
-               : "+a"(a[0][0]), "+a"(a[0][1]), "+a"(a[0][2]), "+a"(a[0][3]), "+a"(a[1][0]), "+a"(a[1][1]),
-                 "+a"(a[1][2]), "+a"(a[1][3]), "+a"(a[2][0]), "+a"(a[2][1]), "+a"(a[2][2]), "+a"(a[2][3])
-               :: "memory");
-}
 template <bool AGPR> __device__ __forceinline__ void tw_drain_h4(f32x16 (&h)[4]) {
   if constexpr (AGPR)
     asm volatile("s_nop 7\n\ts_nop 7\n\ts_nop 7" : "+a"(h[0]), "+a"(h[1]), "+a"(h[2]), "+a"(h[3]) :: "memory");
@@ -125,7 +111,6 @@
 template <int OFF> __device__ __forceinline__ void tw_load_off(u32x4& r, int voff, const i32x4& rsrc, int so) {
   asm volatile("buffer_load_dwordx4 %0, %1, %2, %3 offen offset:%4" : "=v"(r) : "v"(voff), "s"(rsrc), "s"(so), "n"(OFF) : "memory");
 }
-__device__ __forceinline__ void tw_barrier() { asm volatile("s_waitcnt lgkmcnt(0)\n\ts_barrier" ::: "memory"); }
 
 struct TwArgs {
   int M;
@@ -144,72 +129,6 @@
   bf16* qkv_out;
 };
 
-__device__ __forceinline__ void pw_loadW(u32x4& r, const __amdgpu_buffer_rsrc_t wrb, int lane16, int wave, int NC, int c,
-                                         int n72) {
-  const int cc = c < NC ? c : NC - 1;
-  r = __builtin_amdgcn_raw_buffer_load_b128(wrb, lane16, (cc * TW_FPRE + (n72 / 3) * TW_NT + 3 * wave + n72 % 3) * FRAG_BYTES, 0);
-}
-template <int G, bool NOP>
-__device__ __forceinline__ void pw_chunks(const char* smem, uint32_t bias_lds, int wave, int lane16,
-                                          const __amdgpu_buffer_rsrc_t wrb, int NC, const __amdgpu_buffer_rsrc_t ors,
-                                          u32x4 (&wf)[TW_RING], f32x16 (&acc)[3][4]) {
-  constexpr int D = TW_D, KS = TW_KS, GI = G > 1 ? 1 : 0;
-  auto rdB = [&](int blk) -> u32x4 { return *reinterpret_cast<const u32x4*>(smem + TW_X + blk * FRAG_BYTES + lane16); };
-  u32x4 bq[2][4];
-#pragma unroll 1
-  for (int c = 0; c < NC; ++c) {
-#pragma unroll
-    for (int g = 0; g < G; ++g) bq[0][g] = rdB(g);
-    unroll([&](auto sc) {
-      constexpr int s = decltype(sc)::value, n0 = 3 * s;
-#pragma unroll
-      for (int g = 0; g < G; ++g) {
-#pragma unroll
-        for (int t = 0; t < 3; ++t) {
-          if constexpr (s == 0) mfma32_asm0<true, NOP>(acc[t][g], wf[(n0 + t) % TW_RING], bq[s & 1][g]);
-          else mfma32_asm<true, NOP>(acc[t][g], wf[(n0 + t) % TW_RING], bq[s & 1][g]);
-        }
-        if constexpr (s + 1 < KS) bq[(s + 1) & 1][g] = rdB((s + 1) * 4 + g);
-        if (g == GI) {
-#pragma unroll
-          for (int t = 0; t < 3; ++t) {
-            const int m = n0 + TW_AH + t;
-            if (m < 72) pw_loadW(wf[(n0 + TW_AH + t) % TW_RING], wrb, lane16, wave, NC, c, m);
-            else pw_loadW(wf[(n0 + TW_AH + t) % TW_RING], wrb, lane16, wave, NC, c + 1, m - 72);
-          }
-        }
-      }
-      __builtin_amdgcn_sched_barrier(0);
-    }, std::make_integer_sequence<int, KS>{});
-    tw_drain_o(acc);
-    const int l = lane_id();
-    const uint32_t bb = bias_lds + 4 * (c * D + 16 * (l >> 5));
-#pragma unroll
-    for (int t = 0; t < 3; ++t) {
-      const int T = 3 * wave + t;
-      float bv[16];
-      ld16(bb + 4 * 32 * T, bv);
-#pragma unroll
-      for (int g = 0; g < G; ++g) {
-        const int ro = ((32 * g + (l & 31)) * NC * D + c * D + 32 * T + 16 * (l >> 5)) * 2;
-#pragma unroll
-        for (int h2 = 0; h2 < 2; ++h2) {
-          float y[8];
-#pragma unroll
-          for (int j = 0; j < 8; ++j) y[j] = acc[t][g][8 * h2 + j] + bv[8 * h2 + j];
-          __builtin_amdgcn_raw_buffer_store_b128(u32x4{pack2(y[0], y[1]), pack2(y[2], y[3]), pack2(y[4], y[5]),
-                                                       pack2(y[6], y[7])},
-                                                 ors, ro + 16 * h2, 0, 0);
-        }
-      }
-    }
-  }
-}
-__device__ __forceinline__ __amdgpu_buffer_rsrc_t pw_out_rsrc(bf16* out, int M, long row0, int NC) {
-  const long o_bytes = ((long)M - row0) * NC * TW_D * 2;
-  return __builtin_amdgcn_make_buffer_rsrc((void*)(out + row0 * NC * TW_D), (short)0,
-                                           (int)(o_bytes < 0x7fffffffL ? o_bytes : 0x7fffffffL), 0x00020000);
-}
 
 template <bool STAMP, int G, bool PROJ>
 __device__ __forceinline__ void tailw_body(const TwArgs& p, const long row0, const int wave) {
diff --git a/rag-snvbert_amd/csrc/tailw_shared.h b/rag-snvbert_amd/csrc/tailw_shared.h
--- /dev/null
+++ b/rag-snvbert_amd/csrc/tailw_shared.h
@@ -0,0 +1,92 @@
+#pragma once
+#include "common.h"
+#include "mfma32.h"
+
+namespace snvrag {
+
+constexpr int TW_D = 384, TW_NT = 12, TW_KS = 24;
+constexpr int TW_FPRE = TW_NT * TW_KS;
+constexpr int TW_FPC = 96;
+constexpr int TW_NFRAG = TW_FPRE + 24 * TW_FPC;
+constexpr int TW_X = 0;
+constexpr int TW_H = 96 * 1024;
+constexpr int TW_LDS = 160 * 1024;
+constexpr int TW_AH = 9;
+constexpr int TW_RING = 12;
+
+__device__ __forceinline__ void tw_drain_o(f32x16 (&a)[3][4]) {
+  asm volatile("s_nop 7\n\ts_nop 7\n\ts_nop 7"
+               : "+a"(a[0][0]), "+a"(a[0][1]), "+a"(a[0][2]), "+a"(a[0][3]), "+a"(a[1][0]), "+a"(a[1][1]),
+                 "+a"(a[1][2]), "+a"(a[1][3]), "+a"(a[2][0]), "+a"(a[2][1]), "+a"(a[2][2]), "+a"(a[2][3])
+               :: "memory");
+}
+__device__ __forceinline__ void tw_barrier() { asm volatile("s_waitcnt lgkmcnt(0)\n\ts_barrier" ::: "memory"); }
+
+__device__ __forceinline__ void pw_loadW(u32x4& r, const __amdgpu_buffer_rsrc_t wrb, int lane16, int wave, int NC, int c,
+                                         int n72) {
+  const int cc = c < NC ? c : NC - 1;
+  r = __builtin_amdgcn_raw_buffer_load_b128(wrb, lane16, (cc * TW_FPRE + (n72 / 3) * TW_NT + 3 * wave + n72 % 3) * FRAG_BYTES, 0);
+}
+template <int G, bool NOP>
+__device__ __forceinline__ void pw_chunks(const char* smem, uint32_t bias_lds, int wave, int lane16,
+                                          const __amdgpu_buffer_rsrc_t wrb, int NC, const __amdgpu_buffer_rsrc_t ors,
+                                          u32x4 (&wf)[TW_RING], f32x16 (&acc)[3][4]) {
+  constexpr int D = TW_D, KS = TW_KS, GI = G > 1 ? 1 : 0;
+  auto rdB = [&](int blk) -> u32x4 { return *reinterpret_cast<const u32x4*>(smem + TW_X + blk * FRAG_BYTES + lane16); };
+  u32x4 bq[2][4];
+#pragma unroll 1
+  for (int c = 0; c < NC; ++c) {
+#pragma unroll
+    for (int g = 0; g < G; ++g) bq[0][g] = rdB(g);
+    unroll([&](auto sc) {
+      constexpr int s = decltype(sc)::value, n0 = 3 * s;
+#pragma unroll
+      for (int g = 0; g < G; ++g) {
+#pragma unroll
+        for (int t = 0; t < 3; ++t) {
+          if constexpr (s == 0) mfma32_asm0<true, NOP>(acc[t][g], wf[(n0 + t) % TW_RING], bq[s & 1][g]);
+          else mfma32_asm<true, NOP>(acc[t][g], wf[(n0 + t) % TW_RING], bq[s & 1][g]);
+        }
+        if constexpr (s + 1 < KS) bq[(s + 1) & 1][g] = rdB((s + 1) * 4 + g);
+        if (g == GI) {
+#pragma unroll
+          for (int t = 0; t < 3; ++t) {
+            const int m = n0 + TW_AH + t;
+            if (m < 72) pw_loadW(wf[(n0 + TW_AH + t) % TW_RING], wrb, lane16, wave, NC, c, m);
+            else pw_loadW(wf[(n0 + TW_AH + t) % TW_RING], wrb, lane16, wave, NC, c + 1, m - 72);
+          }
+        }
+      }
+      __builtin_amdgcn_sched_barrier(0);
+    }, std::make_integer_sequence<int, KS>{});
+    tw_drain_o(acc);
+    const int l = lane_id();
+    const uint32_t bb = bias_lds + 4 * (c * D + 16 * (l >> 5));
+#pragma unroll
+    for (int t = 0; t < 3; ++t) {
+      const int T = 3 * wave + t;
+      float bv[16];
+      ld16(bb + 4 * 32 * T, bv);
+#pragma unroll
+      for (int g = 0; g < G; ++g) {
+        const int ro = ((32 * g + (l & 31)) * NC * D + c * D + 32 * T + 16 * (l >> 5)) * 2;
+#pragma unroll
+        for (int h2 = 0; h2 < 2; ++h2) {
+          float y[8];
+#pragma unroll
+          for (int j = 0; j < 8; ++j) y[j] = acc[t][g][8 * h2 + j] + bv[8 * h2 + j];
+          __builtin_amdgcn_raw_buffer_store_b128(u32x4{pack2(y[0], y[1]), pack2(y[2], y[3]), pack2(y[4], y[5]),
+                                                       pack2(y[6], y[7])},
+                                                 ors, ro + 16 * h2, 0, 0);
+        }
+      }
+    }
+  }
+}
+__device__ __forceinline__ __amdgpu_buffer_rsrc_t pw_out_rsrc(bf16* out, int M, long row0, int NC) {
+  const long o_bytes = ((long)M - row0) * NC * TW_D * 2;
+  return __builtin_amdgcn_make_buffer_rsrc((void*)(out + row0 * NC * TW_D), (short)0,
+                                           (int)(o_bytes < 0x7fffffffL ? o_bytes : 0x7fffffffL), 0x00020000);
+}
+
+}
diff --git a/rag-snvbert_amd/src/engine.py b/rag-snvbert_amd/src/engine.py
--- a/rag-snvbert_amd/src/engine.py
+++ b/rag-snvbert_amd/src/engine.py
@@ -150,6 +150,8 @@
             P.rf["f0_sg"], P.rf["f0_v"] = K.sgemm_pack(P.rf["f0"]), K.sgemm_vec(P.rf["f0b"])
         if sg_ok and D == 384 and P.rf["f3"].shape == (D, 4 * D) and self.rag_tail_wide:
             P.rf["f3_g2"] = K.gemm256_pack(P.rf["f3"])
+        if "f0_sg" in P.rf and "f3_g2" in P.rf:
+            P.rf["rf_ws"] = K.ragfuse_pack(P.rf["f0"], P.rf["f3"])
         mlp_ok = sg_ok and D == 384
         if mlp_ok and P.rf["a0"].shape == (4 * D, D) and P.rf["a3"].shape == (D, 4 * D):
             P.rf["a_mlp"] = K.mlp_pack(P.rf["a0"], P.rf["a3"])
@@ -257,6 +259,12 @@
             out.append(r.to(self.dtype))
         return torch.cat(out, 0).contiguous()
 
+    def _encoder_ws(self, T, nseq: int, L: int, D: int, device) -> torch.Tensor:
+        ws_bytes = K.encoder_ws_bytes(T, nseq, L, D, self.packed().heads)
+        if self._enc_ws is None or self._enc_ws.numel() < ws_bytes or self._enc_ws.device != device:
+            self._enc_ws = torch.empty(ws_bytes, device=device, dtype=torch.uint8)
+        return self._enc_ws
+
     def forward_bert(self, x: Dict[str, torch.Tensor]) -> Dict[str, torch.Tensor]:
         P = self.packed()
         T, D = self.dtype, P.D
@@ -298,6 +306,18 @@
                 else:
                     t = K.linear(fa, rf["a0"], rf["a0b"], act=N.ACT_GELU)
                 aw = K.linear(t, rf["a3"], rf["a3b"], act=N.ACT_SIGMOID)
+            if "rf_ws" in rf and K.get_option("rag_fuse"):
+                ly = P.layers_t[0] if P.layers_t else {}
+                ws = self._encoder_ws(T, 2 * B, L, D, h1.device)
+                qkv0 = "qkv_pw" in ly and K.encoder_one_chunk(T, 2 * B, L, D) and 2 * BL * 3 * D * 2 < 2 ** 31
+                xx = torch.empty(2 * B, L, D, device=h1.device, dtype=T)
+                K.ragfuse_forward(fused[:2 * B], fused[2 * B:], aw, BL, rf["rf_ws"], rf["f0b"], rf["f3b"],
+                                  (rf["g"], rf["bb"]), rf["rs"], af.view(-1), BL,
+                                  qkv_pw=ly["qkv_pw"] if qkv0 else None, b_qkv=ly["b_qkv"] if qkv0 else None,
+                                  qkv_out=K.encoder_qkv0(ws, 2 * BL, D) if qkv0 else None, out=xx)
+                (K.encoder_forward_qkv0 if qkv0 else K.encoder_forward)(xx, P.layers, P.heads, ws)
+                return dict(h1_after=xx[:B], h2_after=xx[B:], h1_before=hm[:B], h2_before=hm[B:2 * B],
+                            af=af, af_p=af_p, x_all=xx, B=B, L=L)
             if "f0_sg" in rf:
                 h = K.sgemm_cat(fused[:2 * B], fused[2 * B:], aw, BL, rf["f0_sg"], rf["f0"].shape[0], rf["f0_v"])
             else:
@@ -312,10 +332,7 @@
                               post_scale=rf["rs"], post_af=af, post_af_period=BL, post_maf=True)
         else:
             xx = fused[:2 * B].clone()
-        ws_bytes = K.encoder_ws_bytes(T, 2 * B, L, D, P.heads)
-        if self._enc_ws is None or self._enc_ws.numel() < ws_bytes or self._enc_ws.device != h1.device:
-            self._enc_ws = torch.empty(ws_bytes, device=h1.device, dtype=torch.uint8)
-        K.encoder_forward(xx, P.layers, P.heads, self._enc_ws)
+        K.encoder_forward(xx, P.layers, P.heads, self._encoder_ws(T, 2 * B, L, D, h1.device))
         return dict(h1_after=xx[:B], h2_after=xx[B:], h1_before=hm[:B], h2_before=hm[B:2 * B],
                     af=af, af_p=af_p, x_all=xx, B=B, L=L)
 
diff --git a/rag-snvbert_amd/src/kernels.py b/rag-snvbert_amd/src/kernels.py
--- a/rag-snvbert_amd/src/kernels.py
+++ b/rag-snvbert_amd/src/kernels.py
@@ -507,8 +507,73 @@
     return int(N.lib().snvrag_encoder_ws_bytes(_dt(dtype), nseq, L, D, heads))
 
 
+def encoder_one_chunk(dtype: torch.dtype, nseq: int, L: int, D: int) -> bool:
+    return int(N.lib().snvrag_encoder_chunk_seqs(_dt(dtype), nseq, L, D)) >= nseq
+
+
+def encoder_forward_qkv0(x: torch.Tensor, layers: Sequence["N.LayerW"], heads: int, ws: torch.Tensor) -> torch.Tensor:
+    nseq, L, D = x.shape
+    arr = (N.LayerW * len(layers))(*layers)
+    check(N.lib().snvrag_encoder_forward_qkv0(_dt(x.dtype), nseq, L, D, heads, len(layers), arr, ptr(_c(x)),
+                                              ptr(ws), ws.numel(), 1, stream_ptr()), "encoder_forward_qkv0")
+    return x
+
+
+def encoder_qkv0(ws: torch.Tensor, M: int, D: int) -> torch.Tensor:
+    return ws[:M * 3 * D * 2].view(torch.bfloat16).view(M, 3 * D)
+
+
+def ragfuse_pack(w0: torch.Tensor, w3: torch.Tensor) -> torch.Tensor:
+    N.require_gpu(w0, w3)
+    D = w3.shape[0]
+    nbytes = int(N.lib().snvrag_ragfuse_pack_bytes(D))
+    if nbytes == 0 or tuple(w0.shape) != (4 * D, 2 * D) or tuple(w3.shape) != (D, 4 * D):
+        raise ValueError(f"the rag fusion kernel needs D = 384, W0 [4D, 2D], W3 [D, 4D]; got {tuple(w0.shape)}, "
+                         f"{tuple(w3.shape)}")
+    ws = [_c(t.to(torch.bfloat16).contiguous()) for t in (w0, w3)]
+    out = torch.empty(nbytes, device=w0.device, dtype=torch.uint8)
+    check(N.lib().snvrag_ragfuse_pack(D, ptr(ws[0]), ptr(ws[1]), ptr(out), stream_ptr()), "ragfuse_pack")
+    return out
+
+
+def ragfuse_forward(h: torch.Tensor, h_rag: torch.Tensor, aw: torch.Tensor, period: int, wstream: torch.Tensor,
+                    b0: torch.Tensor, b3: torch.Tensor, ln: Tuple[torch.Tensor, torch.Tensor], post_scale: float,
+                    post_af: torch.Tensor, post_af_period: int, qkv_pw: Optional[torch.Tensor] = None,
+                    b_qkv: Optional[torch.Tensor] = None, qkv_out: Optional[torch.Tensor] = None,
+                    eps: float = 1e-5, out: Optional[torch.Tensor] = None):
+    N.require_gpu(h, h_rag, aw)
+    D = h.shape[-1]
+    M = h.numel() // D
+    for t in (h, h_rag, aw):
+        assert t.dtype == torch.bfloat16 and t.shape[-1] == D and t.is_contiguous()
+    assert h_rag.numel() == M * D and aw.numel() >= period * D
+    f = [_c(t.float().contiguous()) for t in (b0, b3, ln[0], ln[1])]
+    assert f[0].numel() == 4 * D and all(t.numel() == D for t in f[1:])
+    assert post_af.dtype == torch.float32 and post_af.is_contiguous() and post_af.numel() >= post_af_period
+    if out is None:
+        out = torch.empty_like(h)
+    assert out.dtype == torch.bfloat16 and out.is_contiguous() and out.numel() == M * D
+    bq = None
+    if qkv_pw is not None:
+        bq = _c(b_qkv.float().contiguous())
+        if qkv_out is None:
+            qkv_out = torch.empty(M, 3 * D, device=h.device, dtype=torch.bfloat16)
+        assert qkv_out.dtype == torch.bfloat16 and qkv_out.is_contiguous() and qkv_out.numel() == M * 3 * D
+    check(N.lib().snvrag_ragfuse_forward(M, D, ptr(h), ptr(h_rag), ptr(aw), period, ptr(wstream), ptr(f[0]), ptr(f[1]),
+                                         ptr(f[2]), ptr(f[3]), eps, post_scale, ptr(post_af), post_af_period, ptr(out),
+                                         ptr(qkv_pw), ptr(bq), ptr(qkv_out) if qkv_pw is not None else None,
+                                         stream_ptr()), "ragfuse_forward")
+    return out if qkv_pw is None else (out, qkv_out)
+
+
 def selftest_mfma() -> int:
     return int(N.lib().snvrag_selftest_mfma(stream_ptr()))
+
+
+def get_option(name: str) -> int:
+    v = C.c_int64()
+    check(N.lib().snvrag_get_option(name.encode(), C.byref(v)), "get_option")
+    return int(v.value)
 
 
 def set_option(name: str, value: int) -> int:
diff --git a/rag-snvbert_amd/src/native.py b/rag-snvbert_amd/src/native.py
--- a/rag-snvbert_amd/src/native.py
+++ b/rag-snvbert_amd/src/native.py
@@ -133,6 +133,13 @@
     "snvrag_encoder_ws_bytes": ([C.c_int, i64, i64, C.c_int, C.c_int], sz),
     "snvrag_encoder_forward": ([C.c_int, i64, i64, C.c_int, C.c_int, C.c_int, C.POINTER(LayerW), vp, vp, sz, vp],
                                C.c_int),
+    "snvrag_encoder_chunk_seqs": ([C.c_int, i64, i64, C.c_int], i64),
+    "snvrag_encoder_forward_qkv0": ([C.c_int, i64, i64, C.c_int, C.c_int, C.c_int, C.POINTER(LayerW), vp, vp, sz,
+                                     C.c_int, vp], C.c_int),
+    "snvrag_ragfuse_pack_bytes": ([C.c_int], sz),
+    "snvrag_ragfuse_pack": ([C.c_int, vp, vp, vp, vp], C.c_int),
+    "snvrag_ragfuse_forward": ([i64, C.c_int, vp, vp, vp, i64, vp, vp, vp, vp, vp, f32, f32, vp, i64, vp, vp, vp, vp,
+                                vp], C.c_int),
     "snvrag_proj_pack_bytes": ([C.c_int, C.c_int], sz),
     "snvrag_proj_pack": ([C.c_int, C.c_int, vp, vp, vp], C.c_int),
     "snvrag_proj_forward": ([i64, C.c_int, C.c_int, vp, vp, vp, vp, vp], C.c_int),
```

Result: no change. 8.260 million, median of 6 (+0.7%).
